# mkocabas/EpipolarPose

Measured on AMD Instinct MI355X. Metric: images/sec (4-view 256x256, ResNet-50) at 1/2/4/8 MI355X; MPJPE vs ref, higher is better.
Workload: dtype bf16; 1 GPU; configs[1]: ResNet-50 Integral-pose, 4-view 256x256 synthetic, batch=32/GPU, fully-supervised SmoothL1 loss; global_batch=32, joints=17, depth_res=64, optimizer=adam, parallelism=dp1, launch=eager, streams=2, deterministic=True

## Files before the change

### epipolarpose_amd/csrc/head_gemm.hip

```cpp
#include "common.h"
#include "bn_affine.h"
#include <algorithm>
#include <cstdlib>
#include <mutex>
#include <type_traits>
#include <unordered_map>
#include <utility>
#include <vector>

namespace epi {

typedef __bf16 bf16x8 __attribute__((ext_vector_type(8)));
typedef float f32x16 __attribute__((ext_vector_type(16)));

constexpr int GBK = 64;

template <int TM_, int WM_, int WN_, int MIN_WAVES_, int NSTAGE_, bool STAGGER_ = false> struct GemmCfg {
    static constexpr int TM = TM_, WM = WM_, WN = WN_, NW = WM_ * WN_, THREADS = 64 * NW, MIN_WAVES = MIN_WAVES_, NSTAGE = NSTAGE_;
    static constexpr bool STAGGER = STAGGER_;
    static constexpr int BM = WM_ * TM_ * 32, BN = WN_ * 64;
    static constexpr int A_BYTES = BM * 128, B_BYTES = BN * 128, STAGE_BYTES = A_BYTES + B_BYTES;
    static constexpr int AP = BM / 8 / NW, BP = BN / 8 / NW;
    static constexpr bool EARLY = NW == 4 && NSTAGE_ == 2;
    static_assert(AP >= 1 && BP >= 1 && BM % (8 * NW) == 0 && BN % (8 * NW) == 0, "whole pieces per wave");
    static_assert(NSTAGE_ >= 2 && NSTAGE_ <= 4, "LDS ring depth");
};
typedef GemmCfg<2, 2, 2, 2, 2> CfgSmall;
typedef GemmCfg<2, 4, 1, 2, 2> CfgTall;
typedef GemmCfg<4, 2, 4, 1, 2> CfgBigLock;
typedef GemmCfg<4, 2, 4, 1, 2, true> CfgBig;
typedef GemmCfg<1, 2, 2, 3, 2> CfgHalf;
typedef GemmCfg<1, 2, 1, 3, 2> CfgQuarter;
typedef GemmCfg<2, 2, 2, 1, 4> CfgSmallP;
typedef GemmCfg<2, 4, 1, 1, 3> CfgTallP;

struct GemmGather {
    int enabled;
    int Hg, Wg;
    int Hs, Ws, Cs;
    int stride;
    int dy[16], dx[16];
    int pitch;
};
struct GemmScatter {
    int enabled;
    int Hg, Wg;
    int Ho, Wo;
    int so, oy, ox;
};
struct GemmPhases {
    int enabled;
    int ntap[4];
    int dy[4][4], dx[4][4];
    long long bt_off[4];
};
struct GemmBnRed {
    const unsigned short* z;
    const unsigned short* y;
    const float* bn;
    float* sums;
    int relu;
};

struct GemmArgs {
    const unsigned short* A;
    const unsigned short* Bt;
    void* C;
    const float* bias;
    int M, N, K, lda, ldb, ldc;
    GemmGather ga;
    GemmScatter sc;
    GemmPhases ph;
    int k_per_split;
    float* slabs;
    const unsigned short* addend;
    float* stats;
    int stats_copies;
    int coalesce;
    int patch_px;
    int chunks_per_split;
    GemmBnRed br;
    int addend_step;
    int add_h, add_w;
    int store_policy;
    int bn_in_on;
    BnAffine bn_in;
};

__device__ __forceinline__ int lds_off(int row, int chunk) { return row * 128 + ((chunk ^ ((row >> 1) & 7)) << 4); }

__device__ __forceinline__ int xcd_remap(int lin, int total) {
    const int q = total >> 3, r = total & 7, xcd = lin & 7, idx = lin >> 3;
    return (xcd < r ? xcd * (q + 1) : r * (q + 1) + (xcd - r) * q) + idx;
}

__device__ uint4v epi_zero_chunk[1];

__device__ __forceinline__ void glds16(const void* gsrc, char* lds_base) {
    __builtin_amdgcn_global_load_lds((const __attribute__((address_space(1))) void*)gsrc,
                                     (__attribute__((address_space(3))) void*)lds_base, 16, 0, 0);
}

__device__ __forceinline__ uint4v add_bf16x8(uint4v a, uint4v b) {
    const unsigned int aw[4] = {a.x, a.y, a.z, a.w}, bw[4] = {b.x, b.y, b.z, b.w};
    unsigned int o[4];
#pragma unroll
    for (int k = 0; k < 4; ++k)
        o[k] = pack_bf16x2(__uint_as_float(aw[k] << 16) + __uint_as_float(bw[k] << 16),
                           __uint_as_float(aw[k] & 0xffff0000u) + __uint_as_float(bw[k] & 0xffff0000u));
    uint4v r; r.x = o[0]; r.y = o[1]; r.z = o[2]; r.w = o[3];
    return r;
}

struct BnRedCols { float mu[8], rs[8], sc[8], sh[8]; };
__device__ __forceinline__ void bnred_cols(const GemmBnRed& br, int N, int n, BnRedCols& c) {
    const bool ok = n < N;
#pragma unroll
    for (int h = 0; h < 2; ++h) {
        const float4v zero = float4v{0.f, 0.f, 0.f, 0.f};
        const float4v mu = ok ? *reinterpret_cast<const float4v*>(br.bn + n + 4 * h) : zero;
        const float4v rs = ok ? *reinterpret_cast<const float4v*>(br.bn + N + n + 4 * h) : zero;
        const float4v sc = ok ? *reinterpret_cast<const float4v*>(br.bn + 2 * N + n + 4 * h) : zero;
        const float4v sh = ok ? *reinterpret_cast<const float4v*>(br.bn + 3 * N + n + 4 * h) : zero;
        c.mu[4 * h] = mu.x; c.mu[4 * h + 1] = mu.y; c.mu[4 * h + 2] = mu.z; c.mu[4 * h + 3] = mu.w;
        c.rs[4 * h] = rs.x; c.rs[4 * h + 1] = rs.y; c.rs[4 * h + 2] = rs.z; c.rs[4 * h + 3] = rs.w;
        c.sc[4 * h] = sc.x; c.sc[4 * h + 1] = sc.y; c.sc[4 * h + 2] = sc.z; c.sc[4 * h + 3] = sc.w;
        c.sh[4 * h] = sh.x; c.sh[4 * h + 1] = sh.y; c.sh[4 * h + 2] = sh.z; c.sh[4 * h + 3] = sh.w;
    }
}
__device__ __forceinline__ uint4v bnred_apply(const GemmBnRed& br, uint4v o, uint4v zv, uint4v yv, const BnRedCols& c, float (&s)[8], float (&q)[8]);
__device__ __forceinline__ uint4v bnred_row(const GemmBnRed& br, uint4v o, long long off, const BnRedCols& c, float (&s)[8], float (&q)[8]) {
    const uint4v zv = *reinterpret_cast<const uint4v*>(br.z + off);
    uint4v yv = uint4v{0u, 0u, 0u, 0u};
    if (br.relu && br.y) yv = *reinterpret_cast<const uint4v*>(br.y + off);
    return bnred_apply(br, o, zv, yv, c, s, q);
}
__device__ __forceinline__ uint4v bnred_apply(const GemmBnRed& br, uint4v o, uint4v zv, uint4v yv, const BnRedCols& c, float (&s)[8], float (&q)[8]) {
    unsigned int ow[4] = {o.x, o.y, o.z, o.w};
    const unsigned int zw[4] = {zv.x, zv.y, zv.z, zv.w}, yw[4] = {yv.x, yv.y, yv.z, yv.w};
#pragma unroll
    for (int k = 0; k < 4; ++k) {
#pragma unroll
        for (int h = 0; h < 2; ++h) {
            const int e = 2 * k + h;
            const unsigned int keep = h ? 0xffff0000u : 0x0000ffffu;
            const float g = __uint_as_float(h ? (ow[k] & 0xffff0000u) : (ow[k] << 16));
            const float xv = __uint_as_float(h ? (zw[k] & 0xffff0000u) : (zw[k] << 16));
            bool on = true;
            if (br.relu) on = br.y ? (__uint_as_float(h ? (yw[k] & 0xffff0000u) : (yw[k] << 16)) > 0.f) : (xv * c.sc[e] + c.sh[e] > 0.f);
            const float dz = on ? g : 0.f;
            s[e] += dz;
            q[e] = fmaf(dz, (xv - c.mu[e]) * c.rs[e], q[e]);
            if (!on) ow[k] &= ~keep;
        }
    }
    uint4v r; r.x = ow[0]; r.y = ow[1]; r.z = ow[2]; r.w = ow[3];
    return r;
}

#ifdef EPI_GEMM_TRACE
constexpr int GEMM_TRACE_WGS = 8192, GEMM_TRACE_SLOTS = 16;
__device__ unsigned long long epi_gemm_trace[GEMM_TRACE_WGS * GEMM_TRACE_SLOTS];
#define GEMM_STAMP_V(i, v)                                                                                               \
    do {                                                                                                                 \
        const int wg_ = blockIdx.x + gridDim.x * (blockIdx.y + gridDim.y * blockIdx.z);                                  \
        if (threadIdx.x == 0 && wg_ < GEMM_TRACE_WGS) epi_gemm_trace[wg_ * GEMM_TRACE_SLOTS + (i)] = (v);               \
    } while (0)
#define GEMM_STAMP(i) GEMM_STAMP_V(i, __builtin_amdgcn_s_memtime())
#else
#define GEMM_STAMP_V(i, v) do {} while (0)
#define GEMM_STAMP(i) do {} while (0)
#endif

struct EpiArgs {
    void* C;
    const float* bias;
    const unsigned short* addend;
    float* stats;
    int M, N, ldc, stats_copies, addend_step, add_h, add_w, store_policy;
    GemmScatter sc;
    GemmBnRed br;
};
#define EPI_ARGS_OF(p) EpiArgs{(p).C, (p).bias, (p).addend, (p).stats, (p).M, (p).N, (p).ldc, (p).stats_copies, (p).addend_step, (p).add_h, (p).add_w, (p).store_policy, (p).sc, (p).br}
template <int TM, int WM, int WN, int THREADS, bool RED, bool RED_PREFETCH = true>
__device__ __forceinline__ void coalesced_epilogue(const EpiArgs p, f32x16 (&acc)[TM][2], char* smem, int m0, int n0, int tile_m, int wm, int wn, int wid,
                                                   int lane, int tid, int sc_oy, int sc_ox) {
    constexpr int GBN = WN * 64, ROWS = TM * 4;
    const int frow = lane & 31, fhalf = lane >> 5, c8 = lane & 7, r8 = lane >> 3;
    char* mine = smem + wid * (TM * 32 * 128);
    const int n = n0 + wn * 64 + c8 * 8;
    const int m_first = m0 + wm * (TM * 32) + r8;
    const bool col_ok = n < p.N;
    const bool scatter = p.sc.enabled != 0, has_add = p.addend != nullptr, half_add = p.addend_step == 2, nt_stores = p.store_policy == 1;
    auto row_off = [&](int it, bool& ok, auto sc_c) __attribute__((always_inline)) -> long long {
        const int m = m_first + 8 * it;
        ok = col_ok && m < p.M;
        if (!decltype(sc_c)::value) return (long long)m * p.ldc + n;
        const int hw = p.sc.Hg * p.sc.Wg;
        const int b = m / hw, rem = m - b * hw;
        const int i = rem / p.sc.Wg, j = rem - i * p.sc.Wg;
        return (((long long)b * p.sc.Ho + i * p.sc.so + sc_oy) * p.sc.Wo + j * p.sc.so + sc_ox) * p.ldc + n;
    };
    auto addend_at = [&](int m, long long off) __attribute__((always_inline)) -> uint4v {
        if (!half_add) return *reinterpret_cast<const uint4v*>(p.addend + off);
        const int hw = p.add_h * p.add_w;
        const int b = m / hw, rem = m - b * hw;
        const int yy = rem / p.add_w, xx = rem - yy * p.add_w;
        if ((yy | xx) & 1) return uint4v{0u, 0u, 0u, 0u};
        const long long ar = ((long long)b * (p.add_h >> 1) + (yy >> 1)) * (p.add_w >> 1) + (xx >> 1);
        return *reinterpret_cast<const uint4v*>(p.addend + ar * p.ldc + n);
    };
    constexpr bool AD_EARLY = !(RED && (TM >= 4 || !RED_PREFETCH));
    constexpr int RED_GROUP = 4;
    constexpr bool RED_EARLY = RED && RED_PREFETCH && TM <= 2;
    uint4v ad[AD_EARLY ? ROWS : 1];
    uint4v zpre[RED_EARLY ? ROWS : 1], ypre[RED_EARLY ? ROWS : 1];
    auto prefetch = [&](auto sc_c) __attribute__((always_inline)) {
        if (AD_EARLY && has_add) {
#pragma unroll
            for (int it = 0; it < ROWS; ++it) {
                bool ok;
                const long long off = row_off(it, ok, sc_c);
                ad[it] = ok ? addend_at(m_first + 8 * it, off) : uint4v{0u, 0u, 0u, 0u};
            }
        }
        if (RED_EARLY) {
            const bool use_y = p.br.relu && p.br.y;
#pragma unroll
            for (int it = 0; it < ROWS; ++it) {
                bool ok;
                const long long off = row_off(it, ok, sc_c);
                zpre[it] = ok ? *reinterpret_cast<const uint4v*>(p.br.z + off) : uint4v{0u, 0u, 0u, 0u};
                ypre[it] = (ok && use_y) ? *reinterpret_cast<const uint4v*>(p.br.y + off) : uint4v{0u, 0u, 0u, 0u};
            }
        }
    };
    if (RED_EARLY || (AD_EARLY && has_add)) { if (scatter) prefetch(std::true_type{}); else prefetch(std::false_type{}); }
    auto park = [&](auto bias_c) __attribute__((always_inline)) {
        constexpr bool BIAS = decltype(bias_c)::value;
#pragma unroll
        for (int tj = 0; tj < 2; ++tj)
#pragma unroll
            for (int q = 0; q < 4; ++q) {
                float b[4] = {0.f, 0.f, 0.f, 0.f};
                if (BIAS) {
                    const int nq = n0 + wn * 64 + tj * 32 + 8 * q + 4 * fhalf;
#pragma unroll
                    for (int e = 0; e < 4; ++e) b[e] = nq + e < p.N ? p.bias[nq + e] : 0.f;
                }
#pragma unroll
                for (int ti = 0; ti < TM; ++ti) {
                    const int row = ti * 32 + frow;
                    uint2 t;
                    if (BIAS) {
                        t.x = pack_bf16x2(acc[ti][tj][4 * q] + b[0], acc[ti][tj][4 * q + 1] + b[1]);
                        t.y = pack_bf16x2(acc[ti][tj][4 * q + 2] + b[2], acc[ti][tj][4 * q + 3] + b[3]);
                    } else {
                        t.x = pack_bf16x2(acc[ti][tj][4 * q], acc[ti][tj][4 * q + 1]);
                        t.y = pack_bf16x2(acc[ti][tj][4 * q + 2], acc[ti][tj][4 * q + 3]);
                    }
                    const int unit = tj * 8 + 2 * q + fhalf;
                    *reinterpret_cast<uint2*>(mine + row * 128 + ((unit ^ (row & 15)) << 3)) = t;
                }
            }
    };
    if (p.bias) park(std::true_type{}); else park(std::false_type{});
    GEMM_STAMP(5);
    float ssum[8], ssq[8];
#pragma unroll
    for (int k = 0; k < 8; ++k) { ssum[k] = 0.f; ssq[k] = 0.f; }
    BnRedCols rcols;
    if (RED) bnred_cols(p.br, p.N, n, rcols);
    auto copy_rows = [&](auto stats_c, auto add_c, auto sc_c) __attribute__((always_inline)) {
        constexpr bool STATS = decltype(stats_c)::value, ADD = decltype(add_c)::value;
#pragma unroll
        for (int it = 0; it < ROWS; ++it) {
            if (RED && !RED_EARLY && it % RED_GROUP == 0 && it) __builtin_amdgcn_sched_barrier(0);
            const int row = it * 8 + r8, sw = row & 15;
            const uint2 lo = *reinterpret_cast<const uint2*>(mine + row * 128 + (((2 * c8) ^ sw) << 3));
            const uint2 hi = *reinterpret_cast<const uint2*>(mine + row * 128 + (((2 * c8 + 1) ^ sw) << 3));
            bool ok;
            const long long off = row_off(it, ok, sc_c);
            if (!ok) continue;
            if (STATS) {
                const unsigned int w4[4] = {lo.x, lo.y, hi.x, hi.y};
#pragma unroll
                for (int k = 0; k < 4; ++k) {
                    const float a = __uint_as_float(w4[k] << 16), b = __uint_as_float(w4[k] & 0xffff0000u);
                    ssum[2 * k] += a; ssq[2 * k] = fmaf(a, a, ssq[2 * k]);
                    ssum[2 * k + 1] += b; ssq[2 * k + 1] = fmaf(b, b, ssq[2 * k + 1]);
                }
            }
            uint4v o; o.x = lo.x; o.y = lo.y; o.z = hi.x; o.w = hi.y;
            if (ADD) o = add_bf16x8(o, AD_EARLY ? ad[it] : addend_at(m_first + 8 * it, off));
            if (RED) o = RED_EARLY ? bnred_apply(p.br, o, zpre[it], ypre[it], rcols, ssum, ssq) : bnred_row(p.br, o, off, rcols, ssum, ssq);
            uint4v* dst = reinterpret_cast<uint4v*>(reinterpret_cast<unsigned short*>(p.C) + off);
            if (nt_stores) __builtin_nontemporal_store(o, dst);
            else *dst = o;
        }
    };
    const bool has_stats = !RED && p.stats != nullptr;
    auto copy_sc = [&](auto sc_c) __attribute__((always_inline)) {
        if (has_stats) { if (has_add) copy_rows(std::true_type{}, std::true_type{}, sc_c); else copy_rows(std::true_type{}, std::false_type{}, sc_c); }
        else if (has_add) copy_rows(std::false_type{}, std::true_type{}, sc_c);
        else copy_rows(std::false_type{}, std::false_type{}, sc_c);
    };
    if (scatter) copy_sc(std::true_type{}); else copy_sc(std::false_type{});
    GEMM_STAMP(6);
    if (has_stats || RED) {
#pragma unroll
        for (int k = 0; k < 8; ++k) {
#pragma unroll
            for (int o = 8; o < 64; o <<= 1) { ssum[k] += __shfl_xor(ssum[k], o, 64); ssq[k] += __shfl_xor(ssq[k], o, 64); }
        }
        float* st = reinterpret_cast<float*>(smem + WM * WN * (TM * 32 * 128));
        if (lane < 8) {
            float* row = st + wm * (2 * GBN) + wn * 64 + c8 * 8;
            *reinterpret_cast<float4v*>(row) = float4v{ssum[0], ssum[1], ssum[2], ssum[3]};
            *reinterpret_cast<float4v*>(row + 4) = float4v{ssum[4], ssum[5], ssum[6], ssum[7]};
            *reinterpret_cast<float4v*>(row + GBN) = float4v{ssq[0], ssq[1], ssq[2], ssq[3]};
            *reinterpret_cast<float4v*>(row + GBN + 4) = float4v{ssq[4], ssq[5], ssq[6], ssq[7]};
        }
        __syncthreads();
        float* dst = RED ? p.br.sums : p.stats + (long long)(tile_m % p.stats_copies) * 2 * p.N;
        for (int t = tid; t < 2 * GBN; t += THREADS) {
            float v = 0.f;
#pragma unroll
            for (int w = 0; w < WM; ++w) v += st[w * (2 * GBN) + t];
            const int which = t / GBN, col = n0 + (t % GBN);
            if (col < p.N) atomicAdd(dst + which * p.N + col, v);
        }
    }
#ifdef EPI_GEMM_TRACE
    asm volatile("s_waitcnt vmcnt(0)" ::: "memory");
    GEMM_STAMP(7);
    GEMM_STAMP_V(8, __builtin_amdgcn_s_memrealtime());
#endif
}

enum { A_PLAIN = 0, A_GATHER = 1, A_PHASED = 2 };


__device__ __forceinline__ bf16x8 bn_in_apply(bf16x8 a, const float4v (&t)[4]) {
    const uint4v u = __builtin_bit_cast(uint4v, a);
    const unsigned int w[4] = {u.x, u.y, u.z, u.w};
    unsigned int o[4];
#pragma unroll
    for (int k = 0; k < 4; ++k) {
        const float lo = __uint_as_float(w[k] << 16), hi = __uint_as_float(w[k] & 0xffff0000u);
        o[k] = pack_bf16x2(fmaxf(lo * t[k].x + t[k].y, 0.f), fmaxf(hi * t[k].z + t[k].w, 0.f));
    }
    uint4v r; r.x = o[0]; r.y = o[1]; r.z = o[2]; r.w = o[3];
    return __builtin_bit_cast(bf16x8, r);
}

template <bool OUT_F32, typename Cfg, int MODE, bool RED = false, bool BNIN = false>
__global__ __launch_bounds__(Cfg::THREADS, Cfg::MIN_WAVES) void head_gemm_kernel(GemmArgs p) {
    static_assert(!BNIN || (MODE == A_PLAIN && Cfg::NSTAGE == 2), "BatchNorm on the A operand: plain rows, two-stage loop");
    constexpr int GBM = Cfg::BM, GBN = Cfg::BN, TM = Cfg::TM, AP = Cfg::AP, BP = Cfg::BP;
    extern __shared__ __attribute__((aligned(16))) char smem[];
    const int tid = threadIdx.x, lane = tid & 63, wid = tid >> 6;
    GEMM_STAMP(0);
    GEMM_STAMP_V(1, __builtin_amdgcn_s_memrealtime());
    GEMM_STAMP_V(9, (unsigned long long)__builtin_amdgcn_s_getreg((31 << 11) | 4));
    GEMM_STAMP_V(10, (unsigned long long)__builtin_amdgcn_s_getreg((31 << 11) | 20));
    const int wm = wid / Cfg::WN, wn = wid % Cfg::WN;
    const int tiles_n = (p.N + GBN - 1) / GBN;
    const int total_wg = gridDim.x * gridDim.y * gridDim.z;
    int lid = xcd_remap(blockIdx.x + gridDim.x * (blockIdx.y + gridDim.y * blockIdx.z), total_wg);
    const int tile_id = lid % (int)gridDim.x;
    lid /= (int)gridDim.x;
    const int split_id = lid % (int)gridDim.y, phase = lid / (int)gridDim.y;
    int tile_m = tile_id / tiles_n, tile_n = tile_id - tile_m * tiles_n;
    if constexpr (GBM == 256 && GBN == 256) {
        constexpr int GM = 4;
        const int tiles_m = (p.M + GBM - 1) / GBM, per_group = GM * tiles_n, g = tile_id / per_group, i = tile_id - g * per_group;
        const int rows = min(GM, tiles_m - g * GM);
        tile_m = g * GM + i % rows;
        tile_n = i / rows;
    }
    const int m0 = tile_m * GBM, n0 = tile_n * GBN;
    const int ph = phase >> 1, pw = phase & 1;
    const unsigned short* Bt = p.Bt + (MODE == A_PHASED ? p.ph.bt_off[phase] : 0);
    const int ldb = MODE == A_PHASED ? p.ph.ntap[phase] * p.ga.Cs : p.ldb;
    const int sc_oy = MODE == A_PHASED ? ph : p.sc.oy, sc_ox = MODE == A_PHASED ? pw : p.sc.ox;
    const int k_total = MODE == A_PHASED ? p.ph.ntap[phase] * p.ga.Cs : p.K;
    const int k_begin = split_id * p.k_per_split;
    const int k_end = min(k_total, k_begin + p.k_per_split);
    const int* tap_dy = MODE == A_PHASED ? p.ph.dy[phase] : p.ga.dy;
    const int* tap_dx = MODE == A_PHASED ? p.ph.dx[phase] : p.ga.dx;

    const int schunk_phys = lane & 7;
    int a_pix[AP], a_mask[AP], a_chunk[AP], b_chunk[BP];
    const unsigned short* a_ptr[AP];
    const unsigned short* b_ptr[BP];
    bool b_ok[BP];
    const int ntaps = MODE == A_PLAIN ? 0 : k_total / p.ga.Cs;
#pragma unroll
    for (int ps = 0; ps < AP; ++ps) {
        const int trow = (wid * AP + ps) * 8 + (lane >> 3);
        a_chunk[ps] = (schunk_phys ^ ((trow >> 1) & 7)) * 8;
        const int m = m0 + trow;
        const bool ok = m < p.M;
        if (MODE != A_PLAIN) {
            const int hw = p.ga.Hg * p.ga.Wg;
            const int n = m / hw, rem = m - n * hw;
            const int i = rem / p.ga.Wg, j = rem - i * p.ga.Wg;
            const int iy = i * p.ga.stride, jx = j * p.ga.stride;
            a_pix[ps] = (n * p.ga.Hs + iy) * p.ga.Ws + jx;
            int mask = 0;
            for (int t = 0; t < ntaps; ++t) {
                const int y = iy + tap_dy[t], x = jx + tap_dx[t];
                if (ok && (unsigned)y < (unsigned)p.ga.Hs && (unsigned)x < (unsigned)p.ga.Ws) mask |= 1 << t;
            }
            a_mask[ps] = mask;
            a_ptr[ps] = p.A + a_chunk[ps];
        } else {
            a_pix[ps] = 0;
            a_mask[ps] = ok ? 1 : 0;
            a_ptr[ps] = p.A + (long long)(ok ? m : 0) * p.lda + a_chunk[ps];
        }
    }
#pragma unroll
    for (int ps = 0; ps < BP; ++ps) {
        const int trow = (wid * BP + ps) * 8 + (lane >> 3);
        b_chunk[ps] = (schunk_phys ^ ((trow >> 1) & 7)) * 8;
        const int n = n0 + trow;
        b_ok[ps] = n < p.N;
        b_ptr[ps] = Bt + (long long)(b_ok[ps] ? n : 0) * ldb + b_chunk[ps];
    }
    const char* zero_src = reinterpret_cast<const char*>(epi_zero_chunk);
    const int nk = k_end > k_begin ? (k_end - k_begin + GBK - 1) / GBK : 0;
    int k_run = k_begin;
    int g_tap = MODE == A_PLAIN ? 0 : k_run / p.ga.Cs;
    int g_c0 = MODE == A_PLAIN ? 0 : k_run - g_tap * p.ga.Cs;
    int g_shift = (MODE == A_PLAIN || ntaps == 0) ? 0 : tap_dy[min(g_tap, ntaps - 1)] * p.ga.Ws + tap_dx[min(g_tap, ntaps - 1)];
    auto issue_a = [&](int ps, int, int buf) {
        const int k0 = k_run;
        char* a_s = smem + buf * Cfg::STAGE_BYTES + __builtin_amdgcn_readfirstlane(wid) * (AP * 1024);
        const void* src;
        if (MODE != A_PLAIN) {
            const unsigned eoff = (unsigned)(a_pix[ps] + g_shift) * (unsigned)(p.ga.pitch ? p.ga.pitch : p.ga.Cs) + (unsigned)g_c0;
            const bool in_k = !Cfg::STAGGER || k0 < k_end;
            src = (in_k && ((a_mask[ps] >> (g_tap & 31)) & 1)) ? reinterpret_cast<const void*>(a_ptr[ps] + eoff) : reinterpret_cast<const void*>(zero_src);
        } else {
            const bool ok = a_mask[ps] && (k0 + a_chunk[ps] < k_end);
            src = ok ? reinterpret_cast<const void*>(a_ptr[ps] + k0) : reinterpret_cast<const void*>(zero_src);
        }
        glds16(src, a_s + ps * 1024);
    };
    auto issue_b = [&](int ps, int, int buf) {
        const int k0 = k_run;
        char* b_s = smem + buf * Cfg::STAGE_BYTES + Cfg::A_BYTES + __builtin_amdgcn_readfirstlane(wid) * (BP * 1024);
        const bool ok = b_ok[ps] && (MODE != A_PLAIN || k0 + b_chunk[ps] < k_end);
        glds16(ok ? reinterpret_cast<const void*>(b_ptr[ps] + k0) : reinterpret_cast<const void*>(zero_src), b_s + ps * 1024);
    };
    auto advance_gather = [&]() {
        k_run += GBK;
        if (MODE != A_PLAIN) {
            g_c0 += GBK;
            if (g_c0 >= p.ga.Cs) {
                g_c0 = 0;
                g_tap += 1;
                const int t = min(g_tap, ntaps - 1);
                g_shift = tap_dy[t] * p.ga.Ws + tap_dx[t];
            }
        }
    };
    auto issue_tile = [&](int k0, int buf) {
#pragma unroll
        for (int ps = 0; ps < AP; ++ps) issue_a(ps, k0, buf);
#pragma unroll
        for (int ps = 0; ps < BP; ++ps) issue_b(ps, k0, buf);
        advance_gather();
    };

    f32x16 acc[TM][2];
#pragma unroll
    for (int i = 0; i < TM; ++i)
#pragma unroll
        for (int j = 0; j < 2; ++j)
#pragma unroll
            for (int r = 0; r < 16; ++r) acc[i][j][r] = 0.f;

    const int frow = lane & 31, fhalf = lane >> 5;
    float2* bn_tab = reinterpret_cast<float2*>(smem + Cfg::NSTAGE * Cfg::STAGE_BYTES);
    if (BNIN) {
        const bool lead = (blockIdx.x | blockIdx.y | blockIdx.z) == 0;
        for (int k = tid; k < p.K; k += Cfg::THREADS) {
            float sc, sh;
            bn_derive(p.bn_in, p.K, k, lead, sc, sh);
            bn_tab[k] = float2{sc, sh};
        }
        if (lead && tid == 0 && p.bn_in.num_batches && p.bn_in.sums) p.bn_in.num_batches[0] += 1;
    }
    const int a_frag = lds_off(wm * (TM * 32) + frow, fhalf), b_frag = lds_off(wn * 64 + frow, fhalf);
    auto read_frags = [&](const char* a_s, const char* b_s, int ks, bf16x8 (&af)[TM], bf16x8 (&bfr)[2]) {
#pragma unroll
        for (int t = 0; t < TM; ++t)
            af[t] = __builtin_bit_cast(bf16x8, *reinterpret_cast<const uint4v*>(a_s + ((a_frag ^ (ks << 5)) + t * 4096)));
#pragma unroll
        for (int t = 0; t < 2; ++t)
            bfr[t] = __builtin_bit_cast(bf16x8, *reinterpret_cast<const uint4v*>(b_s + ((b_frag ^ (ks << 5)) + t * 4096)));
    };
    auto issue_quarter = [&](int ks, int k0, int buf) {
#pragma unroll
        for (int ps = 0; ps < AP; ++ps)
            if (ps * 4 / AP == ks) issue_a(ps, k0, buf);
#pragma unroll
        for (int ps = 0; ps < BP; ++ps)
            if ((BP >= 4 ? ps * 4 / BP : ps) == ks) issue_b(ps, k0, buf);
        if (ks == 3) advance_gather();
    };
    auto compute_tile = [&](int buf, bool spread_next, int k_next, int buf_next, int k_tile = 0) {
        const char* a_s = smem + buf * Cfg::STAGE_BYTES;
        const char* b_s = a_s + Cfg::A_BYTES;
        bf16x8 af[2][TM], bfr[2][2];
        float4v bt[2][4];
        auto read_tab = [&](int ks, float4v (&t)[4]) {
            const float4v* src = reinterpret_cast<const float4v*>(bn_tab + k_tile + ks * 16 + fhalf * 8);
#pragma unroll
            for (int q = 0; q < 4; ++q) t[q] = src[q];
        };
        read_frags(a_s, b_s, 0, af[0], bfr[0]);
        if (BNIN) read_tab(0, bt[0]);
#pragma unroll
        for (int ks = 0; ks < 4; ++ks) {
            if (ks < 3) read_frags(a_s, b_s, ks + 1, af[(ks + 1) & 1], bfr[(ks + 1) & 1]);
            if (BNIN && ks < 3) read_tab(ks + 1, bt[(ks + 1) & 1]);
            __builtin_amdgcn_sched_barrier(0);
            if (BNIN) {
#pragma unroll
                for (int ti = 0; ti < TM; ++ti) af[ks & 1][ti] = bn_in_apply(af[ks & 1][ti], bt[ks & 1]);
            }
            if (spread_next) issue_quarter(ks, k_next, buf_next);
#pragma unroll
            for (int ti = 0; ti < TM; ++ti)
#pragma unroll
                for (int tj = 0; tj < 2; ++tj)
                    acc[ti][tj] = __builtin_amdgcn_mfma_f32_32x32x16_bf16(bfr[ks & 1][tj], af[ks & 1][ti], acc[ti][tj], 0, 0, 0);
        }
    };
    GEMM_STAMP(2);
    GEMM_STAMP_V(11, (unsigned long long)nk);
    if constexpr (Cfg::STAGGER) {
        static_assert(AP == 4 && BP == 4 && TM == 4 && Cfg::NW == 8 && Cfg::NSTAGE == 2 && !BNIN, "staggered loop: 256 x 256 tile, 8 waves");
        const int grp = __builtin_amdgcn_readfirstlane(wid) >> 2;
        int kb_run = k_begin;
        auto issue_a_tile = [&](int buf) {
#pragma unroll
            for (int ps = 0; ps < AP; ++ps) issue_a(ps, 0, buf);
            advance_gather();
        };
        auto issue_b_tile = [&](int buf) {
            char* b_s = smem + buf * Cfg::STAGE_BYTES + Cfg::A_BYTES + __builtin_amdgcn_readfirstlane(wid) * (BP * 1024);
#pragma unroll
            for (int ps = 0; ps < BP; ++ps) {
                const bool ok = b_ok[ps] && kb_run + b_chunk[ps] < k_end;
                glds16(ok ? reinterpret_cast<const void*>(b_ptr[ps] + kb_run) : reinterpret_cast<const void*>(zero_src), b_s + ps * 1024);
            }
            kb_run += GBK;
        };
        issue_b_tile(0);
        issue_a_tile(0);
        issue_b_tile(1);
        asm volatile("s_waitcnt vmcnt(4)" ::: "memory");
        __builtin_amdgcn_s_barrier();
        GEMM_STAMP(3);
        if (grp) __builtin_amdgcn_s_barrier();
        bf16x8 af[4][2], bfr[4][2];
        auto mfma_half = [&](int h) {
            __builtin_amdgcn_s_setprio(1);
#pragma unroll
            for (int ks = 0; ks < 4; ++ks)
#pragma unroll
                for (int ti = 0; ti < 2; ++ti)
#pragma unroll
                    for (int tj = 0; tj < 2; ++tj)
                        acc[2 * h + ti][tj] = __builtin_amdgcn_mfma_f32_32x32x16_bf16(bfr[ks][tj], af[ks][ti], acc[2 * h + ti][tj], 0, 0, 0);
            __builtin_amdgcn_s_setprio(0);
        };
        for (int kt = 0; kt < nk; ++kt) {
            const int buf = kt & 1;
            const char* a_s = smem + buf * Cfg::STAGE_BYTES;
            const char* b_s = a_s + Cfg::A_BYTES;
#pragma unroll
            for (int ks = 0; ks < 4; ++ks)
#pragma unroll
                for (int tj = 0; tj < 2; ++tj)
                    bfr[ks][tj] = __builtin_bit_cast(bf16x8, *reinterpret_cast<const uint4v*>(b_s + ((b_frag ^ (ks << 5)) + tj * 4096)));
#pragma unroll
            for (int ks = 0; ks < 4; ++ks)
#pragma unroll
                for (int ti = 0; ti < 2; ++ti)
                    af[ks][ti] = __builtin_bit_cast(bf16x8, *reinterpret_cast<const uint4v*>(a_s + ((a_frag ^ (ks << 5)) + ti * 4096)));
            __builtin_amdgcn_sched_barrier(0);
            issue_a_tile(buf ^ 1);
            __builtin_amdgcn_sched_barrier(0);
            asm volatile("s_waitcnt lgkmcnt(0)" ::: "memory");
            __builtin_amdgcn_s_barrier();
            __builtin_amdgcn_sched_barrier(0);
            mfma_half(0);
            __builtin_amdgcn_sched_barrier(0);
            asm volatile("s_waitcnt vmcnt(4)" ::: "memory");
            __builtin_amdgcn_s_barrier();
            __builtin_amdgcn_sched_barrier(0);
#pragma unroll
            for (int ks = 0; ks < 4; ++ks)
#pragma unroll
                for (int ti = 0; ti < 2; ++ti)
                    af[ks][ti] = __builtin_bit_cast(bf16x8, *reinterpret_cast<const uint4v*>(a_s + ((a_frag ^ (ks << 5)) + (2 + ti) * 4096)));
            __builtin_amdgcn_sched_barrier(0);
            issue_b_tile(buf);
            __builtin_amdgcn_sched_barrier(0);
            asm volatile("s_waitcnt lgkmcnt(0)" ::: "memory");
            __builtin_amdgcn_s_barrier();
            __builtin_amdgcn_sched_barrier(0);
            mfma_half(1);
            __builtin_amdgcn_sched_barrier(0);
            asm volatile("s_waitcnt vmcnt(4)" ::: "memory");
            __builtin_amdgcn_s_barrier();
            __builtin_amdgcn_sched_barrier(0);
        }
        if (!grp) __builtin_amdgcn_s_barrier();
        asm volatile("s_waitcnt vmcnt(0) lgkmcnt(0)" ::: "memory");
        __builtin_amdgcn_s_barrier();
    } else if constexpr (Cfg::NSTAGE > 2) {
        constexpr int S = Cfg::NSTAGE, DPT = AP + BP;
#pragma unroll
        for (int t = 0; t < S - 1; ++t)
            if (t < nk) issue_tile(k_begin + t * GBK, t);
        int kt = 0;
        for (; kt + (S - 2) < nk; ++kt) {
            asm volatile("s_waitcnt vmcnt(%0)" ::"n"((S - 2) * DPT) : "memory");
            __builtin_amdgcn_s_barrier();
#ifdef EPI_GEMM_TRACE
            if (kt == 0) GEMM_STAMP(3);
#endif
            const int nxt = kt + S - 1;
            compute_tile(kt % S, nxt < nk, k_begin + nxt * GBK, nxt % S);
        }
        for (; kt < nk; ++kt) {
            if (S > 3 && nk - 1 - kt == 1) asm volatile("s_waitcnt vmcnt(%0)" ::"n"(DPT) : "memory");
            else asm volatile("s_waitcnt vmcnt(0)" ::: "memory");
            __builtin_amdgcn_s_barrier();
            compute_tile(kt % S, false, 0, 0);
        }
        asm volatile("s_waitcnt lgkmcnt(0)" ::: "memory");
        __builtin_amdgcn_s_barrier();
    } else {
        if (nk > 0) issue_tile(k_begin, 0);
        __syncthreads();
        GEMM_STAMP(3);
        for (int kt = 0; kt < nk; ++kt) {
            const bool has_next = kt + 1 < nk;
            const int k_next = k_begin + (kt + 1) * GBK, buf = kt & 1;
            if (Cfg::EARLY && has_next) issue_tile(k_next, buf ^ 1);
            compute_tile(buf, !Cfg::EARLY && has_next, k_next, buf ^ 1, k_begin + kt * GBK);
            __syncthreads();
        }
    }

    GEMM_STAMP(4);
    if (gridDim.y > 1) {
        float* slab = p.slabs + ((long long)split_id * gridDim.z + phase) * p.M * p.N;
#pragma unroll
        for (int ti = 0; ti < TM; ++ti) {
            const int m = m0 + wm * (TM * 32) + ti * 32 + frow;
            if (m >= p.M) continue;
#pragma unroll
            for (int tj = 0; tj < 2; ++tj)
#pragma unroll
                for (int q = 0; q < 4; ++q) {
                    const int n = n0 + wn * 64 + tj * 32 + 8 * q + 4 * fhalf;
                    if (n + 3 < p.N) {
                        float4v t; t.x = acc[ti][tj][4 * q]; t.y = acc[ti][tj][4 * q + 1]; t.z = acc[ti][tj][4 * q + 2]; t.w = acc[ti][tj][4 * q + 3];
                        *reinterpret_cast<float4v*>(slab + (long long)m * p.N + n) = t;
                    } else {
                        for (int e = 0; e < 4 && n + e < p.N; ++e) slab[(long long)m * p.N + n + e] = acc[ti][tj][4 * q + e];
                    }
                }
        }
#ifdef EPI_GEMM_TRACE
        GEMM_STAMP(6);
        asm volatile("s_waitcnt vmcnt(0)" ::: "memory");
        GEMM_STAMP(7);
        GEMM_STAMP_V(8, __builtin_amdgcn_s_memrealtime());
#endif
        return;
    }
    if constexpr (!OUT_F32) {
        if (p.coalesce) {
            coalesced_epilogue<TM, Cfg::WM, Cfg::WN, Cfg::THREADS, RED>(EPI_ARGS_OF(p), acc, smem, m0, n0, tile_m, wm, wn, wid, lane, tid, sc_oy, sc_ox);
            return;
        }
    }
#pragma unroll
    for (int ti = 0; ti < TM; ++ti) {
        const int m = m0 + wm * (TM * 32) + ti * 32 + frow;
        const bool row_ok = m < p.M;
        long long orow = m;
        if (p.sc.enabled) {
            const int hw = p.sc.Hg * p.sc.Wg;
            const int n = m / hw, rem = m - n * hw;
            const int i = rem / p.sc.Wg, j = rem - i * p.sc.Wg;
            orow = ((long long)n * p.sc.Ho + i * p.sc.so + sc_oy) * p.sc.Wo + j * p.sc.so + sc_ox;
        }
#pragma unroll
        for (int tj = 0; tj < 2; ++tj) {
#pragma unroll
            for (int q = 0; q < 4; ++q) {
                const int n = n0 + wn * 64 + tj * 32 + 8 * q + 4 * fhalf;
                float v[4];
#pragma unroll
                for (int e = 0; e < 4; ++e) {
                    v[e] = acc[ti][tj][4 * q + e];
                    if (p.bias && n + e < p.N) v[e] += p.bias[n + e];
                }
                if (row_ok && n < p.N) {
                    if (OUT_F32) {
                        float* c = reinterpret_cast<float*>(p.C) + orow * p.ldc + n;
                        if (n + 3 < p.N) { float4v t; t.x = v[0]; t.y = v[1]; t.z = v[2]; t.w = v[3]; *reinterpret_cast<float4v*>(c) = t; }
                        else for (int e = 0; e < 4 && n + e < p.N; ++e) c[e] = v[e];
                    } else {
                        unsigned short* c = reinterpret_cast<unsigned short*>(p.C) + orow * p.ldc + n;
                        if (p.addend)
                            for (int e = 0; e < 4 && n + e < p.N; ++e) v[e] = bf16_to_f32(f32_to_bf16(v[e])) + bf16_to_f32(p.addend[orow * p.ldc + n + e]);
                        if (n + 3 < p.N) {
                            uint2 t;
                            t.x = pack_bf16x2(v[0], v[1]);
                            t.y = pack_bf16x2(v[2], v[3]);
                            *reinterpret_cast<uint2*>(c) = t;
                        } else for (int e = 0; e < 4 && n + e < p.N; ++e) c[e] = f32_to_bf16(v[e]);
                    }
                }
            }
        }
    }
}

constexpr int AS_WAVES = 8, AS_LOADERS = 2, AS_RING = 3;
constexpr int AS_THREADS = 64 * (AS_WAVES + AS_LOADERS), AS_BM = 32 * AS_WAVES, AS_BN = 64;

template <int KSTEPS>
__global__ __launch_bounds__(AS_THREADS, 1) void head_gemm_astat_kernel(GemmArgs p) {
    constexpr int K = 16 * KSTEPS, ROW_BYTES = 2 * K, CHUNKS = ROW_BYTES / 16;
    constexpr int BTILE = AS_BN * ROW_BYTES;
    constexpr int ROWS_PER_PIECE = 1024 / ROW_BYTES, PIECES = BTILE / 1024 / AS_LOADERS;
    extern __shared__ __attribute__((aligned(16))) char smem[];
    const int tid = threadIdx.x, lane = tid & 63, wid = tid >> 6;
    const bool loader = wid >= AS_WAVES;
    const int frow = lane & 31, fhalf = lane >> 5;
    const int m0 = xcd_remap(blockIdx.x, gridDim.x) * AS_BM + wid * 32;
    const int n_tiles = (p.N + AS_BN - 1) / AS_BN;
    const char* zero_src = reinterpret_cast<const char*>(epi_zero_chunk);
    float* bias_s = reinterpret_cast<float*>(smem + AS_RING * BTILE + AS_WAVES * 4096);
    float* stats_s = bias_s + n_tiles * AS_BN;
    for (int n = tid; n < n_tiles * AS_BN; n += AS_THREADS) bias_s[n] = (p.bias && n < p.N) ? p.bias[n] : 0.f;
    if (p.stats)
        for (int n = tid; n < 2 * n_tiles * AS_BN; n += AS_THREADS) stats_s[n] = 0.f;

    auto issue_b = [&](int nt) {
        const int lw = wid - AS_WAVES;
        char* dst = smem + (nt % AS_RING) * BTILE + lw * (PIECES * 1024);
#pragma unroll 8
        for (int q = 0; q < PIECES; ++q) {
            const int r = (lw * PIECES + q) * ROWS_PER_PIECE + lane / CHUNKS;
            const int chunk = (lane % CHUNKS) ^ (r % CHUNKS);
            const int n = nt * AS_BN + r;
            const void* src = n < p.N ? reinterpret_cast<const void*>(p.Bt + (long long)n * p.ldb + chunk * 8)
                                      : reinterpret_cast<const void*>(zero_src);
            glds16(src, dst + q * 1024);
        }
    };
    bf16x8 af[KSTEPS];
    if (loader) {
        issue_b(0);
        if (n_tiles > 1) issue_b(1);
    } else {
        const int m = m0 + frow;
        const uint4v* arow = reinterpret_cast<const uint4v*>(p.A + (long long)(m < p.M ? m : 0) * p.lda) + fhalf;
#pragma unroll
        for (int ks = 0; ks < KSTEPS; ++ks) {
            uint4v v = arow[2 * ks];
            if (m >= p.M) v.x = v.y = v.z = v.w = 0u;
            af[ks] = __builtin_bit_cast(bf16x8, v);
        }
    }
    __syncthreads();
    if (loader) {
        for (int nt = 0; nt < n_tiles; ++nt) {
            if (nt + 2 < n_tiles) {
                issue_b(nt + 2);
                asm volatile("s_waitcnt vmcnt(%0)\n\ts_barrier" ::"n"(PIECES) : "memory");
            } else {
                asm volatile("s_waitcnt vmcnt(0)\n\ts_barrier" ::: "memory");
            }
        }
        if (p.stats) __builtin_amdgcn_s_barrier();
        return;
    }
    char* stage = smem + AS_RING * BTILE + wid * 4096;
    const int c8 = lane & 7;
    auto slices = [&](auto add_c, auto stats_c) __attribute__((always_inline)) {
    constexpr bool ADD = decltype(add_c)::value, STATS = decltype(stats_c)::value;
    for (int nt = 0; nt < n_tiles; ++nt) {
        f32x16 acc[2];
#pragma unroll
        for (int j = 0; j < 2; ++j)
#pragma unroll
            for (int r = 0; r < 16; ++r) acc[j][r] = 0.f;
        const unsigned slice_off = (unsigned)(nt % AS_RING) * BTILE;
        auto read_b = [&](int ks, uint4v (&f)[2]) {
#pragma unroll
            for (int tj = 0; tj < 2; ++tj) {
                const int r = tj * 32 + frow;
                const unsigned off = (slice_off + r * ROW_BYTES + (((fhalf ^ r) % CHUNKS) << 4)) ^ (unsigned)(((2 * ks) % CHUNKS) << 4);
                f[tj] = *reinterpret_cast<const uint4v*>(smem + off);
            }
        };
        uint4v ad[4];
        auto load_addend = [&]() {
            if (!ADD) return;
#pragma unroll
            for (int it = 0; it < 4; ++it) {
                const int m = m0 + it * 8 + (lane >> 3), nn = nt * AS_BN + (lane & 7) * 8;
                ad[it] = (m < p.M && nn < p.N) ? *reinterpret_cast<const uint4v*>(p.addend + (long long)m * p.ldc + nn) : uint4v{0u, 0u, 0u, 0u};
            }
        };
        if (KSTEPS <= 8) load_addend();
        uint4v fb[3][2];
        read_b(0, fb[0]);
        if (KSTEPS > 1) read_b(1, fb[1]);
#pragma unroll
        for (int ks = 0; ks < KSTEPS; ++ks) {
            if (ks + 2 < KSTEPS) read_b(ks + 2, fb[(ks + 2) % 3]);
            __builtin_amdgcn_sched_barrier(0);
#pragma unroll
            for (int tj = 0; tj < 2; ++tj)
                acc[tj] = __builtin_amdgcn_mfma_f32_32x32x16_bf16(__builtin_bit_cast(bf16x8, fb[ks % 3][tj]), af[ks], acc[tj], 0, 0, 0);
        }
        asm volatile("s_waitcnt lgkmcnt(0)\n\ts_barrier" ::: "memory");
        const int n0 = nt * AS_BN;
#pragma unroll
        for (int tj = 0; tj < 2; ++tj)
#pragma unroll
            for (int q = 0; q < 4; ++q) {
                const int nl = tj * 32 + 8 * q + 4 * fhalf;
                const float4v bv = *reinterpret_cast<const float4v*>(bias_s + n0 + nl);
                const float v0 = acc[tj][4 * q] + bv.x, v1 = acc[tj][4 * q + 1] + bv.y, v2 = acc[tj][4 * q + 2] + bv.z,
                            v3 = acc[tj][4 * q + 3] + bv.w;
                uint2 t;
                t.x = pack_bf16x2(v0, v1);
                t.y = pack_bf16x2(v2, v3);
                const int unit = tj * 8 + 2 * q + fhalf;
                *reinterpret_cast<uint2*>(stage + frow * 128 + ((unit ^ (frow & 15)) << 3)) = t;
            }
        const int n = n0 + c8 * 8;
        float ssum[8], ssq[8];
#pragma unroll
        for (int k = 0; k < 8; ++k) { ssum[k] = 0.f; ssq[k] = 0.f; }
#pragma unroll
        for (int it = 0; it < 4; ++it) {
            const int row = it * 8 + (lane >> 3), sw = row & 15;
            const uint2 lo = *reinterpret_cast<const uint2*>(stage + row * 128 + (((2 * c8) ^ sw) << 3));
            const uint2 hi = *reinterpret_cast<const uint2*>(stage + row * 128 + (((2 * c8 + 1) ^ sw) << 3));
            const int m = m0 + row;
            if (m < p.M && n < p.N) {
                uint4v o; o.x = lo.x; o.y = lo.y; o.z = hi.x; o.w = hi.y;
                if (ADD) o = add_bf16x8(o, KSTEPS <= 8 ? ad[it] : *reinterpret_cast<const uint4v*>(p.addend + (long long)m * p.ldc + n));
                *reinterpret_cast<uint4v*>(reinterpret_cast<unsigned short*>(p.C) + (long long)m * p.ldc + n) = o;
                if (STATS) {
                    const unsigned int w4[4] = {lo.x, lo.y, hi.x, hi.y};
#pragma unroll
                    for (int k = 0; k < 4; ++k) {
                        const float a = __uint_as_float(w4[k] << 16), b = __uint_as_float(w4[k] & 0xffff0000u);
                        ssum[2 * k] += a; ssq[2 * k] = fmaf(a, a, ssq[2 * k]);
                        ssum[2 * k + 1] += b; ssq[2 * k + 1] = fmaf(b, b, ssq[2 * k + 1]);
                    }
                }
            }
        }
        if (STATS) {
#pragma unroll
            for (int k = 0; k < 8; ++k) {
#pragma unroll
                for (int o = 8; o < 64; o <<= 1) { ssum[k] += __shfl_xor(ssum[k], o, 64); ssq[k] += __shfl_xor(ssq[k], o, 64); }
            }
            if (lane < 8) {
#pragma unroll
                for (int k = 0; k < 8; ++k) {
                    atomicAdd(stats_s + n + k, ssum[k]);
                    atomicAdd(stats_s + n_tiles * AS_BN + n + k, ssq[k]);
                }
            }
        }
    }
    };
    if (p.addend) { if (p.stats) slices(std::true_type{}, std::true_type{}); else slices(std::true_type{}, std::false_type{}); }
    else if (p.stats) slices(std::false_type{}, std::true_type{});
    else slices(std::false_type{}, std::false_type{});
    if (p.stats) {
        asm volatile("s_waitcnt lgkmcnt(0)\n\ts_barrier" ::: "memory");
        float* dst = p.stats + (long long)(blockIdx.x % p.stats_copies) * 2 * p.N;
        for (int n = tid; n < p.N; n += 64 * AS_WAVES) {
            atomicAdd(dst + n, stats_s[n]);
            atomicAdd(dst + p.N + n, stats_s[n_tiles * AS_BN + n]);
        }
    }
}

template <int TM_, int WM_, int WN_> struct PatchCfg {
    static constexpr int TM = TM_, WM = WM_, WN = WN_, NW = WM_ * WN_, THREADS = 64 * NW;
    static constexpr int BM = WM_ * TM_ * 32, BN = WN_ * 64, B_BYTES = BN * 128, BP = BN / 8 / NW;
    static_assert(NW == 8 && BP >= 1, "8 waves");
};
typedef PatchCfg<2, 4, 2> PatchWide;
typedef PatchCfg<1, 8, 1> PatchNarrow;
typedef PatchCfg<1, 4, 2> PatchHalf;
constexpr int PATCH_TAPS = 9, PATCH_APW = 8;

#ifdef EPI_PATCH_TRACE
__device__ unsigned long long epi_patch_trace[64 * 96];
#define PATCH_STAMP(i)                                                                                                   \
    do {                                                                                                                 \
        const int wg_ = blockIdx.x + gridDim.x * blockIdx.y;                                                             \
        if (lane == 0 && wid == 0 && wg_ % 16 == 0 && wg_ / 16 < 64 && (i) < 96) epi_patch_trace[(wg_ / 16) * 96 + (i)] = __builtin_amdgcn_s_memtime(); \
    } while (0)
#else
#define PATCH_STAMP(i) do {} while (0)
#endif

template <typename Cfg, int NB, bool SINGLE, bool RED = false>
__global__ __launch_bounds__(Cfg::THREADS, SINGLE ? 4 : 2) void conv_patch_kernel(GemmArgs p) {
    constexpr int TM = Cfg::TM, GBN = Cfg::BN, BP = Cfg::BP, NW = Cfg::NW, BB = Cfg::B_BYTES;
    constexpr int NPATCH = SINGLE ? 1 : 2, GROUP = BP + (SINGLE ? 0 : 1);
    extern __shared__ __attribute__((aligned(16))) char smem[];
    const int tid = threadIdx.x, lane = tid & 63, wid = __builtin_amdgcn_readfirstlane(tid >> 6);
    const int wm = wid / Cfg::WN, wn = wid % Cfg::WN;
    const int tiles_n = (p.N + GBN - 1) / GBN;
    const int lid = xcd_remap(blockIdx.x + gridDim.x * blockIdx.y, gridDim.x * gridDim.y);
    const int tile_id = lid % (int)gridDim.x, split_id = lid / (int)gridDim.x;
    const int tile_m = tile_id / tiles_n, tile_n = tile_id - tile_m * tiles_n;
    const int m0 = tile_m * Cfg::BM, n0 = tile_n * GBN;
    const int W = p.ga.Wg, H = p.ga.Hg, Cs = p.ga.Cs;
    const int c_begin = split_id * p.chunks_per_split, c_end = min(Cs / GBK, c_begin + p.chunks_per_split);
    const int PB = p.patch_px * 128;
    const int ring_off = NPATCH * PB, dummy_off = ring_off + NB * BB, zero_off = dummy_off + 1024;
    PATCH_STAMP(0);
    if (tid < 32) reinterpret_cast<float*>(smem + zero_off)[tid] = 0.f;
    const char* zero_src = reinterpret_cast<const char*>(epi_zero_chunk);

    auto a_off = [&](int j) -> int {
        const int prow = (j * NW + wid) * 8 + (lane >> 3);
        const long long pin = (long long)m0 - (W + 1) + prow;
        const bool ok = prow < p.patch_px && pin >= 0 && pin < p.M;
        return ok ? (int)pin * Cs + (((lane & 7) ^ ((prow >> 1) & 7)) << 3) : -1;
    };
    const unsigned short* b_ptr[BP];
    bool b_ok[BP];
#pragma unroll
    for (int ps = 0; ps < BP; ++ps) {
        const int trow = (wid * BP + ps) * 8 + (lane >> 3);
        const int n = n0 + trow;
        b_ok[ps] = n < p.N;
        b_ptr[ps] = p.Bt + (long long)(b_ok[ps] ? n : 0) * p.ldb + (((lane & 7) ^ ((trow >> 1) & 7)) << 3);
    }
    auto issue_a = [&](int j, int c, int buf) {
        const bool real = j < PATCH_APW && (j * NW + wid) * 8 < p.patch_px && c < c_end;
        char* dst = real ? smem + buf * PB + (j * NW + wid) * 1024 : smem + dummy_off;
        const int off = a_off(j);
        glds16((real && off >= 0) ? reinterpret_cast<const void*>(p.A + off + c * GBK) : reinterpret_cast<const void*>(zero_src), dst);
    };
    auto issue_b = [&](int t, int c, int slot, bool real) {
#pragma unroll
        for (int ps = 0; ps < BP; ++ps) {
            char* dst = real ? smem + ring_off + slot * BB + (wid * BP + ps) * 1024 : smem + dummy_off;
            const void* src = (real && b_ok[ps]) ? reinterpret_cast<const void*>(b_ptr[ps] + t * Cs + c * GBK) : reinterpret_cast<const void*>(zero_src);
            glds16(src, dst);
        }
    };

    const int frow = lane & 31, fhalf = lane >> 5;
    const int b_frag = ring_off + lds_off(wn * 64 + frow, fhalf);

    f32x16 acc[TM][2];
#pragma unroll
    for (int i = 0; i < TM; ++i)
#pragma unroll
        for (int j = 0; j < 2; ++j)
#pragma unroll
            for (int r = 0; r < 16; ++r) acc[i][j][r] = 0.f;

    const int nsteps = (c_end - c_begin) * PATCH_TAPS;
    if (nsteps > 0) {
#pragma unroll
        for (int j = 0; j < PATCH_APW; ++j) issue_a(j, c_begin, 0);
        issue_b(0, c_begin, 0, true);
        if (NB > 2) issue_b(1, c_begin, 1, true);
    }
    __builtin_amdgcn_sched_barrier(0);
    int amask[TM], arow[TM];
#pragma unroll
    for (int ti = 0; ti < TM; ++ti) {
        const int r = wm * (TM * 32) + ti * 32 + frow, m = m0 + r;
        arow[ti] = r;
        const int j = m % W, i = (m / W) % H;
        int mask = 0;
#pragma unroll
        for (int t = 0; t < PATCH_TAPS; ++t) {
            const int y = i + p.ga.dy[t], x = j + p.ga.dx[t];
            if (m < p.M && (unsigned)y < (unsigned)H && (unsigned)x < (unsigned)W) mask |= 1 << t;
        }
        amask[ti] = mask;
    }
    PATCH_STAMP(1);
    asm volatile("s_waitcnt vmcnt(0) lgkmcnt(0)" ::: "memory");
    __builtin_amdgcn_s_barrier();
    PATCH_STAMP(2);
    int step_no = 0;

    int slot = 0;
    for (int c = c_begin; c < c_end; ++c) {
        const int pbuf = SINGLE ? 0 : (c - c_begin) & 1;
#pragma unroll
        for (int t = 0; t < PATCH_TAPS; ++t) {
            {
                int ta = t + NB - 1, ca = c;
                if (ta >= PATCH_TAPS) { ta -= PATCH_TAPS; ca += 1; }
                int sa = slot + NB - 1; if (sa >= NB) sa -= NB;
                issue_b(ta, ca, sa, ca < c_end);
                if (!SINGLE) issue_a(t, c + 1, pbuf ^ 1);
            }
            const int sh = (p.ga.dy[t] + 1) * W + p.ga.dx[t] + 1;
            int a_addr[TM];
#pragma unroll
            for (int ti = 0; ti < TM; ++ti) {
                const int pr = arow[ti] + sh;
                const int in = pbuf * PB + pr * 128 + ((fhalf ^ ((pr >> 1) & 7)) << 4);
                a_addr[ti] = ((amask[ti] >> t) & 1) ? in : zero_off;
            }
            const int b_addr = b_frag + slot * BB;
            bf16x8 af[2][TM], bfr[2][2];
            auto read_frags = [&](int ks, bf16x8 (&a)[TM], bf16x8 (&b)[2]) {
#pragma unroll
                for (int ti = 0; ti < TM; ++ti) a[ti] = __builtin_bit_cast(bf16x8, *reinterpret_cast<const uint4v*>(smem + (a_addr[ti] ^ (ks << 5))));
#pragma unroll
                for (int tj = 0; tj < 2; ++tj) b[tj] = __builtin_bit_cast(bf16x8, *reinterpret_cast<const uint4v*>(smem + ((b_addr ^ (ks << 5)) + tj * 4096)));
            };
            read_frags(0, af[0], bfr[0]);
#pragma unroll
            for (int ks = 0; ks < 4; ++ks) {
                if (ks < 3) read_frags(ks + 1, af[(ks + 1) & 1], bfr[(ks + 1) & 1]);
                __builtin_amdgcn_sched_barrier(0);
#pragma unroll
                for (int ti = 0; ti < TM; ++ti)
#pragma unroll
                    for (int tj = 0; tj < 2; ++tj)
                        acc[ti][tj] = __builtin_amdgcn_mfma_f32_32x32x16_bf16(bfr[ks & 1][tj], af[ks & 1][ti], acc[ti][tj], 0, 0, 0);
            }
            asm volatile("s_waitcnt vmcnt(%0)" ::"n"((NB - 2) * GROUP) : "memory");
            __builtin_amdgcn_s_barrier();
            slot = slot + 1 == NB ? 0 : slot + 1;
            PATCH_STAMP(3 + step_no);
            ++step_no;
        }
    }
    asm volatile("s_waitcnt vmcnt(0) lgkmcnt(0)" ::: "memory");
    __builtin_amdgcn_s_barrier();
    PATCH_STAMP(3 + step_no);

    if (gridDim.y > 1) {
        float* slab = p.slabs + (long long)split_id * p.M * p.N;
#pragma unroll
        for (int ti = 0; ti < TM; ++ti) {
            const int m = m0 + arow[ti];
            if (m >= p.M) continue;
#pragma unroll
            for (int tj = 0; tj < 2; ++tj)
#pragma unroll
                for (int q = 0; q < 4; ++q) {
                    const int n = n0 + wn * 64 + tj * 32 + 8 * q + 4 * fhalf;
                    if (n + 3 < p.N) {
                        float4v t; t.x = acc[ti][tj][4 * q]; t.y = acc[ti][tj][4 * q + 1]; t.z = acc[ti][tj][4 * q + 2]; t.w = acc[ti][tj][4 * q + 3];
                        *reinterpret_cast<float4v*>(slab + (long long)m * p.N + n) = t;
                    }
                }
        }
#ifdef EPI_PATCH_TRACE
        asm volatile("s_waitcnt vmcnt(0)" ::: "memory");
        PATCH_STAMP(4 + step_no);
#endif
        return;
    }
    coalesced_epilogue<TM, Cfg::WM, Cfg::WN, Cfg::THREADS, RED, false>(EPI_ARGS_OF(p), acc, smem, m0, n0, tile_m, wm, wn, wid, lane, tid, 0, 0);
#ifdef EPI_PATCH_TRACE
    asm volatile("s_waitcnt vmcnt(0)" ::: "memory");
    PATCH_STAMP(4 + step_no);
#endif
}

template <bool OUT_F32>
__global__ void splitk_finish_kernel(const float* __restrict__ slabs, int nsplit, int nphase, GemmArgs p) {
    const long long nq = (long long)p.N >> 2;
    const long long t = (long long)blockIdx.x * blockDim.x + threadIdx.x;
    if (t >= (long long)nphase * p.M * nq) return;
    const int n = (int)(t % nq) * 4;
    const long long pm = t / nq;
    const int m = (int)(pm % p.M), phase = (int)(pm / p.M);
    float4v a; a.x = a.y = a.z = a.w = 0.f;
    for (int s = 0; s < nsplit; ++s) {
        const float4v v = *reinterpret_cast<const float4v*>(slabs + (((long long)s * nphase + phase) * p.M + m) * p.N + n);
        a.x += v.x; a.y += v.y; a.z += v.z; a.w += v.w;
    }
    if (p.bias) { a.x += p.bias[n]; a.y += p.bias[n + 1]; a.z += p.bias[n + 2]; a.w += p.bias[n + 3]; }
    long long orow = m;
    if (p.sc.enabled) {
        const int hw = p.sc.Hg * p.sc.Wg;
        const int b = m / hw, rem = m - b * hw;
        const int i = rem / p.sc.Wg, j = rem - i * p.sc.Wg;
        const int oy = p.ph.enabled ? (phase >> 1) : p.sc.oy, ox = p.ph.enabled ? (phase & 1) : p.sc.ox;
        orow = ((long long)b * p.sc.Ho + i * p.sc.so + oy) * p.sc.Wo + j * p.sc.so + ox;
    }
    if (OUT_F32) {
        *reinterpret_cast<float4v*>(reinterpret_cast<float*>(p.C) + orow * p.ldc + n) = a;
    } else {
        if (p.addend) {
            const uint2 r = *reinterpret_cast<const uint2*>(p.addend + orow * p.ldc + n);
            a.x = bf16_to_f32(f32_to_bf16(a.x)) + __uint_as_float(r.x << 16); a.y = bf16_to_f32(f32_to_bf16(a.y)) + __uint_as_float(r.x & 0xffff0000u);
            a.z = bf16_to_f32(f32_to_bf16(a.z)) + __uint_as_float(r.y << 16); a.w = bf16_to_f32(f32_to_bf16(a.w)) + __uint_as_float(r.y & 0xffff0000u);
        }
        uint2 o;
        o.x = pack_bf16x2(a.x, a.y);
        o.y = pack_bf16x2(a.z, a.w);
        *reinterpret_cast<uint2*>(reinterpret_cast<unsigned short*>(p.C) + orow * p.ldc + n) = o;
    }
}

constexpr int FS_ROWS = 32;
__global__ __launch_bounds__(256) void splitk_finish_stats_kernel(const float* __restrict__ slabs, int nsplit, GemmArgs p) {
    __shared__ float red[4][2][256];
    const int tx = threadIdx.x & 63, ty = threadIdx.x >> 6;
    const int col_tiles = (p.N + 255) / 256;
    const int tile_m = blockIdx.x / col_tiles, tile_n = blockIdx.x - tile_m * col_tiles;
    const int n = tile_n * 256 + tx * 4;
    float s1[4] = {0.f, 0.f, 0.f, 0.f}, s2[4] = {0.f, 0.f, 0.f, 0.f};
    if (n < p.N) {
        for (int r = ty; r < FS_ROWS; r += 4) {
            const int m = tile_m * FS_ROWS + r;
            if (m >= p.M) break;
            float4v a; a.x = a.y = a.z = a.w = 0.f;
            for (int sp = 0; sp < nsplit; ++sp) {
                const float4v v = *reinterpret_cast<const float4v*>(slabs + ((long long)sp * p.M + m) * p.N + n);
                a.x += v.x; a.y += v.y; a.z += v.z; a.w += v.w;
            }
            uint2 o;
            o.x = pack_bf16x2(a.x, a.y);
            o.y = pack_bf16x2(a.z, a.w);
            *reinterpret_cast<uint2*>(reinterpret_cast<unsigned short*>(p.C) + (long long)m * p.ldc + n) = o;
            const float v[4] = {__uint_as_float(o.x << 16), __uint_as_float(o.x & 0xffff0000u), __uint_as_float(o.y << 16), __uint_as_float(o.y & 0xffff0000u)};
#pragma unroll
            for (int e = 0; e < 4; ++e) { s1[e] += v[e]; s2[e] = fmaf(v[e], v[e], s2[e]); }
        }
    }
#pragma unroll
    for (int e = 0; e < 4; ++e) { red[ty][0][tx * 4 + e] = s1[e]; red[ty][1][tx * 4 + e] = s2[e]; }
    __syncthreads();
    float* dst = p.stats + (long long)(tile_m % p.stats_copies) * 2 * p.N;
    for (int t = threadIdx.x; t < 512; t += 256) {
        const int which = t >> 8, c = t & 255, col = tile_n * 256 + c;
        if (col < p.N) atomicAdd(dst + which * p.N + col, red[0][which][c] + red[1][which][c] + red[2][which][c] + red[3][which][c]);
    }
}

}

using namespace epi;

enum { CFG_SMALL = 0, CFG_TALL = 1, CFG_BIG = 2, CFG_HALF = 3, CFG_QUARTER = 4 };
struct GemmPlan { int cfg; int nsplit, kps; long long tiles; int pipe; };

static int g_tile_force_fwd();
static int gemm_tile_override() {
    const int v = 0;
    const int f = g_tile_force_fwd();
    return f == 1 || f == 2 ? f : (f == 5 ? 2 : v);
}

static int g_pipe_force_fwd();
static int gemm_pipe_mode() {
    const int v = 0;
    const int f = g_pipe_force_fwd();
    return f >= 0 ? f : v;
}

static int g_store_policy = -1;
static int gemm_store_policy() {
    if (g_store_policy < 0) g_store_policy = 0;
    return g_store_policy;
}
extern "C" int epi_gemm_store_policy(int v) {
    const int before = gemm_store_policy();
    if (v >= 0) g_store_policy = v;
    return before;
}
static int g_tile_force = 0, g_pipe_force = -1;
extern "C" int epi_gemm_tune(int tile, int pipe) {
    if (tile >= 0) g_tile_force = tile;
    if (pipe >= -1) g_pipe_force = pipe;
    return g_tile_force;
}

static int g_tile_force_fwd() { return g_tile_force; }
static int g_pipe_force_fwd() { return g_pipe_force; }

static GemmPlan gemm_plan_cfg(int cfg, int M, int N, int K, int nphase, bool pipe = false) {
    GemmPlan pl;
    pl.cfg = cfg;
    pl.pipe = pipe ? 1 : 0;
    const int bm = cfg == CFG_SMALL ? 128 : (cfg == CFG_HALF || cfg == CFG_QUARTER ? 64 : 256);
    const int bn = cfg == CFG_BIG ? 256 : (cfg == CFG_TALL || cfg == CFG_QUARTER ? 64 : 128);
    pl.tiles = (long long)((M + bm - 1) / bm) * ((N + bn - 1) / bn);
    const long long wgs = pl.tiles * nphase;
    const bool one_per_cu = cfg == CFG_BIG || pipe;
    const long long enough_env = 120;
    const long long enough = enough_env, target = one_per_cu ? 256 : 512;
    int nsplit = 1;
    if (wgs < enough) {
        nsplit = (int)(target / wgs);
        const int max_split = K / 512 > 0 ? K / 512 : 1;
        if (nsplit > max_split) nsplit = max_split;
        if (nsplit > 16) nsplit = 16;
        if (nsplit < 1) nsplit = 1;
    }
    if (N % 4) nsplit = 1;
    pl.kps = K;
    if (nsplit > 1) {
        pl.kps = ((K + nsplit - 1) / nsplit + GBK - 1) / GBK * GBK;
        nsplit = (K + pl.kps - 1) / pl.kps;
    }
    pl.nsplit = nsplit;
    return pl;
}

static GemmPlan gemm_plan(int M, int N, int K, int ldc, int nphase, bool out_f32, bool allow_pipe = true) {
    const int ov = gemm_tile_override();
    const bool can_big = !out_f32 && N % 8 == 0 && ldc % 8 == 0;
    if (can_big && ov != 1) {
        const GemmPlan pb = gemm_plan_cfg(CFG_BIG, M, N, K, nphase);
        const int tiles_n = (N + 255) / 256;
        const bool fills = M >= 256 && tiles_n * 256 <= N + N / 4;
        const bool deep = pb.nsplit == 1 ? (K >= 512 && pb.tiles * nphase >= 200) : pb.kps >= 1024;
        const bool big_split_ok = false;
        const bool small_fills_unsplit = (long long)((M + 127) / 128) * ((N + 127) / 128) * nphase >= 200;
        if (ov == 2 || (fills && deep && (pb.nsplit == 1 || big_split_ok || !small_fills_unsplit))) return pb;
    }
    int cfg = (ov == 0 && !out_f32 && N <= 64 && (long long)M * nphase >= 256 * 256) ? CFG_TALL : CFG_SMALL;
    const long long fill_env = 0;
    if (cfg == CFG_SMALL && !out_f32 && (g_tile_force == 3 || g_tile_force == 4)) cfg = g_tile_force == 3 ? CFG_HALF : CFG_QUARTER;
    else if (cfg == CFG_SMALL && ov == 0 && !out_f32 && fill_env > 0) {
        const long long t128 = (long long)((M + 127) / 128) * ((N + 127) / 128) * nphase;
        const long long t64x128 = (long long)((M + 63) / 64) * ((N + 127) / 128) * nphase;
        if (t128 < fill_env) cfg = t64x128 < fill_env ? CFG_QUARTER : CFG_HALF;
    }
    const int pm = (out_f32 || !allow_pipe || cfg == CFG_HALF || cfg == CFG_QUARTER) ? 0 : gemm_pipe_mode();
    if (pm) {
        const GemmPlan pp = gemm_plan_cfg(cfg, M, N, K, nphase, true);
        const bool one_round = pp.tiles * nphase * pp.nsplit <= 256;
        const bool long_underfilled = pp.tiles * nphase * pp.nsplit <= 128 && pp.kps >= 32 * GBK;
        if (pm == 2 || (pm == 1 && pp.kps >= 6 * GBK) || (pm == 3 && one_round && pp.kps >= 6 * GBK) || (pm == 4 && long_underfilled)) return pp;
    }
    return gemm_plan_cfg(cfg, M, N, K, nphase);
}

extern "C" size_t epi_gemm_workspace_bytes(int M, int N, int K, int nphase) {
    if (M <= 0 || N <= 0 || K <= 0 || nphase <= 0) return 0;
    size_t need = 0;
    for (int pipe = 0; pipe < 2; ++pipe) {
        for (int f32 = 0; f32 < 2; ++f32) {
            const GemmPlan pl = gemm_plan(M, N, K, 8, nphase, f32 != 0, pipe != 0);
            if (pl.nsplit > 1) need = std::max(need, (size_t)pl.nsplit * nphase * M * N * sizeof(float));
        }
        const GemmPlan ps = gemm_plan(M, N, K, 4, nphase, false, pipe != 0);
        if (ps.nsplit > 1) need = std::max(need, (size_t)ps.nsplit * nphase * M * N * sizeof(float));
    }
    return need;
}

template <bool OUT_F32, typename Cfg, int MODE, bool RED = false, bool BNIN = false>
static int launch_gemm_mode(const GemmArgs& a, const GemmPlan& pl, int nphase, hipStream_t st) {
    constexpr size_t ring = (size_t)Cfg::NSTAGE * Cfg::STAGE_BYTES;
    const bool one_tile = !BNIN && !Cfg::STAGGER && Cfg::NSTAGE == 2 && pl.kps <= GBK;
    const size_t staged = one_tile ? (size_t)Cfg::STAGE_BYTES : ring;
    const size_t lds = BNIN ? ring + (size_t)a.K * sizeof(float2)
                            : std::max(staged, (size_t)Cfg::WM * Cfg::WN * (Cfg::TM * 32 * 128) + (size_t)Cfg::WM * 2 * Cfg::BN * sizeof(float));
    static_assert(!BNIN || ring >= (size_t)Cfg::WM * Cfg::WN * (Cfg::TM * 32 * 128) + (size_t)Cfg::WM * 2 * Cfg::BN * sizeof(float), "epilogue areas end below the table");
    if (lds > 65536) {
        constexpr size_t full = std::max(ring, (size_t)Cfg::WM * Cfg::WN * (Cfg::TM * 32 * 128) + (size_t)Cfg::WM * 2 * Cfg::BN * sizeof(float));
        static const hipError_t attr = hipFuncSetAttribute(reinterpret_cast<const void*>(&head_gemm_kernel<OUT_F32, Cfg, MODE, RED, BNIN>),
                                                           hipFuncAttributeMaxDynamicSharedMemorySize, BNIN ? (int)(ring + 2048 * sizeof(float2)) : (int)full);
        if (attr != hipSuccess) return EPI_ERR_LAUNCH;
    }
    const dim3 grid((unsigned)pl.tiles, (unsigned)pl.nsplit, (unsigned)nphase);
    hipLaunchKernelGGL((head_gemm_kernel<OUT_F32, Cfg, MODE, RED, BNIN>), grid, dim3(Cfg::THREADS), lds, st, a);
    EPI_CHECK_LAUNCH();
    return EPI_OK;
}
template <bool OUT_F32, typename Cfg, bool RED = false>
static int launch_gemm_cfg(const GemmArgs& a, const GemmPlan& pl, int nphase, hipStream_t st) {
    if (a.ph.enabled) return launch_gemm_mode<OUT_F32, Cfg, A_PHASED, RED>(a, pl, nphase, st);
    if (a.ga.enabled) return launch_gemm_mode<OUT_F32, Cfg, A_GATHER, RED>(a, pl, nphase, st);
    return launch_gemm_mode<OUT_F32, Cfg, A_PLAIN, RED>(a, pl, nphase, st);
}

#ifdef EPI_GEMM_TRACE
extern "C" int epi_gemm_trace_read(unsigned long long* out, int clear) {
    const size_t bytes = sizeof(unsigned long long) * epi::GEMM_TRACE_WGS * epi::GEMM_TRACE_SLOTS;
    if (hipMemcpyFromSymbol(out, HIP_SYMBOL(epi::epi_gemm_trace), bytes) != hipSuccess) return 1;
    if (clear) {
        static unsigned long long zeros[epi::GEMM_TRACE_WGS * epi::GEMM_TRACE_SLOTS];
        if (hipMemcpyToSymbol(HIP_SYMBOL(epi::epi_gemm_trace), zeros, bytes) != hipSuccess) return 1;
    }
    return 0;
}
#endif

#ifdef EPI_PATCH_TRACE
extern "C" int epi_patch_trace_read(unsigned long long* out, int clear) {
    if (hipMemcpyFromSymbol(out, HIP_SYMBOL(epi::epi_patch_trace), sizeof(unsigned long long) * 64 * 96) != hipSuccess) return 1;
    if (clear) {
        static unsigned long long zeros[64 * 96];
        if (hipMemcpyToSymbol(HIP_SYMBOL(epi::epi_patch_trace), zeros, sizeof(zeros)) != hipSuccess) return 1;
    }
    return 0;
}
#endif

enum { PATCH_WIDE = 0, PATCH_NARROW = 1, PATCH_HALF = 2 };
struct PatchPlan { bool ok; int cfg, nb, patch_px, nsplit, cps; long long tiles; size_t lds; bool single; };
static int g_patch_mode = -1;
static int patch_mode() {
    if (g_patch_mode < 0) g_patch_mode = 2;
    return g_patch_mode;
}
extern "C" int epi_conv3x3_patch_mode(int mode) {
    const int before = patch_mode();
    if (mode >= 0 && mode <= 2) g_patch_mode = mode;
    return before;
}
static PatchPlan patch_plan(int M, int N, int Cs, int W, size_t workspace_bytes) {
    PatchPlan pl = {};
    const int nchunks = Cs / GBK;
    pl.cfg = N <= 64 ? PATCH_NARROW : PATCH_WIDE;
    if (pl.cfg == PATCH_WIDE && (long long)((M + 255) / 256) * ((N + 127) / 128) < 200) pl.cfg = PATCH_HALF;
    const int bm = pl.cfg == PATCH_HALF ? 128 : 256, bn = pl.cfg == PATCH_NARROW ? 64 : 128;
    const int tm = pl.cfg == PATCH_WIDE ? 2 : 1, wmv = pl.cfg == PATCH_NARROW ? 8 : 4;
    pl.patch_px = (bm + 2 * W + 2 + 7) / 8 * 8;
    if (pl.patch_px > 8 * 8 * PATCH_APW) return pl;
    const size_t epi = (size_t)8 * tm * 32 * 128 + (size_t)wmv * 2 * bn * sizeof(float);
    pl.single = pl.cfg == PATCH_NARROW && nchunks == 1;
    for (pl.nb = 3; pl.nb >= 2; --pl.nb) {
        pl.lds = std::max((size_t)(pl.single ? 1 : 2) * pl.patch_px * 128 + (size_t)pl.nb * bn * 128 + 1024 + 128, epi);
        if (pl.lds <= 160 * 1024) break;
    }
    if (pl.nb < 2) return pl;
    pl.tiles = (long long)((M + bm - 1) / bm) * ((N + bn - 1) / bn);
    pl.nsplit = 1;
    if (pl.tiles < 120) {
        if (patch_mode() < 2) return pl;
        pl.nsplit = (int)std::min<long long>(nchunks, std::max<long long>(1, 256 / pl.tiles));
    }
    while (pl.nsplit > 1 && (size_t)pl.nsplit * M * N * sizeof(float) > workspace_bytes) --pl.nsplit;
    pl.cps = (nchunks + pl.nsplit - 1) / pl.nsplit;
    pl.nsplit = (nchunks + pl.cps - 1) / pl.cps;
    pl.ok = pl.tiles <= 0x7fffffffLL;
    return pl;
}
static bool patch_eligible(const GemmArgs& a, bool out_f32, int nphase) {
    if (patch_mode() == 0 || out_f32 || nphase != 1 || !a.ga.enabled || a.ph.enabled || a.sc.enabled || a.bias || !a.coalesce) return false;
    if (a.ga.stride != 1 || a.ga.Hg != a.ga.Hs || a.ga.Wg != a.ga.Ws || a.ga.Cs % GBK || a.K != PATCH_TAPS * a.ga.Cs || a.ga.pitch) return false;
    for (int t = 0; t < PATCH_TAPS; ++t)
        if (a.ga.dy[t] < -1 || a.ga.dy[t] > 1 || a.ga.dx[t] < -1 || a.ga.dx[t] > 1) return false;
    return (long long)a.M * a.ga.Cs < (1LL << 31) && gemm_tile_override() == 0;
}
template <typename Cfg, int NB, bool SINGLE = false, bool RED = false>
static int launch_patch_red(const GemmArgs& a, const PatchPlan& pl, hipStream_t st) {
    static const hipError_t attr = hipFuncSetAttribute(reinterpret_cast<const void*>(&conv_patch_kernel<Cfg, NB, SINGLE, RED>),
                                                       hipFuncAttributeMaxDynamicSharedMemorySize, 160 * 1024);
    if (attr != hipSuccess) return EPI_ERR_LAUNCH;
    hipLaunchKernelGGL((conv_patch_kernel<Cfg, NB, SINGLE, RED>), dim3((unsigned)pl.tiles, (unsigned)pl.nsplit), dim3(Cfg::THREADS), pl.lds, st, a);
    EPI_CHECK_LAUNCH();
    return EPI_OK;
}
template <typename Cfg, int NB, bool SINGLE = false>
static int launch_patch(const GemmArgs& a, const PatchPlan& pl, hipStream_t st) {
    return a.br.z ? launch_patch_red<Cfg, NB, SINGLE, true>(a, pl, st) : launch_patch_red<Cfg, NB, SINGLE, false>(a, pl, st);
}

static int launch_gemm(GemmArgs a, bool out_f32, int nphase, void* workspace, size_t workspace_bytes, hipStream_t st, int* stats_done = nullptr,
                       int* red_done = nullptr) {
    if (stats_done) *stats_done = 0;
    if (red_done) *red_done = 0;
    a.store_policy = gemm_store_policy();
    const bool fuse_red = true;
    GemmBnRed want_red = a.br;
    a.br = GemmBnRed{};
    const long long red_max_rows = 1LL << 40;
    const long long red_min_rows = 0;
    if (deterministic() || !fuse_red || !red_done || !want_red.z || !want_red.bn || !want_red.sums || a.stats || a.bias ||
        ((reinterpret_cast<uintptr_t>(want_red.z) | reinterpret_cast<uintptr_t>(want_red.y)) & 15u) || (long long)a.M * nphase > red_max_rows ||
        (long long)a.M * nphase < red_min_rows)
        want_red.z = nullptr;
    if (a.addend && (out_f32 || (reinterpret_cast<uintptr_t>(a.addend) & 15u))) return EPI_ERR_UNSUPPORTED;
    a.coalesce = (!out_f32 && a.N % 8 == 0 && a.ldc % 8 == 0) ? 1 : 0;
    const bool half_addend = a.addend && a.addend_step == 2;
    if (half_addend && (!a.coalesce || a.ga.enabled || a.sc.enabled || a.ph.enabled || nphase != 1 || a.add_h <= 0 || a.add_w <= 0 || ((a.add_h | a.add_w) & 1) ||
                        (long long)a.M % ((long long)a.add_h * a.add_w)))
        return EPI_ERR_UNSUPPORTED;
    const bool fuse_stats = true;
    float* const want_stats = (fuse_stats && !deterministic()) ? a.stats : nullptr;
    a.stats = nullptr;
    if (!a.A || !a.Bt || !a.C || a.M <= 0 || a.N <= 0 || a.K <= 0) return EPI_ERR_INVALID_ARGUMENT;
    if (a.K % 8 || a.ldb % 8 || a.ldc % 4 || (!a.ga.enabled && a.lda % 8)) return EPI_ERR_UNSUPPORTED;
    if ((reinterpret_cast<uintptr_t>(a.A) | reinterpret_cast<uintptr_t>(a.Bt) | reinterpret_cast<uintptr_t>(a.C)) & 15u) return EPI_ERR_UNSUPPORTED;
    if (a.ga.enabled && (a.ga.Cs % GBK)) return EPI_ERR_UNSUPPORTED;
    if (a.bn_in_on) {
        if (out_f32 || a.ga.enabled || a.sc.enabled || a.ph.enabled || nphase != 1 || a.K % GBK || a.K > 2048 || want_red.z || a.bias || a.addend || !a.coalesce ||
            !a.bn_in.gamma || !a.bn_in.beta || !a.bn_in.scale || !a.bn_in.shift)
            return EPI_ERR_UNSUPPORTED;
        const GemmPlan pl = gemm_plan_cfg(CFG_SMALL, a.M, a.N, a.K, 1);
        if (pl.tiles > 0x7fffffffLL) return EPI_ERR_UNSUPPORTED;
        if (pl.nsplit > 1) {
            if (!workspace || (size_t)pl.nsplit * a.M * a.N * sizeof(float) > workspace_bytes) return EPI_ERR_WORKSPACE;
            a.slabs = (float*)workspace;
        }
        a.k_per_split = pl.kps;
        if (want_stats && pl.nsplit == 1) { a.stats = want_stats; if (stats_done) *stats_done = 1; }
        const int rc = launch_gemm_mode<false, CfgSmall, A_PLAIN, false, true>(a, pl, 1, st);
        if (rc != EPI_OK) return rc;
        if (pl.nsplit > 1) {
            if (want_stats && a.N % 4 == 0) {
                a.stats = want_stats;
                if (stats_done) *stats_done = 1;
                const unsigned blocks = (unsigned)(((a.M + FS_ROWS - 1) / FS_ROWS) * ((a.N + 255) / 256));
                hipLaunchKernelGGL(splitk_finish_stats_kernel, dim3(blocks), dim3(256), 0, st, a.slabs, pl.nsplit, a);
            } else {
                const long long n = (long long)a.M * (a.N >> 2);
                hipLaunchKernelGGL(splitk_finish_kernel<false>, dim3((unsigned)((n + 255) / 256)), dim3(256), 0, st, a.slabs, pl.nsplit, 1, a);
            }
            EPI_CHECK_LAUNCH();
        }
        return EPI_OK;
    }
    const bool stats_off_astat = true;
    if (!want_red.z && !(want_stats && stats_off_astat && !a.bias) && !half_addend &&
        !out_f32 && !a.ga.enabled && !a.sc.enabled && nphase == 1 && (a.K == 64 || a.K == 128 || a.K == 256) && a.N % 8 == 0 &&
        a.ldc % 8 == 0 && a.N >= 4 * AS_BN && a.N <= 8192 && a.M >= 64 * AS_BM && gemm_tile_override() == 0) {
        const unsigned grid = (unsigned)((a.M + AS_BM - 1) / AS_BM);
        const bool astat_stats = false;
        if (want_stats && !a.bias && astat_stats) { a.stats = want_stats; if (stats_done) *stats_done = 1; }
#define EPI_ASTAT(KS)                                                                                                      \
        do {                                                                                                               \
            const size_t lds = AS_RING * (size_t)AS_BN * 32 * KS + AS_WAVES * 4096 + (size_t)((a.N + AS_BN - 1) / AS_BN) * AS_BN * 4 * 3;                                          \
            static const hipError_t attr = hipFuncSetAttribute(reinterpret_cast<const void*>(&head_gemm_astat_kernel<KS>),  \
                                                               hipFuncAttributeMaxDynamicSharedMemorySize, (int)lds);      \
            if (attr != hipSuccess) return EPI_ERR_LAUNCH;                                                                 \
            hipLaunchKernelGGL((head_gemm_astat_kernel<KS>), dim3(grid), dim3(AS_THREADS), lds, st, a);                     \
        } while (0)
        if (a.K == 256) EPI_ASTAT(16);
        else if (a.K == 128) EPI_ASTAT(8);
        else EPI_ASTAT(4);
#undef EPI_ASTAT
        EPI_CHECK_LAUNCH();
        return EPI_OK;
    }
    if (patch_eligible(a, out_f32, nphase)) {
        const PatchPlan pp = patch_plan(a.M, a.N, a.ga.Cs, a.ga.Wg, workspace ? workspace_bytes : 0);
        if (pp.ok) {
            a.patch_px = pp.patch_px;
            a.chunks_per_split = pp.cps;
            if (pp.nsplit > 1) a.slabs = (float*)workspace;
            else if (want_stats) { a.stats = want_stats; if (stats_done) *stats_done = 1; }
            else if (want_red.z) { a.br = want_red; *red_done = 1; }
            int rc;
            if (pp.cfg == PATCH_NARROW && pp.single) rc = pp.nb == 3 ? launch_patch<PatchNarrow, 3, true>(a, pp, st) : launch_patch<PatchNarrow, 2, true>(a, pp, st);
            else if (pp.cfg == PATCH_NARROW) rc = pp.nb == 3 ? launch_patch<PatchNarrow, 3>(a, pp, st) : launch_patch<PatchNarrow, 2>(a, pp, st);
            else if (pp.cfg == PATCH_HALF) rc = pp.nb == 3 ? launch_patch<PatchHalf, 3>(a, pp, st) : launch_patch<PatchHalf, 2>(a, pp, st);
            else rc = pp.nb == 3 ? launch_patch<PatchWide, 3>(a, pp, st) : launch_patch<PatchWide, 2>(a, pp, st);
            if (rc != EPI_OK) return rc;
            if (pp.nsplit > 1) {
                if (want_stats && !a.addend) {
                    a.stats = want_stats;
                    if (stats_done) *stats_done = 1;
                    const unsigned blocks = (unsigned)(((a.M + FS_ROWS - 1) / FS_ROWS) * ((a.N + 255) / 256));
                    hipLaunchKernelGGL(splitk_finish_stats_kernel, dim3(blocks), dim3(256), 0, st, a.slabs, pp.nsplit, a);
                } else {
                    const long long n = (long long)a.M * (a.N >> 2);
                    hipLaunchKernelGGL(splitk_finish_kernel<false>, dim3((unsigned)((n + 255) / 256)), dim3(256), 0, st, a.slabs, pp.nsplit, 1, a);
                }
                EPI_CHECK_LAUNCH();
            }
            return EPI_OK;
        }
    }
    GemmPlan pl = gemm_plan(a.M, a.N, a.K, a.ldc, nphase, out_f32);
    if (want_red.z && pl.pipe && pl.cfg != CFG_SMALL) pl = gemm_plan(a.M, a.N, a.K, a.ldc, nphase, out_f32, false);
    if (pl.tiles > 0x7fffffffLL) return EPI_ERR_UNSUPPORTED;
    if (half_addend && pl.nsplit > 1) return EPI_ERR_UNSUPPORTED;
    if (pl.nsplit > 1) {
        if (!workspace || (size_t)pl.nsplit * nphase * a.M * a.N * sizeof(float) > workspace_bytes) return EPI_ERR_WORKSPACE;
        a.slabs = (float*)workspace;
    }
    a.k_per_split = pl.kps;
    if (want_stats && pl.nsplit == 1 && a.coalesce && !a.bias) { a.stats = want_stats; if (stats_done) *stats_done = 1; }
    if (want_red.z && pl.nsplit == 1 && a.coalesce && (!pl.pipe || pl.cfg == CFG_SMALL) && (pl.cfg == CFG_BIG || pl.cfg == CFG_SMALL || pl.cfg == CFG_TALL)) {
        a.br = want_red;
        *red_done = 1;
    }
    int rc;
    if (a.br.z) rc = pl.cfg == CFG_BIG ? launch_gemm_cfg<false, CfgBig, true>(a, pl, nphase, st)
                   : (pl.cfg == CFG_TALL ? launch_gemm_cfg<false, CfgTall, true>(a, pl, nphase, st)
                      : (pl.pipe ? launch_gemm_cfg<false, CfgSmallP, true>(a, pl, nphase, st) : launch_gemm_cfg<false, CfgSmall, true>(a, pl, nphase, st)));
    else if (pl.cfg == CFG_BIG) rc = g_tile_force == 5 ? launch_gemm_cfg<false, CfgBigLock>(a, pl, nphase, st) : launch_gemm_cfg<false, CfgBig>(a, pl, nphase, st);
    else if (out_f32) rc = launch_gemm_cfg<true, CfgSmall>(a, pl, nphase, st);
    else if (pl.cfg == CFG_HALF) rc = launch_gemm_cfg<false, CfgHalf>(a, pl, nphase, st);
    else if (pl.cfg == CFG_QUARTER) rc = launch_gemm_cfg<false, CfgQuarter>(a, pl, nphase, st);
    else if (pl.cfg == CFG_TALL) rc = pl.pipe ? launch_gemm_cfg<false, CfgTallP>(a, pl, nphase, st) : launch_gemm_cfg<false, CfgTall>(a, pl, nphase, st);
    else rc = pl.pipe ? launch_gemm_cfg<false, CfgSmallP>(a, pl, nphase, st) : launch_gemm_cfg<false, CfgSmall>(a, pl, nphase, st);
    if (rc != EPI_OK) return rc;
    if (pl.nsplit > 1) {
        const long long n = (long long)nphase * a.M * (a.N >> 2);
        const dim3 fg((unsigned)((n + 255) / 256));
        if (!out_f32 && want_stats && nphase == 1 && !a.bias && !a.addend && !a.sc.enabled && !a.ph.enabled && a.N % 4 == 0) {
            a.stats = want_stats;
            if (stats_done) *stats_done = 1;
            const unsigned blocks = (unsigned)(((a.M + FS_ROWS - 1) / FS_ROWS) * ((a.N + 255) / 256));
            hipLaunchKernelGGL(splitk_finish_stats_kernel, dim3(blocks), dim3(256), 0, st, a.slabs, pl.nsplit, a);
        } else if (out_f32) hipLaunchKernelGGL(splitk_finish_kernel<true>, fg, dim3(256), 0, st, a.slabs, pl.nsplit, nphase, a);
        else hipLaunchKernelGGL(splitk_finish_kernel<false>, fg, dim3(256), 0, st, a.slabs, pl.nsplit, nphase, a);
        EPI_CHECK_LAUNCH();
    }
    return EPI_OK;
}

static GemmBnRed bnred_args(const EpiBnReduce* r) {
    GemmBnRed b = {};
    if (r && r->z && r->bn && r->sums) {
        b.z = (const unsigned short*)r->z; b.y = (const unsigned short*)r->y; b.bn = r->bn; b.sums = r->sums; b.relu = r->relu ? 1 : 0;
    }
    return b;
}

extern "C" int epi_gemm_bf16_bnred(const void* A, int lda, const void* Bt, int ldb, void* C, int ldc, int M, int N, int K, const EpiBnReduce* red,
                                   int* red_done, void* workspace, size_t workspace_bytes, epi_stream_t stream) {
    if (!red_done) return EPI_ERR_INVALID_ARGUMENT;
    GemmArgs a = {};
    a.A = (const unsigned short*)A; a.Bt = (const unsigned short*)Bt; a.C = C;
    a.M = M; a.N = N; a.K = K; a.lda = lda; a.ldb = ldb; a.ldc = ldc;
    a.br = bnred_args(red);
    return launch_gemm(a, false, 1, workspace, workspace_bytes, (hipStream_t)stream, nullptr, red_done);
}

extern "C" int epi_gemm_bf16(const void* A, int lda, const void* Bt, int ldb, void* C, int ldc, int c_dtype, int M, int N, int K,
                             const float* bias, void* workspace, size_t workspace_bytes, epi_stream_t stream) {
    GemmArgs a = {};
    a.A = (const unsigned short*)A; a.Bt = (const unsigned short*)Bt; a.C = C; a.bias = bias;
    a.M = M; a.N = N; a.K = K; a.lda = lda; a.ldb = ldb; a.ldc = ldc;
    if (c_dtype != EPI_BF16 && c_dtype != EPI_F32) return EPI_ERR_UNSUPPORTED;
    return launch_gemm(a, c_dtype == EPI_F32, 1, workspace, workspace_bytes, (hipStream_t)stream);
}

extern "C" int epi_deconv4x4s2_fwd(const void* x, const void* w_phase, void* y, int B, int H, int W, int Cin, int Cout,
                                   void* workspace, size_t workspace_bytes, epi_stream_t stream) {
    return epi_deconv4x4s2_fwd_stats(x, w_phase, y, B, H, W, Cin, Cout, nullptr, nullptr, workspace, workspace_bytes, stream);
}

static int deconv4x4s2_fwd_impl(const void* x, const void* w_phase, void* y, int B, int H, int W, int Cin, int Cout, float* bn_sums,
                               int* stats_done, void* workspace, size_t workspace_bytes, epi_stream_t stream, bool out_f32) {
    if (stats_done) *stats_done = 0;
    if (!x || !w_phase || !y || B <= 0 || H <= 0 || W <= 0 || Cin <= 0 || Cout <= 0) return EPI_ERR_INVALID_ARGUMENT;
    if (Cin % GBK || Cout % 4) return EPI_ERR_UNSUPPORTED;
    GemmArgs a = {};
    a.A = (const unsigned short*)x; a.Bt = (const unsigned short*)w_phase; a.C = y;
    a.M = B * H * W; a.N = Cout; a.K = 4 * Cin; a.lda = 0; a.ldb = 4 * Cin; a.ldc = Cout;
    a.ga.enabled = 1; a.ga.Hg = H; a.ga.Wg = W; a.ga.Hs = H; a.ga.Ws = W; a.ga.Cs = Cin; a.ga.stride = 1;
    a.sc.enabled = 1; a.sc.Hg = H; a.sc.Wg = W; a.sc.Ho = 2 * H; a.sc.Wo = 2 * W; a.sc.so = 2;
    a.ph.enabled = 1;
    for (int phase = 0; phase < 4; ++phase) {
        a.ph.ntap[phase] = 4;
        a.ph.bt_off[phase] = (long long)phase * Cout * 4 * Cin;
        for (int t = 0; t < 4; ++t) { a.ph.dy[phase][t] = (phase >> 1) - (t >> 1); a.ph.dx[phase][t] = (phase & 1) - (t & 1); }
    }
    a.stats = out_f32 ? nullptr : bn_sums;
    a.stats_copies = epi_bn_sum_copies(Cout);
    return launch_gemm(a, out_f32, 4, workspace, workspace_bytes, (hipStream_t)stream, stats_done);
}
extern "C" int epi_deconv4x4s2_fwd_stats(const void* x, const void* w_phase, void* y, int B, int H, int W, int Cin, int Cout, float* bn_sums,
                                         int* stats_done, void* workspace, size_t workspace_bytes, epi_stream_t stream) {
    return deconv4x4s2_fwd_impl(x, w_phase, y, B, H, W, Cin, Cout, bn_sums, stats_done, workspace, workspace_bytes, stream, false);
}
extern "C" int epi_deconv4x4s2_fwd_f32(const void* x, const void* w_phase, void* y, int B, int H, int W, int Cin, int Cout,
                                       void* workspace, size_t workspace_bytes, epi_stream_t stream) {
    return deconv4x4s2_fwd_impl(x, w_phase, y, B, H, W, Cin, Cout, nullptr, nullptr, workspace, workspace_bytes, stream, true);
}

static int deconv4x4s2_bwd_data_impl(const void* dy, const void* w_bwd, void* dx, int B, int H, int W, int Cin, int Cout,
                                    void* workspace, size_t workspace_bytes, epi_stream_t stream, bool out_f32,
                                    const EpiBnReduce* red = nullptr, int* red_done = nullptr) {
    if (red_done) *red_done = 0;
    if (!dy || !w_bwd || !dx || B <= 0 || H <= 0 || W <= 0 || Cin <= 0 || Cout <= 0) return EPI_ERR_INVALID_ARGUMENT;
    if (Cout % GBK || Cin % 4) return EPI_ERR_UNSUPPORTED;
    GemmArgs a = {};
    a.A = (const unsigned short*)dy; a.Bt = (const unsigned short*)w_bwd; a.C = dx;
    a.M = B * H * W; a.N = Cin; a.K = 16 * Cout; a.lda = 0; a.ldb = 16 * Cout; a.ldc = Cin;
    a.ga.enabled = 1; a.ga.Hg = H; a.ga.Wg = W; a.ga.Hs = 2 * H; a.ga.Ws = 2 * W; a.ga.Cs = Cout; a.ga.stride = 2;
    for (int kh = 0; kh < 4; ++kh)
        for (int kw = 0; kw < 4; ++kw) { a.ga.dy[4 * kh + kw] = kh - 1; a.ga.dx[4 * kh + kw] = kw - 1; }
    a.br = bnred_args(red);
    return launch_gemm(a, out_f32, 1, workspace, workspace_bytes, (hipStream_t)stream, nullptr, red_done);
}
extern "C" int epi_deconv4x4s2_bwd_data(const void* dy, const void* w_bwd, void* dx, int B, int H, int W, int Cin, int Cout,
                                        void* workspace, size_t workspace_bytes, epi_stream_t stream) {
    return deconv4x4s2_bwd_data_impl(dy, w_bwd, dx, B, H, W, Cin, Cout, workspace, workspace_bytes, stream, false);
}
extern "C" int epi_deconv4x4s2_bwd_data_bnred(const void* dy, const void* w_bwd, void* dx, int B, int H, int W, int Cin, int Cout,
                                              const EpiBnReduce* red, int* red_done, void* workspace, size_t workspace_bytes, epi_stream_t stream) {
    if (!red_done) return EPI_ERR_INVALID_ARGUMENT;
    return deconv4x4s2_bwd_data_impl(dy, w_bwd, dx, B, H, W, Cin, Cout, workspace, workspace_bytes, stream, false, red, red_done);
}
extern "C" int epi_deconv4x4s2_bwd_data_f32(const void* dy, const void* w_bwd, void* dx, int B, int H, int W, int Cin, int Cout,
                                            void* workspace, size_t workspace_bytes, epi_stream_t stream) {
    return deconv4x4s2_bwd_data_impl(dy, w_bwd, dx, B, H, W, Cin, Cout, workspace, workspace_bytes, stream, true);
}

namespace epi {
__global__ void pack_deconv_weight_kernel(const unsigned short* __restrict__ w, int Cin, int Cout,
                                          unsigned short* __restrict__ w_phase, unsigned short* __restrict__ w_bwd) {
    const long long t = (long long)blockIdx.x * blockDim.x + threadIdx.x;
    const long long total = (long long)Cin * Cout * 16;
    if (t >= total) return;
    const int kw = (int)(t & 3), kh = (int)((t >> 2) & 3);
    const long long r = t >> 4;
    const int co = (int)(r % Cout), ci = (int)(r / Cout);
    const unsigned short v = w[t];
    if (w_bwd) w_bwd[(long long)ci * 16 * Cout + (kh * 4 + kw) * Cout + co] = v;
    if (w_phase) {
        const int ph = (kh & 1) ? 0 : 1, ty = ph ? (kh == 0 ? 0 : 1) : (kh == 1 ? 0 : 1);
        const int pw = (kw & 1) ? 0 : 1, tx = pw ? (kw == 0 ? 0 : 1) : (kw == 1 ? 0 : 1);
        w_phase[((long long)(2 * ph + pw) * Cout + co) * 4 * Cin + (2 * ty + tx) * Cin + ci] = v;
    }
}
}

extern "C" int epi_deconv4x4s2_pack_weight(const void* w_bf16, int Cin, int Cout, void* w_phase, void* w_bwd, epi_stream_t stream) {
    if (!w_bf16 || Cin <= 0 || Cout <= 0 || (!w_phase && !w_bwd)) return EPI_ERR_INVALID_ARGUMENT;
    const long long total = (long long)Cin * Cout * 16;
    hipLaunchKernelGGL(epi::pack_deconv_weight_kernel, dim3((unsigned)((total + 255) / 256)), dim3(256), 0, (hipStream_t)stream,
                       (const unsigned short*)w_bf16, Cin, Cout, (unsigned short*)w_phase, (unsigned short*)w_bwd);
    EPI_CHECK_LAUNCH();
    return EPI_OK;
}

namespace epi {

typedef short s16x4 __attribute__((ext_vector_type(4)));

struct GemmTnArgs {
    const unsigned short* A;
    const unsigned short* B;
    void* C;
    int R, I, J, lda, ldb;
    int rows_per_split, nsplit;
    int out_bf16;
    int gather;
    int Hg, Wg, Hs, Ws, Cs;
    int stride, pad, KW;
    const float* b_bn;
};

template <int TI_, int WJ_> struct TnCfg {
    static constexpr int TI = TI_, WJ = WJ_, NW = 2 * WJ_, THREADS = 64 * NW;
    static constexpr int BI = 2 * TI_ * 32, BJ = WJ_ * 64;
    static constexpr int A_ROWB = BI * 2, B_ROWB = BJ * 2;
    static constexpr int A_BYTES = GBK * A_ROWB, B_BYTES = GBK * B_ROWB, STAGE_BYTES = A_BYTES + B_BYTES;
    static constexpr int A_PIECES = A_BYTES / 1024 / NW, B_PIECES = B_BYTES / 1024 / NW;
    static constexpr int WG_PER_CU = (2 * STAGE_BYTES <= 49152) ? 3 : (2 * STAGE_BYTES <= 65536 ? 2 : 1);
    static_assert(A_PIECES >= 1 && B_PIECES >= 1 && A_PIECES <= 4 && B_PIECES <= 4, "pieces per wave");
};
typedef TnCfg<2, 2> TnSmall;
typedef TnCfg<1, 2> TnNarrow;
typedef TnCfg<4, 4> TnBig;

template <int ROWB> __device__ __forceinline__ int tn_swz(int row) { return ROWB >= 256 ? 4 * (row & 3) : 4 * ((row >> 1) & 1); }

template <int ROWB>
__device__ __forceinline__ bf16x8 tr_frag(const char* tile, int row0, int col, int lane_c) {
    const int row = row0 + (lane_c >> 2);
    const int chunk = (col >> 3) + ((lane_c & 3) >> 1);
    const char* p = tile + row * ROWB + ((chunk ^ tn_swz<ROWB>(row)) << 4) + 8 * (lane_c & 1);
    struct { s16x4 lo, hi; } v;
    v.lo = __builtin_amdgcn_ds_read_tr16_b64_v4i16((__attribute__((address_space(3))) s16x4*)(p));
    v.hi = __builtin_amdgcn_ds_read_tr16_b64_v4i16((__attribute__((address_space(3))) s16x4*)(p + 4 * ROWB));
    return __builtin_bit_cast(bf16x8, v);
}

__device__ __forceinline__ bf16x8 tn_bn_apply(bf16x8 b, float sc, float sh) {
    const uint4v u = __builtin_bit_cast(uint4v, b);
    const unsigned int w[4] = {u.x, u.y, u.z, u.w};
    unsigned int o[4];
#pragma unroll
    for (int k = 0; k < 4; ++k) {
        const float lo = __uint_as_float(w[k] << 16), hi = __uint_as_float(w[k] & 0xffff0000u);
        o[k] = pack_bf16x2(fmaxf(lo * sc + sh, 0.f), fmaxf(hi * sc + sh, 0.f));
    }
    uint4v r; r.x = o[0]; r.y = o[1]; r.z = o[2]; r.w = o[3];
    return __builtin_bit_cast(bf16x8, r);
}

template <typename Cfg, bool GATHER, bool BNB = false>
__device__ __forceinline__ void tn_body(const GemmTnArgs& p, const int tile_id, const int split, char* smem) {
    static_assert(!(GATHER && BNB), "BatchNorm on the B operand: plain rows only");
    constexpr int TI = Cfg::TI, BI = Cfg::BI, BJ = Cfg::BJ, AP = Cfg::A_PIECES, BP = Cfg::B_PIECES;
    const int tid = threadIdx.x, lane = tid & 63, wid = tid >> 6;
    const int wm = wid / Cfg::WJ, wn = wid % Cfg::WJ;
    const int tiles_j = (p.J + BJ - 1) / BJ;
    const int tile_i = tile_id / tiles_j, tile_j = tile_id - tile_i * tiles_j;
    const int i0 = tile_i * BI, j0 = tile_j * BJ;
    const int r_begin = split * p.rows_per_split;
    const int r_end = min(p.R, r_begin + p.rows_per_split);
    const char* zero_src = reinterpret_cast<const char*>(epi_zero_chunk);

    constexpr int A_CH = Cfg::A_ROWB / 16, A_RPP = 1024 / Cfg::A_ROWB, B_CH = Cfg::B_ROWB / 16, B_RPP = 1024 / Cfg::B_ROWB;
    int a_row[AP], b_row[BP];
    const unsigned short* a_src[AP];
    bool a_colok[AP], b_colok[BP];
    const unsigned short* b_src[BP];
    int b_n[BP];
#pragma unroll
    for (int q = 0; q < AP; ++q) {
        a_row[q] = (wid * AP + q) * A_RPP + lane / A_CH;
        const int col = i0 + (((lane % A_CH) ^ tn_swz<Cfg::A_ROWB>(a_row[q])) << 3);
        a_colok[q] = col < p.I;
        a_src[q] = p.A + (long long)(r_begin + a_row[q]) * p.lda + col;
    }
    const int adv_w = GATHER ? GBK % p.Wg : 0, adv_h = GATHER ? (GBK / p.Wg) % p.Hg : 0, adv_n = GATHER ? GBK / (p.Wg * p.Hg) : 0;
    int b_ih[BP], b_iw[BP], b_sy[BP], b_sx[BP];
#pragma unroll
    for (int q = 0; q < BP; ++q) {
        b_row[q] = (wid * BP + q) * B_RPP + lane / B_CH;
        const int col = j0 + (((lane % B_CH) ^ tn_swz<Cfg::B_ROWB>(b_row[q])) << 3);
        b_colok[q] = col < p.J;
        if (GATHER) {
            const int tap = col / p.Cs, c = col - tap * p.Cs;
            const int kh = tap / p.KW, kw = tap - kh * p.KW;
            b_sy[q] = kh - p.pad;
            b_sx[q] = kw - p.pad;
            const int r = r_begin + b_row[q], hw = p.Hg * p.Wg;
            b_n[q] = r / hw;
            const int rem = r - b_n[q] * hw;
            b_ih[q] = rem / p.Wg;
            b_iw[q] = rem - b_ih[q] * p.Wg;
            b_src[q] = p.B + c;
        } else {
            b_src[q] = p.B + (long long)(r_begin + b_row[q]) * p.ldb + col;
            b_n[q] = b_ih[q] = b_iw[q] = b_sy[q] = b_sx[q] = 0;
        }
    }
    auto issue_tile_piece_a = [&](int q, int r0, int buf) {
        char* a_s = smem + buf * Cfg::STAGE_BYTES + __builtin_amdgcn_readfirstlane(wid) * (AP * 1024);
        const bool ok = a_colok[q] && r0 + a_row[q] < r_end;
        const unsigned short* src = a_src[q] + (long long)(r0 - r_begin) * p.lda;
        glds16(ok ? reinterpret_cast<const void*>(src) : reinterpret_cast<const void*>(zero_src), a_s + q * 1024);
    };
    auto issue_tile_piece_b = [&](int q, int r0, int buf) {
        char* b_s = smem + buf * Cfg::STAGE_BYTES + Cfg::A_BYTES + __builtin_amdgcn_readfirstlane(wid) * (BP * 1024);
        bool ok = b_colok[q] && r0 + b_row[q] < r_end;
        const unsigned short* src;
        if (GATHER) {
            const int y = b_ih[q] * p.stride + b_sy[q], x = b_iw[q] * p.stride + b_sx[q];
            ok = ok && (unsigned)y < (unsigned)p.Hs && (unsigned)x < (unsigned)p.Ws;
            const unsigned pix = (unsigned)((b_n[q] * p.Hs + y) * p.Ws + x);
            src = b_src[q] + pix * (unsigned)p.ldb;
            b_iw[q] += adv_w;
            if (b_iw[q] >= p.Wg) { b_iw[q] -= p.Wg; b_ih[q] += 1; }
            b_ih[q] += adv_h;
            if (b_ih[q] >= p.Hg) { b_ih[q] -= p.Hg; b_n[q] += 1; }
            b_n[q] += adv_n;
        } else {
// ... 1006 lines not shown
```

### epipolarpose_amd/hip.py

```python
import ctypes
import os

import torch

_LIB_DIR = os.environ.get("EPI_LIB_DIR") or os.path.join(os.path.dirname(os.path.abspath(__file__)), "_lib")
_LIB_PATH = os.path.join(_LIB_DIR, "libepipolar_hip.so")
_lib = None

EPI_F32, EPI_BF16, EPI_F64 = 0, 1, 2
EPI_NCHW, EPI_NHWC = 0, 1
LOSS_KINDS = {"l1": 0, "l2": 1, "smoothl1": 2}
TRI_METHODS = {"iterative": 0, "ls": 1, "dlt": 2, "poly": 3}

_vp, _i, _d, _sz = ctypes.c_void_p, ctypes.c_int, ctypes.c_double, ctypes.c_size_t


class EpiViewMeta(ctypes.Structure):
    _fields_ = [(k, _vp) for k in ("center_x", "center_y", "width", "height", "scale", "rot", "R", "T", "f", "c", "P")]


_SIGNATURES = {
    "epi_version": (ctypes.c_char_p, []),
    "epi_status_string": (ctypes.c_char_p, [_i]),
    "epi_softargmax3d_workspace_bytes": (_sz, [_i] * 5),
    "epi_softargmax3d_fwd": (_i, [_vp, _i, _i, _i, _i, _i, _i, _i, _vp, _vp, _vp, _vp, _sz, _vp]),
    "epi_softargmax3d_bwd": (_i, [_vp, _i, _i, _i, _i, _i, _i, _i, _vp, _vp, _vp, _vp, _vp, _vp, _vp]),
    "epi_softargmax3d_bwd_colsums": (_i, [_vp, _i, _i, _i, _i, _i, _i, _i, _vp, _vp, _vp, _vp, _vp, _vp, _vp, ctypes.POINTER(ctypes.c_int), _vp]),
    "epi_joint_loss": (_i, [_vp, _vp, _vp, _i, _i, _i, _i, _i, _vp, _vp, _vp]),
    "epi_argmax_workspace_bytes": (_sz, [_i, _i]),
    "epi_argmax_rows": (_i, [_vp, _i, _i, _i, _vp, _vp, _vp, _sz, _vp]),
    "epi_decode_to_image": (_i, [_vp, _i, _i, ctypes.POINTER(EpiViewMeta), _d, _d, _d, _vp, _vp]),
    "epi_triangulate_iterls": (_i, [_vp, _i, _vp, _i, _i, _i, _i, _d, _i, _vp, _vp, _vp]),
    "epi_triangulate_ls": (_i, [_vp, _i, _vp, _i, _i, _i, _i, _vp, _vp, _vp]),
    "epi_triangulate_dlt": (_i, [_vp, _i, _vp, _i, _i, _i, _i, _vp, _vp, _vp]),
    "epi_triangulate_poly": (_i, [_vp, _i, _vp, _i, _i, _i, _i, _vp, _vp, _vp]),
    "epi_triangulate_staged": (_i, [_i]),
    "epi_fundamental_8point": (_i, [_vp, _vp, _i, _i, _vp, _vp, _vp]),
    "epi_fundamental_lmeds_medians": (_i, [_vp, _i, _vp, _vp, _i, _vp, _vp]),
    "epi_fundamental_errors": (_i, [_vp, _vp, _vp, _i, _vp, _vp]),
    "epi_correct_matches": (_i, [_vp, _vp, _vp, _i, _i, _vp, _vp, _vp]),
    "epi_reproject_labels": (_i, [_vp, _i, _i, _i, ctypes.POINTER(EpiViewMeta), _d, _d, _d, _i, _vp, _vp, _vp]),
    "epi_self_supervision": (_i, [_vp, _i, _i, _i, ctypes.POINTER(EpiViewMeta), _d, _d, _d, _i, _i, _d, _i, _vp, _vp, _vp, _vp]),
    "epi_gemm_workspace_bytes": (_sz, [_i, _i, _i, _i]),
    "epi_gemm_bf16": (_i, [_vp, _i, _vp, _i, _vp, _i, _i, _i, _i, _i, _vp, _vp, _sz, _vp]),
    "epi_deconv4x4s2_pack_weight": (_i, [_vp, _i, _i, _vp, _vp, _vp]),
    "epi_deconv4x4s2_fwd": (_i, [_vp, _vp, _vp, _i, _i, _i, _i, _i, _vp, _sz, _vp]),
    "epi_deconv4x4s2_fwd_stats": (_i, [_vp, _vp, _vp, _i, _i, _i, _i, _i, _vp, _vp, _vp, _sz, _vp]),
    "epi_deconv4x4s2_bwd_data": (_i, [_vp, _vp, _vp, _i, _i, _i, _i, _i, _vp, _sz, _vp]),
    "epi_conv2d_workspace_bytes": (_sz, [_i] * 9),
    "epi_conv2d_fwd": (_i, [_vp, _vp, _vp, _i, _i, _i, _i, _i, _i, _i, _i, _i, _vp, _vp, _vp, _sz, _vp]),
    "epi_conv1x1_fwd_bn_in": (_i, [_vp, _vp, _i, ctypes.c_float, ctypes.c_float, _vp, _vp, _i, _i, _i, _i, _i, _vp, _vp, _vp, _sz, _vp]),
    "epi_conv2d_pack_weight_bwd": (_i, [_vp, _i, _i, _i, _i, _i, _i, _vp, _vp]),
    "epi_conv2d_pack_row_bytes": (_sz, []),
    "epi_conv2d_pack_fill_row": (_i, [_vp, _vp, _vp, _i, _i, _i, _i, _i, _i, ctypes.c_longlong, ctypes.POINTER(ctypes.c_longlong)]),
    "epi_conv2d_pack_weight_bwd_multi": (_i, [_vp, _i, ctypes.c_longlong, _vp]),
    "epi_conv2d_bwd_data": (_i, [_vp, _vp, _vp, _i, _i, _i, _i, _i, _i, _i, _i, _i, _vp, _vp, _sz, _vp]),
    "epi_conv2d_bwd_data_bnred": (_i, [_vp, _vp, _vp, _i, _i, _i, _i, _i, _i, _i, _i, _i, _vp, _i, _vp, _vp, _vp, _sz, _vp]),
    "epi_conv2d_bwd_data_half_addend_ok": (_i, [_i, _i, _i, _i, _i]),
    "epi_deconv4x4s2_bwd_data_bnred": (_i, [_vp, _vp, _vp, _i, _i, _i, _i, _i, _vp, _vp, _vp, _sz, _vp]),
    "epi_gemm_bf16_bnred": (_i, [_vp, _i, _vp, _i, _vp, _i, _i, _i, _i, _vp, _vp, _vp, _sz, _vp]),
    "epi_bn_finalize": (_i, [_vp, ctypes.c_longlong, _i, ctypes.c_float, ctypes.c_float, _i, _vp]),
    "epi_maxpool3x3s2_bn_relu_fwd": (_i, [_vp, _vp, _vp, _vp, _i, _i, _i, _i, _vp]),
    "epi_bn_act_fwd_dual": (_i, [_vp, _vp, ctypes.c_longlong, _i, _vp, _vp, ctypes.c_float, ctypes.c_float, _i, _vp, _vp]),
    "epi_bn_act_bwd_reduced": (_i, [_vp, _vp, ctypes.c_longlong, _i, _vp, _vp, _vp, _vp, _vp, _vp, _vp, _vp, _vp]),
    "epi_conv2d_bwd_weight": (_i, [_vp, _vp, _vp, _i, _i, _i, _i, _i, _i, _i, _i, _i, _i, _vp, ctypes.c_size_t, _vp]),
    "epi_conv2d_bwd_weight_deferred": (_i, [_vp, _vp, _vp, _i, _i, _i, _i, _i, _i, _i, _i, _i, _i, _vp, ctypes.c_size_t, _vp, _vp]),
    "epi_slab_reduce_chunks": (ctypes.c_longlong, [ctypes.c_longlong]),
    "epi_slab_reduce_multi": (_i, [_vp, _i, ctypes.c_longlong, _vp]),
    "epi_wgrad_group_max": (_i, []),
    "epi_wgrad_group_plan": (_i, [_vp, _i, ctypes.POINTER(ctypes.c_size_t), ctypes.POINTER(ctypes.c_int)]),
    "epi_wgrad_group": (_i, [_vp, _i, _vp, _sz, _vp, _vp]),
    "epi_wgrad_item": (_i, [_vp, _vp, _sz, _vp, _vp]),
    "epi_bn_sum_copies": (_i, [_i]),
    "epi_conv3x3_patch_mode": (_i, [_i]),
    "epi_gemm_tune": (_i, [_i, _i]),
    "epi_gemm_store_policy": (_i, [_i]),
    "epi_set_deterministic": (_i, [_i]),
    "epi_bn_act_fwd": (_i, [_vp, _vp, ctypes.c_longlong, _i, _vp, _vp, ctypes.c_float, ctypes.c_float, _i, _i, _vp, _vp, _vp, _vp,
                            _vp, _vp, _vp, _vp, _vp, _vp]),
    "epi_bn_act_bwd": (_i, [_vp, _vp, _vp, ctypes.c_longlong, _i, _vp, _vp, _vp, _vp, _i, _vp, _vp, _vp, _vp, _vp, _vp]),
    "epi_gemm_tn_workspace_bytes": (_sz, [_i, _i, _i, _i]),
    "epi_gemm_tn_plan": (_i, [_i, _i, _i, _i, ctypes.POINTER(ctypes.c_longlong)]),
    "epi_gemm_tn_bf16": (_i, [_vp, _i, _vp, _i, _vp, _i, _i, _i, _vp, _sz, _vp]),
    "epi_deconv4x4s2_bwd_weight": (_i, [_vp, _vp, _vp, _i, _i, _i, _i, _i, _i, _vp, _sz, _vp]),
    "epi_deconv4x4s2_pack_phase_cl": (_i, [_vp, _i, _i, _vp, _vp]),
    "epi_deconv4x4s2_pack_fill_row": (_i, [_vp, _vp, _vp, _i, _i, ctypes.c_longlong, ctypes.POINTER(ctypes.c_longlong)]),
    "epi_column_sums_bf16": (_i, [_vp, ctypes.c_longlong, _i, _vp, _vp]),
    "epi_stem7x7s2_s2d_bytes": (_sz, [_i, _i, _i]),
    "epi_stem7x7s2_workspace_bytes": (_sz, [_i, _i, _i, _i]),
    "epi_stem7x7s2_s2d": (_i, [_vp, _i, _i, _i, _i, _i, _vp, _vp]),
    "epi_stem7x7s2_pack_weight": (_i, [_vp, _i, _i, _vp, _vp]),
    "epi_stem7x7s2_unpack_weight_grad": (_i, [_vp, _i, _i, _vp, _i, _vp]),
    "epi_stem7x7s2_fwd": (_i, [_vp, _vp, _vp, _i, _i, _i, _i, _vp, _vp, _vp, _sz, _vp]),
    "epi_stem7x7s2_bwd_weight": (_i, [_vp, _vp, _vp, _i, _i, _i, _i, _vp, _sz, _vp]),
    "epi_split_bf16": (_i, [_vp, ctypes.c_longlong, _i, _vp, _i, _i, _vp, _vp]),
    "epi_conv2d_fwd_f32": (_i, [_vp, _vp, _vp, _i, _i, _i, _i, _i, _i, _i, _i, _i, _vp, _sz, _vp]),
    "epi_conv2d_bwd_data_f32": (_i, [_vp, _vp, _vp, _i, _i, _i, _i, _i, _i, _i, _i, _i, _vp, _sz, _vp]),
    "epi_deconv4x4s2_fwd_f32": (_i, [_vp, _vp, _vp, _i, _i, _i, _i, _i, _vp, _sz, _vp]),
    "epi_deconv4x4s2_bwd_data_f32": (_i, [_vp, _vp, _vp, _i, _i, _i, _i, _i, _vp, _sz, _vp]),
    "epi_bn_act_fwd_f32": (_i, [_vp, _vp, ctypes.c_longlong, _i, _vp, _vp, ctypes.c_float, ctypes.c_float, _i, _i, _vp, _vp, _vp, _vp,
                                _vp, _vp, _vp, _vp, _vp, _vp]),
    "epi_bn_act_bwd_f32": (_i, [_vp, _vp, _vp, ctypes.c_longlong, _i, _vp, _vp, _vp, _vp, _i, _vp, _vp, _vp, _vp, _vp, _vp]),
    "epi_column_sums_f32": (_i, [_vp, ctypes.c_longlong, _i, _vp, _vp]),
    "epi_maxpool3x3s2_fwd_f32": (_i, [_vp, _vp, _vp, _i, _i, _i, _i, _vp]),
    "epi_maxpool3x3s2_bwd_f32": (_i, [_vp, _vp, _vp, _i, _i, _i, _i, _vp]),
    "epi_adam_tensor_bytes": (_sz, []),
    "epi_adam_chunk_elems": (_i, []),
    "epi_adam_step": (_i, [_vp, _vp, _i, ctypes.c_float, ctypes.c_float, ctypes.c_float, ctypes.c_float, ctypes.c_longlong, _vp]),
    "epi_adam_step_clipped": (_i, [_vp, _vp, _i, ctypes.c_float, ctypes.c_float, ctypes.c_float, ctypes.c_float, ctypes.c_longlong,
                                   ctypes.c_float, _vp, _vp]),
    "epi_dropout_bf16": (_i, [_vp, _vp, ctypes.c_longlong, ctypes.c_float, ctypes.c_ulonglong, _vp]),
    "epi_maxpool3x3s2_fwd": (_i, [_vp, _vp, _vp, _i, _i, _i, _i, _vp]),
    "epi_maxpool3x3s2_bwd": (_i, [_vp, _vp, _vp, _i, _i, _i, _i, _vp]),
    "epi_crop_patches": (_i, [_vp, _vp, _vp, _vp, _vp, _vp, ctypes.POINTER(ctypes.c_float), ctypes.POINTER(ctypes.c_float), _i, _i, _i, _vp,
                              _i, _i, _vp]),
    "epi_crop_patches_occluded": (_i, [_vp, _vp, _vp, _vp, _vp, _vp, ctypes.POINTER(ctypes.c_float), ctypes.POINTER(ctypes.c_float), _i, _i, _i, _vp,
                                       _vp, _vp, _vp, _i, _vp, _i, _i, _vp]),
    "epi_evaluate_poses": (_i, [_vp, _vp, _vp, _vp, _vp, _i, _i, _i, _vp, _i, _vp, _vp, _vp]),
}
EXPORTED_SYMBOLS = tuple(_SIGNATURES)


def lib_path():
    return _LIB_PATH


class _Library:

    def __init__(self, cdll, path, missing):
        self.__dict__.update(_cdll=cdll, _path=path, _missing=frozenset(missing))

    def __getattr__(self, name):
        if name in self._missing:
            raise RuntimeError("%s (loaded through EPI_LIB_DIR) does not export %s: that build predates the entry point -- "
                               "this code path cannot be part of an A/B run against it" % (self._path, name))
        return getattr(self._cdll, name)


def load():
    global _lib
    if _lib is None:
        if not os.path.exists(_LIB_PATH):
            raise RuntimeError("libepipolar_hip.so not found at %s -- build it with `python -m epipolarpose_amd.build` "
                               "(there is no CPU fallback)" % _LIB_PATH)
        lib = ctypes.CDLL(_LIB_PATH)
        missing = []
        for name, (res, args) in _SIGNATURES.items():
            fn = getattr(lib, name, None)
            if fn is None:
                if os.environ.get("EPI_LIB_DIR"):
                    missing.append(name)
                    continue
                raise RuntimeError("%s does not export %s: stale build -- run `python -m epipolarpose_amd.build`" % (_LIB_PATH, name))
            fn.restype = res
            fn.argtypes = args
        _lib = _Library(lib, _LIB_PATH, missing)
    return _lib


class KernelTimer:

    def __init__(self):
        self.enabled = False
        self.records = {}

    def reset(self):
        self.records = {}

    def start(self, name):
        if not self.enabled:
            return None
        ev = (torch.cuda.Event(enable_timing=True), torch.cuda.Event(enable_timing=True))
        ev[0].record()
        self.records.setdefault(name, []).append(ev)
        return ev

    @staticmethod
    def stop(ev):
        if ev is not None:
            ev[1].record()

    def summary(self):
        return {k: (len(v), sum(a.elapsed_time(b) for a, b in v) / len(v)) for k, v in self.records.items()}


timer = KernelTimer()


def _check(status, what):
    if status != 0:
        raise RuntimeError("%s failed: %s" % (what, load().epi_status_string(status).decode()))


_raw_stream = getattr(torch._C, "_cuda_getCurrentRawStream", None)


def _stream(device_index=None):
    if _raw_stream is not None:
        return _raw_stream(torch.cuda.current_device() if device_index is None else device_index)
    return torch.cuda.current_stream().cuda_stream


class _NoCtx:

    def __enter__(self):
        return self

    def __exit__(self, *a):
        return False


_NOCTX = _NoCtx()


def _on(device):
    return _NOCTX


def _dev(t, dtype=None, name="tensor"):
    if not t.is_cuda:
        raise RuntimeError("%s must live on the GPU (no CPU fallback in epipolarpose_amd)" % name)
    if dtype is not None and t.dtype != dtype:
        raise TypeError("%s must be %s, got %s" % (name, dtype, t.dtype))
    return t


def _ptr(t):
    return t.data_ptr() if t is not None else None


def _logits_format(logits):
    if logits.dim() != 4:
        raise ValueError("logits must be [B, J*D, H, W]")
    if logits.dtype == torch.float32:
        dt = EPI_F32
    elif logits.dtype == torch.bfloat16:
        dt = EPI_BF16
    else:
        raise TypeError("logits must be float32 or bfloat16, got %s" % logits.dtype)
    if logits.is_contiguous():
        return dt, EPI_NCHW, logits
    if logits.is_contiguous(memory_format=torch.channels_last):
        return dt, EPI_NHWC, logits
    return dt, EPI_NCHW, logits.contiguous()


_workspaces = {}


def _workspace(nbytes, device):
    key = (device.index, torch.cuda.current_stream(device).cuda_stream)
    ws = _workspaces.get(key)
    if ws is None or ws.numel() < nbytes:
        ws = torch.empty(max(int(nbytes), 1 << 16), dtype=torch.uint8, device=device)
        _workspaces[key] = ws
    return ws


def softargmax3d_fwd(logits, num_joints):
    lib = load()
    _dev(logits, name="logits")
    dt, layout, logits = _logits_format(logits)
    b, c, h, w = logits.shape
    if c % num_joints:
        raise ValueError("channels %d not divisible by num_joints %d" % (c, num_joints))
    d = c // num_joints
    xyz = torch.empty((b, 3 * num_joints), dtype=torch.float32, device=logits.device)
    rmax = torch.empty((b * num_joints,), dtype=torch.float32, device=logits.device)
    rsum = torch.empty_like(rmax)
    nbytes = lib.epi_softargmax3d_workspace_bytes(b, num_joints, d, h, w)
    ws = _workspace(nbytes, logits.device)
    with _on(logits.device):
        ev = timer.start("epi_softargmax3d_fwd")
        _check(lib.epi_softargmax3d_fwd(_ptr(logits), dt, layout, b, num_joints, d, h, w, _ptr(xyz), _ptr(rmax), _ptr(rsum),
                                        _ptr(ws), ws.numel(), _stream()), "epi_softargmax3d_fwd")
        timer.stop(ev)
    return xyz, rmax, rsum


def softargmax3d_bwd(logits, num_joints, row_max, row_sum, xyz, grad_xyz, grad_scale=None, col_sums=None):
    lib = load()
    _dev(logits, name="logits")
    dt, layout, logits = _logits_format(logits)
    b, c, h, w = logits.shape
    d = c // num_joints
    grad_xyz = _dev(grad_xyz, torch.float32, "grad_xyz").contiguous()
    dlogits = torch.empty_like(logits)
    with _on(logits.device):
        ev = timer.start("epi_softargmax3d_bwd")
        if col_sums is not None:
            if col_sums.dtype != torch.float32 or col_sums.numel() != c or not col_sums.is_contiguous() or col_sums.device != logits.device:
                raise ValueError("col_sums must be a contiguous float32 [C] tensor on the logits' device")
            done = ctypes.c_int(0)
            _check(lib.epi_softargmax3d_bwd_colsums(_ptr(logits), dt, layout, b, num_joints, d, h, w, _ptr(row_max), _ptr(row_sum), _ptr(xyz),
                                                    _ptr(grad_xyz), _ptr(grad_scale), _ptr(dlogits), _ptr(col_sums), ctypes.byref(done), _stream()),
                   "epi_softargmax3d_bwd_colsums")
            timer.stop(ev)
            return dlogits, bool(done.value)
        _check(lib.epi_softargmax3d_bwd(_ptr(logits), dt, layout, b, num_joints, d, h, w, _ptr(row_max), _ptr(row_sum),
                                        _ptr(xyz), _ptr(grad_xyz), _ptr(grad_scale), _ptr(dlogits), _stream()),
               "epi_softargmax3d_bwd")
        timer.stop(ev)
    return dlogits


def joint_loss(pred, target, weight, kind, norm=False, size_average=True, need_grad=True):
    lib = load()
    pred = _dev(pred, torch.float32, "pred").contiguous()
    target = _dev(target, name="target").to(torch.float32).contiguous()
    weight = _dev(weight, name="weight").to(torch.float32).contiguous()
    if pred.shape != target.shape or pred.shape != weight.shape or pred.dim() != 2:
        raise ValueError("pred/target/weight must share a [B, n] shape")
    b, n = pred.shape
    loss = torch.empty((), dtype=torch.float32, device=pred.device)
    grad = torch.empty_like(pred) if need_grad else None
    with _on(pred.device):
        _check(lib.epi_joint_loss(_ptr(pred), _ptr(target), _ptr(weight), b, n, LOSS_KINDS[kind], int(bool(norm)),
                                  int(bool(size_average)), _ptr(loss), _ptr(grad), _stream()), "epi_joint_loss")
    return loss, grad


def argmax_rows(x):
    lib = load()
    _dev(x, name="x")
    x = x.contiguous()
    dt = EPI_F32 if x.dtype == torch.float32 else EPI_BF16 if x.dtype == torch.bfloat16 else None
    if dt is None:
        raise TypeError("argmax_rows: float32 or bfloat16 only")
    rows, n = x.shape
    idx = torch.empty((rows,), dtype=torch.int64, device=x.device)
    val = torch.empty((rows,), dtype=torch.float32, device=x.device)
    nbytes = lib.epi_argmax_workspace_bytes(rows, n)
    ws = _workspace(nbytes, x.device)
    with _on(x.device):
        _check(lib.epi_argmax_rows(_ptr(x), dt, rows, n, _ptr(idx), _ptr(val), _ptr(ws), ws.numel(), _stream()),
               "epi_argmax_rows")
    return idx, val


class DeviceMeta:

    KEYS = ("center_x", "center_y", "width", "height", "scale", "rot", "R", "T", "f", "c", "projection_matrix")
    FIELDS = (("center_x", "center_x"), ("center_y", "center_y"), ("width", "width"), ("height", "height"), ("scale", "scale"),
              ("rot", "rot"), ("R", "R"), ("T", "T"), ("f", "f"), ("c", "c"), ("P", "projection_matrix"))

    def __init__(self, meta, device):
        self.tensors = {}
        host = []
        for k in self.KEYS:
            if k not in meta:
                continue
            v = meta[k]
            t = v if isinstance(v, torch.Tensor) else torch.as_tensor(v)
            if t.is_cuda:
                self.tensors[k] = t.to(device=device, dtype=torch.float64).contiguous()
            else:
                host.append((k, t))
        if host:
            total = sum(t.numel() for _, t in host)
            stage = torch.empty(total, dtype=torch.float64)
            if torch.cuda.is_available():
                stage = stage.pin_memory()
            off = 0
            for _, t in host:
                stage[off:off + t.numel()].copy_(t.reshape(-1))
                off += t.numel()
            dev = stage.to(device=device, non_blocking=True)
            self._stage = stage
            off = 0
            for k, t in host:
                self.tensors[k] = dev[off:off + t.numel()].view(t.shape)
                off += t.numel()
        self.batch = int(self.tensors["center_x"].shape[0])
        s = EpiViewMeta()
        for field, key in self.FIELDS:
            setattr(s, field, self.tensors[key].data_ptr() if key in self.tensors else None)
        self.struct = s
# ... 126 lines not shown

def _nhwc_bf16(t, name):
    _dev(t, torch.bfloat16, name)
    if t.dim() != 4:
        raise ValueError("%s must be [B, C, H, W]" % name)
    return t if t.is_contiguous(memory_format=torch.channels_last) else t.contiguous(memory_format=torch.channels_last)


def gemm_bf16(a, bt, bias=None, out_dtype=torch.bfloat16, out=None):
    lib = load()
    _dev(a, torch.bfloat16, "a")
    _dev(bt, torch.bfloat16, "bt")
    if a.stride(1) != 1:
        a = a.contiguous()
    if bt.stride(1) != 1:
        bt = bt.contiguous()
    m, k = a.shape
    n = bt.shape[0]
    if bt.shape[1] != k:
        raise ValueError("inner dimensions differ")
    if out is None:
        out = torch.empty((m, n), dtype=out_dtype, device=a.device)
    cdt = EPI_BF16 if out.dtype == torch.bfloat16 else EPI_F32
    if bias is not None:
        bias = _dev(bias, torch.float32, "bias").contiguous()
    ws = _workspace(lib.epi_gemm_workspace_bytes(m, n, k, 1), a.device)
    with _on(a.device):
        ev = timer.start("epi_gemm_bf16")
        _check(lib.epi_gemm_bf16(_ptr(a), a.stride(0), _ptr(bt), bt.stride(0), _ptr(out), out.stride(0), cdt, m, n, k,
                                 _ptr(bias), _ptr(ws), ws.numel(), _stream()), "epi_gemm_bf16")
        timer.stop(ev)
    return out


def deconv_pack_weight(weight, want_phase=True, want_bwd=True):
    lib = load()
    _dev(weight, name="weight")
    cin, cout, kh, kw = weight.shape
    if (kh, kw) != (4, 4):
        raise ValueError("deconv head kernels cover kernel 4 / stride 2 / padding 1 only")
    w = weight.detach().to(torch.bfloat16).contiguous()
    wp = torch.empty((4, cout, 4 * cin), dtype=torch.bfloat16, device=w.device) if want_phase else None
    wb = torch.empty((cin, 16 * cout), dtype=torch.bfloat16, device=w.device) if want_bwd else None
    with _on(w.device):
        _check(lib.epi_deconv4x4s2_pack_weight(_ptr(w), cin, cout, _ptr(wp), _ptr(wb), _stream()), "epi_deconv4x4s2_pack_weight")
    return wp, wb


def deconv_weight_forms(weight, w_phase=None):
    lib = load()
    _dev(weight, name="weight")
    cin, cout, kh, kw = weight.shape
    if (kh, kw) != (4, 4):
        raise ValueError("deconv head kernels cover kernel 4 / stride 2 / padding 1 only")
    w = weight.detach()
    if w.dtype != torch.bfloat16:
        w = w.to(torch.bfloat16)
    if not w.is_contiguous(memory_format=torch.channels_last):
        w = w.contiguous(memory_format=torch.channels_last)
    if w_phase is None:
        w_phase = torch.empty((4, cout, 4 * cin), dtype=torch.bfloat16, device=w.device)
        _check(lib.epi_deconv4x4s2_pack_phase_cl(_ptr(w), cin, cout, _ptr(w_phase), _stream()), "epi_deconv4x4s2_pack_phase_cl")
    return w_phase, w


def deconv4x4s2_fwd(x, w_phase, bn_sums=None):
    lib = load()
    x = _nhwc_bf16(x, "x")
    b, cin, h, w = x.shape
    cout = w_phase.shape[1]
    y = torch.empty((b, cout, 2 * h, 2 * w), dtype=torch.bfloat16, device=x.device, memory_format=torch.channels_last)
    ws = _workspace(lib.epi_gemm_workspace_bytes(b * h * w, cout, 4 * cin, 4), x.device)
    with _on(x.device):
        ev = timer.start("epi_deconv4x4s2_fwd")
        done = ctypes.c_int(0)
        _check(lib.epi_deconv4x4s2_fwd_stats(_ptr(x), _ptr(w_phase), _ptr(y), b, h, w, cin, cout, _ptr(bn_sums),
                                             ctypes.addressof(done) if bn_sums is not None else None, _ptr(ws), ws.numel(), _stream()),
               "epi_deconv4x4s2_fwd")
        timer.stop(ev)
    return y if bn_sums is None else (y, bool(done.value))


def deconv4x4s2_bwd_data(dy, w_bwd):
    lib = load()
    dy = _nhwc_bf16(dy, "dy")
    b, cout, h2, w2 = dy.shape
    cin = w_bwd.shape[0]
    dx = torch.empty((b, cin, h2 // 2, w2 // 2), dtype=torch.bfloat16, device=dy.device, memory_format=torch.channels_last)
    ws = _workspace(lib.epi_gemm_workspace_bytes(b * (h2 // 2) * (w2 // 2), cin, 16 * cout, 1), dy.device)
    with _on(dy.device):
        ev = timer.start("epi_deconv4x4s2_bwd_data")
        _check(lib.epi_deconv4x4s2_bwd_data(_ptr(dy), _ptr(w_bwd), _ptr(dx), b, h2 // 2, w2 // 2, cin, cout, _ptr(ws), ws.numel(),
                                            _stream()), "epi_deconv4x4s2_bwd_data")
        timer.stop(ev)
    return dx


_glue = None


def glue():
    global _glue
    if _glue is None:
        import importlib.util
        from . import build as _build
        load()
        path = os.path.join(_LIB_DIR, os.path.basename(_build.glue_path()))
        if not os.path.exists(path):
            raise RuntimeError("epipolarpose_amd: %s is missing -- run `python -m epipolarpose_amd.build` (hipcc + g++, gfx950); "
                               "there is no Python/CPU fallback for the fused BatchNorm" % path)
        spec = importlib.util.spec_from_file_location(_build.GLUE_NAME, path)
        mod = importlib.util.module_from_spec(spec)
        spec.loader.exec_module(mod)
        ver = load().epi_version().decode()
        if mod.abi_version() != ver:
            raise RuntimeError("epipolarpose_amd: glue / library version mismatch (%s vs %s): rebuild" % (mod.abi_version(), ver))
        _glue = mod
    return _glue


def gemm_tn_plan(r, i, j, ntap=1):
    plan = (ctypes.c_longlong * 4)()
    _check(load().epi_gemm_tn_plan(r, i, j, ntap, plan), "epi_gemm_tn_plan")
    return {"cfg": int(plan[0]), "tiles": int(plan[1]), "nsplit": int(plan[2]), "rows_per_split": int(plan[3]),
            "slab_bytes": int(plan[2]) * i * j * ntap * 4 if plan[2] > 1 else 0}


def gemm_tn_bf16(a, b):
    lib = load()
    _dev(a, torch.bfloat16, "a")
    _dev(b, torch.bfloat16, "b")
    if a.stride(1) != 1:
        a = a.contiguous()
    if b.stride(1) != 1:
        b = b.contiguous()
    r, i = a.shape
    j = b.shape[1]
    out = torch.empty((i, j), dtype=torch.float32, device=a.device)
    ws = _workspace(lib.epi_gemm_tn_workspace_bytes(r, i, j, 1), a.device)
    with _on(a.device):
        ev = timer.start("epi_gemm_tn_bf16")
        _check(lib.epi_gemm_tn_bf16(_ptr(a), a.stride(0), _ptr(b), b.stride(0), _ptr(out), r, i, j, _ptr(ws), ws.numel(), _stream()),
               "epi_gemm_tn_bf16")
        timer.stop(ev)
    return out


def deconv4x4s2_bwd_weight(x, dy, dtype=torch.float32):
    lib = load()
    x, dy = _nhwc_bf16(x, "x"), _nhwc_bf16(dy, "dy")
    b, cin, h, w = x.shape
    cout = dy.shape[1]
    taps = torch.empty((cin, 16, cout), dtype=dtype, device=x.device)
    ws = _workspace(lib.epi_gemm_tn_workspace_bytes(b * h * w, cin, cout, 16), x.device)
    with _on(x.device):
        ev = timer.start("epi_deconv4x4s2_bwd_weight")
        _check(lib.epi_deconv4x4s2_bwd_weight(_ptr(x), _ptr(dy), _ptr(taps), EPI_BF16 if dtype == torch.bfloat16 else EPI_F32, b, h, w, cin, cout,
                                              _ptr(ws), ws.numel(), _stream()), "epi_deconv4x4s2_bwd_weight")
        timer.stop(ev)
    return taps.view(cin, 4, 4, cout).permute(0, 3, 1, 2)


def conv2d_bwd_weight(x, dy, kernel, stride=1, padding=0, dtype=torch.float32):
    lib = load()
    x, dy = _nhwc_bf16(x, "x"), _nhwc_bf16(dy, "dy")
    b, cin, h, w = x.shape
    cout = dy.shape[1]
    kh, kw = (kernel, kernel) if isinstance(kernel, int) else kernel
    ho, wo = (h + 2 * padding - kh) // stride + 1, (w + 2 * padding - kw) // stride + 1
    if tuple(dy.shape) != (b, cout, ho, wo):
        raise ValueError("dy shape %s does not match the convolution geometry %s" % (tuple(dy.shape), (b, cout, ho, wo)))
    dw = torch.empty((cout, cin, kh, kw), dtype=dtype, device=x.device).contiguous(memory_format=torch.channels_last)
    ws = _workspace(lib.epi_gemm_tn_workspace_bytes(b * ho * wo, cout, cin, kh * kw), x.device)
    with _on(x.device):
        _check(lib.epi_conv2d_bwd_weight(_ptr(x), _ptr(dy), _ptr(dw), EPI_BF16 if dtype == torch.bfloat16 else EPI_F32, b, h, w, cin, cout,
                                         kh, kw, stride, padding, _ptr(ws), ws.numel(), _stream()), "epi_conv2d_bwd_weight")
    return dw


class EpiWgradItem(ctypes.Structure):
    _fields_ = ([("x", _vp), ("dy", _vp), ("dw", _vp)] + [(k, _i) for k in ("dw_dtype", "kind", "B", "H", "W", "Cin", "Cout", "KH", "KW", "stride", "pad")]
                + [("x_scale_shift", _vp)])


class EpiBnReduce(ctypes.Structure):
    _fields_ = [("z", _vp), ("y", _vp), ("bn", _vp), ("sums", _vp), ("relu", _i)]


class EpiSlabReduce(ctypes.Structure):
    _fields_ = [("slabs", _vp), ("out", _vp), ("n", ctypes.c_longlong), ("chunk_begin", ctypes.c_longlong), ("nsplit", _i), ("out_bf16", _i)]


def wgrad_group_max():
    return int(load().epi_wgrad_group_max())


def wgrad_group_plan(shapes):
    n = len(shapes)
    items = (EpiWgradItem * n)()
    for it, (kind, b, h, w, cin, cout, k, stride, pad) in zip(items, shapes):
        it.dw_dtype, it.kind = EPI_BF16, 1 if kind == "deconv" else 0
        it.B, it.H, it.W, it.Cin, it.Cout, it.KH, it.KW, it.stride, it.pad = b, h, w, cin, cout, k, k, stride, pad
    slab = ctypes.c_size_t(0)
    ns = (ctypes.c_int * n)()
    _check(load().epi_wgrad_group_plan(items, n, ctypes.byref(slab), ns), "epi_wgrad_group_plan")
    return int(slab.value), list(ns)


def wgrad_group(jobs, dtype=torch.float32):
    lib = load()
    n = len(jobs)
    items = (EpiWgradItem * n)()
    outs, keep = [], []
    for it, (kind, x, dy, k, stride, pad) in zip(items, jobs):
        x, dy = _nhwc_bf16(x, "x"), _nhwc_bf16(dy, "dy")
        keep += [x, dy]
        b, cin, h, w = x.shape
        cout = dy.shape[1]
        if kind == "deconv":
            dw = torch.empty((cin, 16, cout), dtype=dtype, device=x.device)
            outs.append(dw.view(cin, 4, 4, cout).permute(0, 3, 1, 2))
            it.kind = 1
        else:
            dw = torch.empty((cout, cin, k, k), dtype=dtype, device=x.device).contiguous(memory_format=torch.channels_last)
            outs.append(dw)
            it.kind = 0
        keep.append(dw)
        it.x, it.dy, it.dw = _ptr(x), _ptr(dy), _ptr(dw)
        it.dw_dtype = EPI_BF16 if dtype == torch.bfloat16 else EPI_F32
        it.B, it.H, it.W, it.Cin, it.Cout, it.KH, it.KW, it.stride, it.pad = b, h, w, cin, cout, k, k, stride, pad
    dev = keep[0].device
    slab = ctypes.c_size_t(0)
    _check(lib.epi_wgrad_group_plan(items, n, ctypes.byref(slab), None), "epi_wgrad_group_plan")
    ws = torch.empty(max(int(slab.value), 256), dtype=torch.uint8, device=dev)
    pend = (EpiSlabReduce * n)()
    with _on(dev):
        _check(lib.epi_wgrad_group(items, n, _ptr(ws), ws.numel(), pend, _stream()), "epi_wgrad_group")
        rows = [p for p in pend if p.nsplit > 0]
        if rows:
            table = (EpiSlabReduce * len(rows))()
            chunks = 0
            for dst, src in zip(table, rows):
                ctypes.memmove(ctypes.byref(dst), ctypes.byref(src), ctypes.sizeof(EpiSlabReduce))
                dst.chunk_begin = chunks
                chunks += int(lib.epi_slab_reduce_chunks(src.n))
            raw = torch.frombuffer(bytearray(bytes(table)), dtype=torch.uint8).to(dev)
            _check(lib.epi_slab_reduce_multi(_ptr(raw), len(rows), chunks, _stream()), "epi_slab_reduce_multi")
            keep.append(raw)
        torch.cuda.current_stream(dev).synchronize()
    return outs


def stem_conv_fwd(x, weight, bn_sums=None):
    lib = load()
    _dev(x, name="x")
    b, _, h, w = x.shape
    cout = weight.shape[0]
    nhwc = x.is_contiguous(memory_format=torch.channels_last)
    if not nhwc:
        x = x.contiguous()
    w16 = weight.detach().to(torch.bfloat16)
    w_cl = w16.is_contiguous(memory_format=torch.channels_last) and not w16.is_contiguous()
    if not w_cl:
        w16 = w16.contiguous()
    s2d = torch.empty(lib.epi_stem7x7s2_s2d_bytes(b, h, w) // 2, dtype=torch.bfloat16, device=x.device)
    wp = torch.empty(cout * 256, dtype=torch.bfloat16, device=x.device)
    y = torch.empty((b, cout, h // 2, w // 2), dtype=torch.bfloat16, device=x.device, memory_format=torch.channels_last)
    ws = _workspace(lib.epi_stem7x7s2_workspace_bytes(b, h, w, cout), x.device)
    done = ctypes.c_int(0)
    _check(lib.epi_stem7x7s2_s2d(_ptr(x), EPI_F32 if x.dtype == torch.float32 else EPI_BF16, EPI_NHWC if nhwc else EPI_NCHW, b, h, w, _ptr(s2d), _stream()),
           "epi_stem7x7s2_s2d")
    _check(lib.epi_stem7x7s2_pack_weight(_ptr(w16), 1 if w_cl else 0, cout, _ptr(wp), _stream()), "epi_stem7x7s2_pack_weight")
    _check(lib.epi_stem7x7s2_fwd(_ptr(s2d), _ptr(wp), _ptr(y), b, h, w, cout, _ptr(bn_sums), ctypes.addressof(done) if bn_sums is not None else None,
                                 _ptr(ws), ws.numel(), _stream()), "epi_stem7x7s2_fwd")
    return y, s2d


def stem_conv_bwd_weight(s2d, dy, image_hw, dtype=torch.float32):
    lib = load()
    dy = _nhwc_bf16(dy, "dy")
    b, cout = dy.shape[0], dy.shape[1]
    h, w = image_hw
    dwp = torch.empty(cout * 256, dtype=torch.float32, device=dy.device)
    dw = torch.empty((cout, 3, 7, 7), dtype=dtype, device=dy.device)
    ws = _workspace(lib.epi_stem7x7s2_workspace_bytes(b, h, w, cout), dy.device)
    _check(lib.epi_stem7x7s2_bwd_weight(_ptr(s2d), _ptr(dy), _ptr(dwp), b, h, w, cout, _ptr(ws), ws.numel(), _stream()), "epi_stem7x7s2_bwd_weight")
    _check(lib.epi_stem7x7s2_unpack_weight_grad(_ptr(dwp), cout, 0, _ptr(dw), EPI_BF16 if dtype == torch.bfloat16 else EPI_F32, _stream()),
           "epi_stem7x7s2_unpack_weight_grad")
    return dw


def _cl_weight_bf16(weight):
    _dev(weight, name="weight")
    w = weight.detach()
    if w.dtype != torch.bfloat16:
        w = w.to(torch.bfloat16)
    return w if w.is_contiguous(memory_format=torch.channels_last) else w.contiguous(memory_format=torch.channels_last)


def conv3x3_patch_mode(mode=-1):
    return int(load().epi_conv3x3_patch_mode(int(mode)))


def set_deterministic(on=True):
    before = int(load().epi_set_deterministic(1 if on else 0))
    if before < 0:
        raise RuntimeError("epi_set_deterministic: could not allocate the partial-sum scratch")
    return bool(before)


def is_deterministic():
    return bool(load().epi_set_deterministic(-1))


def bn_sum_copies(channels):
    return 4 if channels <= 512 else 1


def conv2d_fwd(x, weight, stride=1, padding=0, bn_sums=None):
    lib = load()
    x = _nhwc_bf16(x, "x")
    w = _cl_weight_bf16(weight)
    b, cin, h, wd = x.shape
    cout, _, kh, kw = w.shape
    ho, wo = (h + 2 * padding - kh) // stride + 1, (wd + 2 * padding - kw) // stride + 1
    y = torch.empty((b, cout, ho, wo), dtype=torch.bfloat16, device=x.device, memory_format=torch.channels_last)
    ws = _workspace(lib.epi_conv2d_workspace_bytes(b, h, wd, cin, cout, kh, kw, stride, padding), x.device)
    ev = timer.start("epi_conv2d_fwd")
    done = ctypes.c_int(0)
    _check(lib.epi_conv2d_fwd(_ptr(x), _ptr(w), _ptr(y), b, h, wd, cin, cout, kh, kw, stride, padding, _ptr(bn_sums),
                              ctypes.addressof(done) if bn_sums is not None else None, _ptr(ws), ws.numel(), _stream()), "epi_conv2d_fwd")
    timer.stop(ev)
    return y if bn_sums is None else (y, bool(done.value))


def conv2d_pack_weight_bwd(weight, stride=1, padding=0, out=None):
    lib = load()
    w = _cl_weight_bf16(weight)
    cout, cin, kh, kw = w.shape
    if out is None:
        out = torch.empty(w.numel(), dtype=torch.bfloat16, device=w.device)
    _check(lib.epi_conv2d_pack_weight_bwd(_ptr(w), cout, cin, kh, kw, stride, padding, _ptr(out), _stream()), "epi_conv2d_pack_weight_bwd")
    return out


def conv2d_bwd_data_bnred(dy, w_bwd, in_shape, kernel, stride, padding, z, bn, relu=True, y=None, addend=None, addend_step=1):
    lib = load()
    dy = _nhwc_bf16(dy, "dy")
    z = _nhwc_bf16(z, "z")
    b, cin, h, wd = in_shape
    cout = dy.shape[1]
    kh, kw = (kernel, kernel) if isinstance(kernel, int) else kernel
    if tuple(z.shape) != (b, cin, h, wd) or tuple(bn.shape) != (4, cin) or bn.dtype != torch.float32 or not bn.is_contiguous():
        raise ValueError("z must have the shape of dx and bn must be f32 [4, Cin]")
    dx = torch.empty((b, cin, h, wd), dtype=torch.bfloat16, device=dy.device, memory_format=torch.channels_last)
    sums = torch.zeros(2, cin, dtype=torch.float32, device=dy.device)
    ws = _workspace(lib.epi_conv2d_workspace_bytes(b, h, wd, cin, cout, kh, kw, stride, padding), dy.device)
    if addend is not None:
        addend = _nhwc_bf16(addend, "addend")
    if y is not None:
        y = _nhwc_bf16(y, "y")
    red = EpiBnReduce(_ptr(z), _ptr(y), _ptr(bn), _ptr(sums), 1 if relu else 0)
    done = ctypes.c_int(0)
    with _on(dy.device):
        _check(lib.epi_conv2d_bwd_data_bnred(_ptr(dy), _ptr(w_bwd), _ptr(dx), b, h, wd, cin, cout, kh, kw, stride, padding, _ptr(addend), addend_step,
                                             ctypes.byref(red), ctypes.byref(done), _ptr(ws), ws.numel(), _stream()), "epi_conv2d_bwd_data_bnred")
    return dx, sums, bool(done.value)


def conv2d_bwd_data(dy, w_bwd, in_shape, kernel, stride=1, padding=0, addend=None):
    lib = load()
    dy = _nhwc_bf16(dy, "dy")
    b, cin, h, wd = in_shape
    cout = dy.shape[1]
    kh, kw = (kernel, kernel) if isinstance(kernel, int) else kernel
    dx = torch.empty((b, cin, h, wd), dtype=torch.bfloat16, device=dy.device, memory_format=torch.channels_last)
    ws = _workspace(lib.epi_conv2d_workspace_bytes(b, h, wd, cin, cout, kh, kw, stride, padding), dy.device)
    ev = timer.start("epi_conv2d_bwd_data")
    if addend is not None:
        addend = _nhwc_bf16(addend, "addend")
        if tuple(addend.shape) != tuple(dx.shape):
            raise ValueError("addend must have the shape of dx")
    _check(lib.epi_conv2d_bwd_data(_ptr(dy), _ptr(w_bwd), _ptr(dx), b, h, wd, cin, cout, kh, kw, stride, padding, _ptr(addend), _ptr(ws),
                                   ws.numel(), _stream()), "epi_conv2d_bwd_data")
    timer.stop(ev)
    return dx


def column_sum_bf16(x):
    lib = load()
    _dev(x, torch.bfloat16, "x")
    x = x if x.is_contiguous() else x.contiguous()
    r, c = x.shape
    sums = torch.zeros(2 * c, dtype=torch.float32, device=x.device)
    with _on(x.device):
        _check(lib.epi_column_sums_bf16(_ptr(x), r, c, _ptr(sums), _stream()), "epi_column_sums_bf16")
    return sums[:c]


def adam_step(table_dev, chunks_dev, nchunks, lr, beta1, beta2, eps, step):
    lib = load()
    ev = timer.start("epi_adam_step")
    _check(lib.epi_adam_step(_ptr(table_dev), _ptr(chunks_dev), nchunks, lr, beta1, beta2, eps, step, _stream()), "epi_adam_step")
    timer.stop(ev)


def adam_step_clipped(table_dev, chunks_dev, nchunks, lr, beta1, beta2, eps, step, max_norm, norm_sq):
    lib = load()
    _check(lib.epi_adam_step_clipped(_ptr(table_dev), _ptr(chunks_dev), nchunks, lr, beta1, beta2, eps, step, max_norm, _ptr(norm_sq),
                                     _stream()), "epi_adam_step_clipped")


def dropout_bf16(x, p, seed, out=None):
    lib = load()
    _dev(x, torch.bfloat16, "x")
    x = x.contiguous()
    out = torch.empty_like(x) if out is None else out
    _check(lib.epi_dropout_bf16(_ptr(x), _ptr(out), x.numel(), float(p), int(seed) & 0xFFFFFFFFFFFFFFFF, _stream()), "epi_dropout_bf16")
    return out


def maxpool3x3s2_fwd(x):
    lib = load()
    x = _nhwc_bf16(x, "x")
    b, c, h, w = x.shape
    ho, wo = (h - 1) // 2 + 1, (w - 1) // 2 + 1
    y = torch.empty((b, c, ho, wo), dtype=torch.bfloat16, device=x.device, memory_format=torch.channels_last)
    pos = torch.empty((b, ho, wo, c), dtype=torch.uint8, device=x.device)
    with _on(x.device):
        _check(lib.epi_maxpool3x3s2_fwd(_ptr(x), _ptr(y), _ptr(pos), b, h, w, c, _stream()), "epi_maxpool3x3s2_fwd")
    return y, pos


def maxpool3x3s2_bwd(dy, pos, in_hw):
    lib = load()
    dy = _nhwc_bf16(dy, "dy")
    _dev(pos, torch.uint8, "pos")
    b, c = dy.shape[0], dy.shape[1]
    h, w = in_hw
    dx = torch.empty((b, c, h, w), dtype=torch.bfloat16, device=dy.device, memory_format=torch.channels_last)
    with _on(dy.device):
        _check(lib.epi_maxpool3x3s2_bwd(_ptr(dy), _ptr(pos), _ptr(dx), b, h, w, c, _stream()), "epi_maxpool3x3s2_bwd")
    return dx


def evaluate_poses(pred_img, gt_img, pelvis_z, fl, c_p, root, j14):
    lib = load()
    for t in (pred_img, gt_img, pelvis_z, fl, c_p):
        _dev(t, torch.float64)
    pred_img, gt_img = pred_img.contiguous(), gt_img.contiguous()
    n, j, _ = pred_img.shape
    j14_t = torch.tensor(list(j14), dtype=torch.int32, device=pred_img.device)
    metrics = torch.empty((n, 9), dtype=torch.float64, device=pred_img.device)
    per_joint = torch.empty((n, j), dtype=torch.float64, device=pred_img.device)
    _check(lib.epi_evaluate_poses(_ptr(pred_img), _ptr(gt_img), _ptr(pelvis_z.contiguous()), _ptr(fl.contiguous()), _ptr(c_p.contiguous()),
                                  n, j, root, _ptr(j14_t), len(j14), _ptr(metrics), _ptr(per_joint), _stream()), "epi_evaluate_poses")
    return metrics, per_joint


def crop_patches(frames, frame_offset, frame_hw, trans, patch_h, patch_w, do_flip=None, color_scale=None, mean=None, std=None,
                 dtype=torch.float32, channels_last=False, occluders=None, placements=None):
    lib = load()
    _dev(frames, torch.uint8, "frames")
    frame_offset = _dev(frame_offset, torch.int64, "frame_offset").contiguous()
    frame_hw = _dev(frame_hw, torch.int32, "frame_hw").contiguous()
    trans = _dev(trans, torch.float64, "trans").contiguous()
    b = trans.shape[0]
    if do_flip is not None:
        do_flip = _dev(do_flip, name="do_flip").to(torch.int32).contiguous()
    if color_scale is not None:
        color_scale = _dev(color_scale, name="color_scale").to(torch.float32).contiguous()
    out = torch.empty((b, 3, patch_h, patch_w), dtype=dtype, device=frames.device,
                      memory_format=torch.channels_last if channels_last else torch.contiguous_format)
    m3 = (ctypes.c_float * 3)(*[float(v) for v in mean]) if mean is not None else None
    s3 = (ctypes.c_float * 3)(*[float(v) for v in std]) if std is not None else None
    if occluders is not None and placements is not None:
        bank, occ_off, occ_hw = occluders
        _dev(bank, torch.uint8, "occluder bank")
        occ_off = _dev(occ_off, torch.int64, "occluder offsets").contiguous()
        occ_hw = _dev(occ_hw, torch.int32, "occluder sizes").contiguous()
        placements = _dev(placements, torch.int32, "placements").contiguous()
        if placements.dim() != 3 or placements.shape[0] != b or placements.shape[2] != 5:
            raise ValueError("placements must be int32 [B, max_occ, 5]")
        _check(lib.epi_crop_patches_occluded(_ptr(frames), _ptr(frame_offset), _ptr(frame_hw), _ptr(trans), _ptr(do_flip), _ptr(color_scale), m3, s3,
                                             b, patch_h, patch_w, _ptr(bank), _ptr(occ_off), _ptr(occ_hw), _ptr(placements), placements.shape[1],
                                             _ptr(out), EPI_BF16 if dtype == torch.bfloat16 else EPI_F32,
                                             EPI_NHWC if channels_last else EPI_NCHW, _stream()), "epi_crop_patches_occluded")
        return out
    _check(lib.epi_crop_patches(_ptr(frames), _ptr(frame_offset), _ptr(frame_hw), _ptr(trans), _ptr(do_flip), _ptr(color_scale), m3, s3, b,
                                patch_h, patch_w, _ptr(out), EPI_BF16 if dtype == torch.bfloat16 else EPI_F32,
                                EPI_NHWC if channels_last else EPI_NCHW, _stream()), "epi_crop_patches")
    return out
```

### include/epipolar_hip.h

```cpp
#ifndef EPIPOLAR_HIP_H
#define EPIPOLAR_HIP_H

#include <stddef.h>
#include <stdint.h>

#ifdef __cplusplus
extern "C" {
#endif

typedef void* epi_stream_t;

enum epi_status {
    EPI_OK = 0,
    EPI_ERR_INVALID_ARGUMENT = 1,
    EPI_ERR_UNSUPPORTED = 2,
    EPI_ERR_WORKSPACE = 3,
    EPI_ERR_LAUNCH = 4
};

enum epi_dtype { EPI_F32 = 0, EPI_BF16 = 1, EPI_F64 = 2 };
enum epi_layout {
    EPI_NCHW = 0,
    EPI_NHWC = 1
};
enum epi_loss_kind { EPI_LOSS_L1 = 0, EPI_LOSS_L2 = 1, EPI_LOSS_SMOOTH_L1 = 2 };

const char* epi_version(void);
const char* epi_status_string(int status);

int epi_set_deterministic(int on);

size_t epi_softargmax3d_workspace_bytes(int B, int J, int D, int H, int W);

int epi_softargmax3d_fwd(const void* logits, int dtype, int layout, int B, int J, int D, int H, int W,
                         float* xyz, float* row_max, float* row_sum,
                         void* workspace, size_t workspace_bytes, epi_stream_t stream);

int epi_softargmax3d_bwd(const void* logits, int dtype, int layout, int B, int J, int D, int H, int W,
                         const float* row_max, const float* row_sum, const float* xyz,
                         const float* grad_xyz, const float* grad_scale,
                         void* dlogits, epi_stream_t stream);
int epi_softargmax3d_bwd_colsums(const void* logits, int dtype, int layout, int B, int J, int D, int H, int W,
                                 const float* row_max, const float* row_sum, const float* xyz,
                                 const float* grad_xyz, const float* grad_scale,
                                 void* dlogits, float* col_sums, int* col_sums_done, epi_stream_t stream);

int epi_joint_loss(const float* pred, const float* target, const float* weight, int B, int n,
                   int kind, int norm, int size_average, float* loss, float* grad_pred, epi_stream_t stream);

size_t epi_argmax_workspace_bytes(int rows, int n);
int epi_argmax_rows(const void* x, int dtype, int rows, int n, int64_t* idx, float* val,
                    void* workspace, size_t workspace_bytes, epi_stream_t stream);

typedef struct epi_view_meta {
    const double* center_x;
    const double* center_y;
    const double* width;
    const double* height;
    const double* scale;
    const double* rot;
    const double* R;
    const double* T;
    const double* f;
    const double* c;
    const double* P;
} epi_view_meta;

int epi_decode_to_image(const float* xyz, int B, int J, const epi_view_meta* meta_host,
                        double patch_w, double patch_h, double rect3d, double* kps_img, epi_stream_t stream);

int epi_triangulate_iterls(const void* kps, int kps_stride, const void* P, int dtype, int G, int V, int J,
                           double tolerance, int max_iter, void* X, int32_t* status, epi_stream_t stream);
int epi_triangulate_ls(const void* kps, int kps_stride, const void* P, int dtype, int G, int V, int J,
                       void* X, int32_t* status, epi_stream_t stream);
int epi_triangulate_dlt(const void* kps, int kps_stride, const void* P, int dtype, int G, int V, int J,
                        void* X, int32_t* status, epi_stream_t stream);
int epi_triangulate_staged(int on);

int epi_triangulate_poly(const void* kps, int kps_stride, const void* P, int dtype, int G, int V, int J,
                         void* X, int32_t* status, epi_stream_t stream);

int epi_fundamental_8point(const double* u1, const double* u2, int G, int J, double* F, int32_t* status, epi_stream_t stream);

int epi_fundamental_lmeds_medians(const double* F, int H, const double* u1, const double* u2, int N, double* medians, epi_stream_t stream);
int epi_fundamental_errors(const double* F, const double* u1, const double* u2, int N, float* err, epi_stream_t stream);

int epi_correct_matches(const double* F, const double* u1, const double* u2, int G, int J,
                        double* out1, double* out2, epi_stream_t stream);

int epi_reproject_labels(const double* X, int G, int V, int J, const epi_view_meta* meta_host,
                         double patch_w, double patch_h, double rect3d, int root_joint,
                         float* label, float* weight, epi_stream_t stream);

int epi_self_supervision(const float* xyz, int G, int V, int J, const epi_view_meta* meta_host,
                         double patch_w, double patch_h, double rect3d, int root_joint,
                         int method, double tolerance, int max_iter,
                         float* label, float* weight, double* X_out, epi_stream_t stream);


size_t epi_gemm_workspace_bytes(int M, int N, int K, int nphase);
int epi_gemm_bf16(const void* A, int lda, const void* Bt, int ldb, void* C, int ldc, int c_dtype,
                  int M, int N, int K, const float* bias, void* workspace, size_t workspace_bytes, epi_stream_t stream);

int epi_deconv4x4s2_pack_weight(const void* w_bf16, int Cin, int Cout, void* w_phase, void* w_bwd,
                                epi_stream_t stream);
int epi_deconv4x4s2_pack_phase_cl(const void* w_cl, int Cin, int Cout, void* w_phase, epi_stream_t stream);
int epi_deconv4x4s2_pack_fill_row(void* row_host, const void* w_cl, void* w_phase, int Cin, int Cout, long long tile_begin,
                                  long long* ntiles);

int epi_deconv4x4s2_fwd(const void* x, const void* w_phase, void* y, int B, int H, int W, int Cin, int Cout,
                        void* workspace, size_t workspace_bytes, epi_stream_t stream);
int epi_deconv4x4s2_fwd_stats(const void* x, const void* w_phase, void* y, int B, int H, int W, int Cin, int Cout, float* bn_sums,
                              int* stats_done, void* workspace, size_t workspace_bytes, epi_stream_t stream);

int epi_deconv4x4s2_bwd_data(const void* dy, const void* w_bwd, void* dx, int B, int H, int W, int Cin, int Cout,
                             void* workspace, size_t workspace_bytes, epi_stream_t stream);

int epi_bn_sum_copies(int C);
int epi_bn_act_fwd(const void* x, const void* residual, long long R, int C, const float* gamma, const float* beta,
                   float eps, float momentum, int training, int relu, float* running_mean, float* running_var,
                   long long* num_batches_tracked, float* mean, float* rstd, float* scale_shift, float* sums_ws,
                   float* bwd_sums, void* y, epi_stream_t stream);
int epi_bn_act_bwd(const void* dy, const void* x, const void* y, long long R, int C, const float* gamma,
                   const float* mean, const float* rstd, const float* scale_shift, int relu,
                   float* dbeta_dgamma, void* dx, void* dres, float* fwd_sums_clear, float* param_grads, epi_stream_t stream);

typedef struct EpiBnLayer {
    const float* gamma;
    const float* beta;
    float* running_mean;
    float* running_var;
    long long* num_batches_tracked;
    float* mean;
    float* rstd;
    float* scale_shift;
    float* sums_ws;
    float* bwd_sums;
} EpiBnLayer;
int epi_bn_act_fwd_dual(const void* x, const void* x_proj, long long R, int C, const EpiBnLayer* main_bn, const EpiBnLayer* proj_bn,
                        float eps, float momentum, int training, void* y, epi_stream_t stream);
int epi_bn_finalize(const EpiBnLayer* layer, long long R, int C, float eps, float momentum, int training, epi_stream_t stream);
int epi_maxpool3x3s2_bn_relu_fwd(const void* x, const float* scale_shift, void* y, void* pos, int B, int H, int W, int C, epi_stream_t stream);

typedef struct EpiBnReduce {
    const void* z;
    const void* y;
    const float* bn;
    float* sums;
    int relu;
} EpiBnReduce;
int epi_bn_act_bwd_reduced(const void* dz, const void* x, long long R, int C, const float* gamma, const float* mean, const float* rstd,
                           const float* scale_shift, const float* dbeta_dgamma, void* dx, float* fwd_sums_clear, float* param_grads,
                           epi_stream_t stream);
int epi_conv2d_bwd_data_bnred(const void* dy, const void* w_bwd, void* dx, int B, int H, int W, int Cin, int Cout, int KH, int KW,
                              int stride, int pad, const void* addend, int addend_step, const EpiBnReduce* red, int* red_done, void* workspace,
                              size_t workspace_bytes, epi_stream_t stream);
int epi_conv2d_bwd_data_half_addend_ok(int B, int H, int W, int Cin, int Cout);
int epi_deconv4x4s2_bwd_data_bnred(const void* dy, const void* w_bwd, void* dx, int B, int H, int W, int Cin, int Cout,
                                   const EpiBnReduce* red, int* red_done, void* workspace, size_t workspace_bytes, epi_stream_t stream);
int epi_gemm_bf16_bnred(const void* A, int lda, const void* Bt, int ldb, void* C, int ldc, int M, int N, int K, const EpiBnReduce* red,
                        int* red_done, void* workspace, size_t workspace_bytes, epi_stream_t stream);

size_t epi_conv2d_workspace_bytes(int B, int H, int W, int Cin, int Cout, int KH, int KW, int stride, int pad);
int epi_conv3x3_patch_mode(int mode);
int epi_gemm_tune(int tile, int pipe);
int epi_gemm_store_policy(int policy);
int epi_conv2d_fwd(const void* x, const void* w, void* y, int B, int H, int W, int Cin, int Cout, int KH, int KW,
                   int stride, int pad, float* bn_sums, int* bn_sums_done, void* workspace, size_t workspace_bytes,
                   epi_stream_t stream);
int epi_conv1x1_fwd_bn_in(const void* z, const EpiBnLayer* in_bn, int in_training, float eps, float momentum, const void* w, void* y, int B, int H, int W,
                          int Cin, int Cout, float* bn_sums, int* bn_sums_done, void* workspace, size_t workspace_bytes, epi_stream_t stream);
int epi_conv2d_pack_weight_bwd(const void* w, int Cout, int Cin, int KH, int KW, int stride, int pad, void* w_bwd,
                               epi_stream_t stream);
size_t epi_conv2d_pack_row_bytes(void);
int epi_conv2d_pack_fill_row(void* row_host, const void* w, void* w_bwd, int Cout, int Cin, int KH, int KW, int stride, int pad,
                             long long tile_begin, long long* ntiles);
int epi_conv2d_pack_weight_bwd_multi(const void* rows, int nrows, long long total_tiles, epi_stream_t stream);
int epi_conv2d_bwd_data(const void* dy, const void* w_bwd, void* dx, int B, int H, int W, int Cin, int Cout, int KH, int KW,
                        int stride, int pad, const void* addend, void* workspace, size_t workspace_bytes, epi_stream_t stream);

int epi_conv2d_bwd_weight(const void* x, const void* dy, void* dw, int dw_dtype, int B, int H, int W, int Cin, int Cout,
                          int KH, int KW, int stride, int pad, void* workspace, size_t workspace_bytes, epi_stream_t stream);
typedef struct EpiSlabReduce {
    const float* slabs;
    void* out;
    long long n;
    long long chunk_begin;
    int nsplit, out_bf16;
} EpiSlabReduce;
int epi_conv2d_bwd_weight_deferred(const void* x, const void* dy, void* dw, int dw_dtype, int B, int H, int W, int Cin, int Cout,
                                   int KH, int KW, int stride, int pad, void* workspace, size_t workspace_bytes,
                                   EpiSlabReduce* pending, epi_stream_t stream);
long long epi_slab_reduce_chunks(long long n);
int epi_slab_reduce_multi(const EpiSlabReduce* rows_dev, int nrows, long long total_chunks, epi_stream_t stream);

enum { EPI_WGRAD_CONV2D = 0, EPI_WGRAD_DECONV4X4S2 = 1 };
typedef struct EpiWgradItem {
    const void* x;
    const void* dy;
    void* dw;
    int dw_dtype, kind;
    int B, H, W, Cin, Cout, KH, KW, stride, pad;
    const float* x_scale_shift;
} EpiWgradItem;
int epi_wgrad_group_max(void);
int epi_wgrad_group_plan(const EpiWgradItem* items, int n, size_t* slab_bytes, int* nsplit);
int epi_wgrad_group(const EpiWgradItem* items, int n, void* slab_ws, size_t slab_bytes, EpiSlabReduce* pending, epi_stream_t stream);
int epi_wgrad_item(const EpiWgradItem* item, void* workspace, size_t workspace_bytes, EpiSlabReduce* pending, epi_stream_t stream);

size_t epi_gemm_tn_workspace_bytes(int R, int I, int J, int ntap);
int epi_gemm_tn_plan(int R, int I, int J, int ntap, long long* plan);
int epi_gemm_tn_bf16(const void* A, int lda, const void* B, int ldb, float* C, int R, int I, int J,
                     void* workspace, size_t workspace_bytes, epi_stream_t stream);
int epi_deconv4x4s2_bwd_weight(const void* x, const void* dy, void* dw_taps, int dw_dtype, int B, int H, int W, int Cin, int Cout,
                               void* workspace, size_t workspace_bytes, epi_stream_t stream);
int epi_column_sums_bf16(const void* x, long long R, int C, float* sums, epi_stream_t stream);

size_t epi_adam_tensor_bytes(void);
int epi_adam_chunk_elems(void);
int epi_adam_step(const void* table, const void* chunks, int nchunks, float lr, float beta1, float beta2, float eps,
                  long long step, epi_stream_t stream);
int epi_adam_step_clipped(const void* table, const void* chunks, int nchunks, float lr, float beta1, float beta2, float eps,
                          long long step, float max_norm, float* norm_sq, epi_stream_t stream);

int epi_dropout_bf16(const void* x, void* y, long long n, float p, unsigned long long seed, epi_stream_t stream);

int epi_maxpool3x3s2_fwd(const void* x, void* y, void* pos, int B, int H, int W, int C, epi_stream_t stream);
int epi_maxpool3x3s2_bwd(const void* dy, const void* pos, void* dx, int B, int H, int W, int C, epi_stream_t stream);

int epi_crop_patches(const void* frames, const long long* frame_offset, const int* frame_hw, const double* trans,
                     const int* do_flip, const float* color_scale, const float* mean_host, const float* std_host, int B,
                     int patch_h, int patch_w, void* out, int out_dtype, int out_layout, epi_stream_t stream);
int epi_crop_patches_occluded(const void* frames, const long long* frame_offset, const int* frame_hw, const double* trans,
                              const int* do_flip, const float* color_scale, const float* mean_host, const float* std_host, int B,
                              int patch_h, int patch_w, const void* occ_bank, const long long* occ_offset, const int* occ_hw,
                              const int* occ_place, int max_occ, void* out, int out_dtype, int out_layout, epi_stream_t stream);

int epi_evaluate_poses(const double* pred_img, const double* gt_img, const double* pelvis_z, const double* fl,
                       const double* c_p, int N, int J, int root, const int32_t* j14, int n14, double* metrics,
                       double* per_joint, epi_stream_t stream);

size_t epi_stem7x7s2_s2d_bytes(int B, int H, int W);
size_t epi_stem7x7s2_workspace_bytes(int B, int H, int W, int Cout);
int epi_stem7x7s2_s2d(const void* x, int x_dtype, int x_layout, int B, int H, int W, void* s2d, epi_stream_t stream);
int epi_stem7x7s2_pack_weight(const void* w_bf16, int channels_last, int Cout, void* wp, epi_stream_t stream);
int epi_stem7x7s2_unpack_weight_grad(const float* dwp, int Cout, int channels_last, void* dw, int dw_dtype, epi_stream_t stream);
int epi_stem7x7s2_fwd(const void* s2d, const void* wp, void* y, int B, int H, int W, int Cout, float* bn_sums, int* bn_sums_done,
                      void* workspace, size_t workspace_bytes, epi_stream_t stream);
int epi_stem7x7s2_bwd_weight(const void* s2d, const void* dy, float* dwp, int B, int H, int W, int Cout, void* workspace,
                             size_t workspace_bytes, epi_stream_t stream);

int epi_split_bf16(const float* x, long long rows, int C, const int* pieces, int nblk, int row_concat, void* out, epi_stream_t stream);
int epi_conv2d_fwd_f32(const void* x, const void* w, void* y, int B, int H, int W, int Cin, int Cout, int KH, int KW, int stride, int pad,
                       void* workspace, size_t workspace_bytes, epi_stream_t stream);
int epi_conv2d_bwd_data_f32(const void* dy, const void* w_bwd, void* dx, int B, int H, int W, int Cin, int Cout, int KH, int KW,
                            int stride, int pad, void* workspace, size_t workspace_bytes, epi_stream_t stream);
int epi_deconv4x4s2_fwd_f32(const void* x, const void* w_phase, void* y, int B, int H, int W, int Cin, int Cout, void* workspace,
                            size_t workspace_bytes, epi_stream_t stream);
int epi_deconv4x4s2_bwd_data_f32(const void* dy, const void* w_bwd, void* dx, int B, int H, int W, int Cin, int Cout, void* workspace,
                                 size_t workspace_bytes, epi_stream_t stream);
int epi_bn_act_fwd_f32(const void* x, const void* residual, long long R, int C, const float* gamma, const float* beta, float eps,
                       float momentum, int training, int relu, float* running_mean, float* running_var,
                       long long* num_batches_tracked, float* mean, float* rstd, float* scale_shift, float* sums_ws, float* bwd_sums,
                       void* y, epi_stream_t stream);
int epi_bn_act_bwd_f32(const void* dy, const void* x, const void* y, long long R, int C, const float* gamma, const float* mean,
                       const float* rstd, const float* scale_shift, int relu, float* dbeta_dgamma, void* dx, void* dres,
                       float* fwd_sums_clear, float* param_grads, epi_stream_t stream);
int epi_column_sums_f32(const void* x, long long R, int C, float* sums, epi_stream_t stream);
int epi_maxpool3x3s2_fwd_f32(const void* x, void* y, void* pos, int B, int H, int W, int C, epi_stream_t stream);
int epi_maxpool3x3s2_bwd_f32(const void* dy, const void* pos, void* dx, int B, int H, int W, int C, epi_stream_t stream);

#ifdef __cplusplus
}
#endif
#endif
```

Baseline: 5303 images/s.

## Add deep-step 3x3 patch conv variant processing one filter row per barrier

```diff
diff --git a/epipolarpose_amd/csrc/head_gemm.hip b/epipolarpose_amd/csrc/head_gemm.hip
--- a/epipolarpose_amd/csrc/head_gemm.hip
+++ b/epipolarpose_amd/csrc/head_gemm.hip
@@ -182,18 +182,19 @@
     GemmBnRed br;
 };
 #define EPI_ARGS_OF(p) EpiArgs{(p).C, (p).bias, (p).addend, (p).stats, (p).M, (p).N, (p).ldc, (p).stats_copies, (p).addend_step, (p).add_h, (p).add_w, (p).store_policy, (p).sc, (p).br}
-template <int TM, int WM, int WN, int THREADS, bool RED, bool RED_PREFETCH = true>
-__device__ __forceinline__ void coalesced_epilogue(const EpiArgs p, f32x16 (&acc)[TM][2], char* smem, int m0, int n0, int tile_m, int wm, int wn, int wid,
+template <int TM, int WM, int WN, int THREADS, bool RED, bool RED_PREFETCH = true, int NJ = 2>
+__device__ __forceinline__ void coalesced_epilogue(const EpiArgs p, f32x16 (&acc)[TM][NJ], char* smem, int m0, int n0, int tile_m, int wm, int wn, int wid,
                                                    int lane, int tid, int sc_oy, int sc_ox) {
-    constexpr int GBN = WN * 64, ROWS = TM * 4;
-    const int frow = lane & 31, fhalf = lane >> 5, c8 = lane & 7, r8 = lane >> 3;
-    char* mine = smem + wid * (TM * 32 * 128);
-    const int n = n0 + wn * 64 + c8 * 8;
+    static_assert(NJ == 1 || NJ == 2, "one or two 32-column blocks per wave");
+    constexpr int WCOLS = NJ * 32, GBN = WN * WCOLS, RB = WCOLS * 2, CL = WCOLS / 8, RPI = 64 / CL, ROWS = TM * 32 / RPI, SWM = 8 * NJ - 1;
+    const int frow = lane & 31, fhalf = lane >> 5, c8 = lane & (CL - 1), r8 = lane / CL;
+    char* mine = smem + wid * (TM * 32 * RB);
+    const int n = n0 + wn * WCOLS + c8 * 8;
     const int m_first = m0 + wm * (TM * 32) + r8;
     const bool col_ok = n < p.N;
     const bool scatter = p.sc.enabled != 0, has_add = p.addend != nullptr, half_add = p.addend_step == 2, nt_stores = p.store_policy == 1;
     auto row_off = [&](int it, bool& ok, auto sc_c) __attribute__((always_inline)) -> long long {
-        const int m = m_first + 8 * it;
+        const int m = m_first + RPI * it;
         ok = col_ok && m < p.M;
         if (!decltype(sc_c)::value) return (long long)m * p.ldc + n;
         const int hw = p.sc.Hg * p.sc.Wg;
@@ -221,7 +222,7 @@
             for (int it = 0; it < ROWS; ++it) {
                 bool ok;
                 const long long off = row_off(it, ok, sc_c);
-                ad[it] = ok ? addend_at(m_first + 8 * it, off) : uint4v{0u, 0u, 0u, 0u};
+                ad[it] = ok ? addend_at(m_first + RPI * it, off) : uint4v{0u, 0u, 0u, 0u};
             }
         }
         if (RED_EARLY) {
@@ -239,12 +240,12 @@
     auto park = [&](auto bias_c) __attribute__((always_inline)) {
         constexpr bool BIAS = decltype(bias_c)::value;
 #pragma unroll
-        for (int tj = 0; tj < 2; ++tj)
+        for (int tj = 0; tj < NJ; ++tj)
 #pragma unroll
             for (int q = 0; q < 4; ++q) {
                 float b[4] = {0.f, 0.f, 0.f, 0.f};
                 if (BIAS) {
-                    const int nq = n0 + wn * 64 + tj * 32 + 8 * q + 4 * fhalf;
+                    const int nq = n0 + wn * WCOLS + tj * 32 + 8 * q + 4 * fhalf;
 #pragma unroll
                     for (int e = 0; e < 4; ++e) b[e] = nq + e < p.N ? p.bias[nq + e] : 0.f;
                 }
@@ -260,7 +261,7 @@
                         t.y = pack_bf16x2(acc[ti][tj][4 * q + 2], acc[ti][tj][4 * q + 3]);
                     }
                     const int unit = tj * 8 + 2 * q + fhalf;
-                    *reinterpret_cast<uint2*>(mine + row * 128 + ((unit ^ (row & 15)) << 3)) = t;
+                    *reinterpret_cast<uint2*>(mine + row * RB + ((unit ^ (row & SWM)) << 3)) = t;
                 }
             }
     };
@@ -276,9 +277,9 @@
 #pragma unroll
         for (int it = 0; it < ROWS; ++it) {
             if (RED && !RED_EARLY && it % RED_GROUP == 0 && it) __builtin_amdgcn_sched_barrier(0);
-            const int row = it * 8 + r8, sw = row & 15;
-            const uint2 lo = *reinterpret_cast<const uint2*>(mine + row * 128 + (((2 * c8) ^ sw) << 3));
-            const uint2 hi = *reinterpret_cast<const uint2*>(mine + row * 128 + (((2 * c8 + 1) ^ sw) << 3));
+            const int row = it * RPI + r8, sw = row & SWM;
+            const uint2 lo = *reinterpret_cast<const uint2*>(mine + row * RB + (((2 * c8) ^ sw) << 3));
+            const uint2 hi = *reinterpret_cast<const uint2*>(mine + row * RB + (((2 * c8 + 1) ^ sw) << 3));
             bool ok;
             const long long off = row_off(it, ok, sc_c);
             if (!ok) continue;
@@ -292,7 +293,7 @@
                 }
             }
             uint4v o; o.x = lo.x; o.y = lo.y; o.z = hi.x; o.w = hi.y;
-            if (ADD) o = add_bf16x8(o, AD_EARLY ? ad[it] : addend_at(m_first + 8 * it, off));
+            if (ADD) o = add_bf16x8(o, AD_EARLY ? ad[it] : addend_at(m_first + RPI * it, off));
             if (RED) o = RED_EARLY ? bnred_apply(p.br, o, zpre[it], ypre[it], rcols, ssum, ssq) : bnred_row(p.br, o, off, rcols, ssum, ssq);
             uint4v* dst = reinterpret_cast<uint4v*>(reinterpret_cast<unsigned short*>(p.C) + off);
             if (nt_stores) __builtin_nontemporal_store(o, dst);
@@ -311,11 +312,11 @@
 #pragma unroll
         for (int k = 0; k < 8; ++k) {
 #pragma unroll
-            for (int o = 8; o < 64; o <<= 1) { ssum[k] += __shfl_xor(ssum[k], o, 64); ssq[k] += __shfl_xor(ssq[k], o, 64); }
-        }
-        float* st = reinterpret_cast<float*>(smem + WM * WN * (TM * 32 * 128));
-        if (lane < 8) {
-            float* row = st + wm * (2 * GBN) + wn * 64 + c8 * 8;
+            for (int o = CL; o < 64; o <<= 1) { ssum[k] += __shfl_xor(ssum[k], o, 64); ssq[k] += __shfl_xor(ssq[k], o, 64); }
+        }
+        float* st = reinterpret_cast<float*>(smem + WM * WN * (TM * 32 * RB));
+        if (lane < CL) {
+            float* row = st + wm * (2 * GBN) + wn * WCOLS + c8 * 8;
             *reinterpret_cast<float4v*>(row) = float4v{ssum[0], ssum[1], ssum[2], ssum[3]};
             *reinterpret_cast<float4v*>(row + 4) = float4v{ssum[4], ssum[5], ssum[6], ssum[7]};
             *reinterpret_cast<float4v*>(row + GBN) = float4v{ssq[0], ssq[1], ssq[2], ssq[3]};
@@ -910,31 +911,34 @@
     }
 }
 
-template <int TM_, int WM_, int WN_> struct PatchCfg {
-    static constexpr int TM = TM_, WM = WM_, WN = WN_, NW = WM_ * WN_, THREADS = 64 * NW;
-    static constexpr int BM = WM_ * TM_ * 32, BN = WN_ * 64, B_BYTES = BN * 128, BP = BN / 8 / NW;
+template <int TM_, int WM_, int WN_, int NJ_ = 2> struct PatchCfg {
+    static constexpr int TM = TM_, WM = WM_, WN = WN_, NJ = NJ_, NW = WM_ * WN_, THREADS = 64 * NW;
+    static constexpr int BM = WM_ * TM_ * 32, BN = WN_ * NJ_ * 32, B_BYTES = BN * 128, BP = BN / 8 / NW;
     static_assert(NW == 8 && BP >= 1, "8 waves");
 };
 typedef PatchCfg<2, 4, 2> PatchWide;
 typedef PatchCfg<1, 8, 1> PatchNarrow;
 typedef PatchCfg<1, 4, 2> PatchHalf;
+typedef PatchCfg<1, 4, 2, 1> PatchDeep;
 constexpr int PATCH_TAPS = 9, PATCH_APW = 8;
 
 #ifdef EPI_PATCH_TRACE
-__device__ unsigned long long epi_patch_trace[64 * 96];
+constexpr int PATCH_TRACE_SLOTS = 128;
+__device__ unsigned long long epi_patch_trace[64 * PATCH_TRACE_SLOTS];
 #define PATCH_STAMP(i)                                                                                                   \
     do {                                                                                                                 \
         const int wg_ = blockIdx.x + gridDim.x * blockIdx.y;                                                             \
-        if (lane == 0 && wid == 0 && wg_ % 16 == 0 && wg_ / 16 < 64 && (i) < 96) epi_patch_trace[(wg_ / 16) * 96 + (i)] = __builtin_amdgcn_s_memtime(); \
+        if (lane == 0 && wid == 0 && wg_ % 16 == 0 && wg_ / 16 < 64 && (i) < PATCH_TRACE_SLOTS) epi_patch_trace[(wg_ / 16) * PATCH_TRACE_SLOTS + (i)] = __builtin_amdgcn_s_memtime(); \
     } while (0)
 #else
 #define PATCH_STAMP(i) do {} while (0)
 #endif
 
-template <typename Cfg, int NB, bool SINGLE, bool RED = false>
+template <typename Cfg, int NB, bool SINGLE, bool RED = false, int TS = 1>
 __global__ __launch_bounds__(Cfg::THREADS, SINGLE ? 4 : 2) void conv_patch_kernel(GemmArgs p) {
-    constexpr int TM = Cfg::TM, GBN = Cfg::BN, BP = Cfg::BP, NW = Cfg::NW, BB = Cfg::B_BYTES;
-    constexpr int NPATCH = SINGLE ? 1 : 2, GROUP = BP + (SINGLE ? 0 : 1);
+    static_assert(TS == 1 || TS == 3, "a step is one tap or one filter row");
+    constexpr int TM = Cfg::TM, NJ = Cfg::NJ, GBN = Cfg::BN, BP = Cfg::BP, NW = Cfg::NW, BB = Cfg::B_BYTES;
+    constexpr int NPATCH = SINGLE ? 1 : 2, GROUP = TS * (BP + (SINGLE ? 0 : 1)), RING = NB * TS, AHEAD = (NB - 1) * TS;
     extern __shared__ __attribute__((aligned(16))) char smem[];
     const int tid = threadIdx.x, lane = tid & 63, wid = __builtin_amdgcn_readfirstlane(tid >> 6);
     const int wm = wid / Cfg::WN, wn = wid % Cfg::WN;
@@ -946,7 +950,7 @@
     const int W = p.ga.Wg, H = p.ga.Hg, Cs = p.ga.Cs;
     const int c_begin = split_id * p.chunks_per_split, c_end = min(Cs / GBK, c_begin + p.chunks_per_split);
     const int PB = p.patch_px * 128;
-    const int ring_off = NPATCH * PB, dummy_off = ring_off + NB * BB, zero_off = dummy_off + 1024;
+    const int ring_off = NPATCH * PB, dummy_off = ring_off + RING * BB, zero_off = dummy_off + 1024;
     PATCH_STAMP(0);
     if (tid < 32) reinterpret_cast<float*>(smem + zero_off)[tid] = 0.f;
     const char* zero_src = reinterpret_cast<const char*>(epi_zero_chunk);
@@ -982,13 +986,13 @@
     };
 
     const int frow = lane & 31, fhalf = lane >> 5;
-    const int b_frag = ring_off + lds_off(wn * 64 + frow, fhalf);
-
-    f32x16 acc[TM][2];
+    const int b_frag = ring_off + lds_off(wn * (NJ * 32) + frow, fhalf);
+
+    f32x16 acc[TM][NJ];
 #pragma unroll
     for (int i = 0; i < TM; ++i)
 #pragma unroll
-        for (int j = 0; j < 2; ++j)
+        for (int j = 0; j < NJ; ++j)
 #pragma unroll
             for (int r = 0; r < 16; ++r) acc[i][j][r] = 0.f;
 
@@ -996,8 +1000,8 @@
     if (nsteps > 0) {
 #pragma unroll
         for (int j = 0; j < PATCH_APW; ++j) issue_a(j, c_begin, 0);
-        issue_b(0, c_begin, 0, true);
-        if (NB > 2) issue_b(1, c_begin, 1, true);
+#pragma unroll
+        for (int g = 0; g < AHEAD; ++g) issue_b(g, c_begin, g, true);
     }
     __builtin_amdgcn_sched_barrier(0);
     int amask[TM], arow[TM];
@@ -1024,51 +1028,61 @@
     for (int c = c_begin; c < c_end; ++c) {
         const int pbuf = SINGLE ? 0 : (c - c_begin) & 1;
 #pragma unroll
-        for (int t = 0; t < PATCH_TAPS; ++t) {
-            {
-                int ta = t + NB - 1, ca = c;
+        for (int t0 = 0; t0 < PATCH_TAPS; t0 += TS) {
+#pragma unroll
+            for (int tt = 0; tt < TS; ++tt) {
+                int ta = t0 + tt + AHEAD, ca = c;
                 if (ta >= PATCH_TAPS) { ta -= PATCH_TAPS; ca += 1; }
-                int sa = slot + NB - 1; if (sa >= NB) sa -= NB;
+                int sa = slot + tt + AHEAD; if (sa >= RING) sa -= RING;
                 issue_b(ta, ca, sa, ca < c_end);
-                if (!SINGLE) issue_a(t, c + 1, pbuf ^ 1);
+                if (!SINGLE) issue_a(t0 + tt, c + 1, pbuf ^ 1);
             }
-            const int sh = (p.ga.dy[t] + 1) * W + p.ga.dx[t] + 1;
-            int a_addr[TM];
-#pragma unroll
-            for (int ti = 0; ti < TM; ++ti) {
-                const int pr = arow[ti] + sh;
-                const int in = pbuf * PB + pr * 128 + ((fhalf ^ ((pr >> 1) & 7)) << 4);
-                a_addr[ti] = ((amask[ti] >> t) & 1) ? in : zero_off;
+            int a_addr[TS][TM], b_addr[TS];
+#pragma unroll
+            for (int tt = 0; tt < TS; ++tt) {
+                const int t = t0 + tt;
+                const int sh = (p.ga.dy[t] + 1) * W + p.ga.dx[t] + 1;
+#pragma unroll
+                for (int ti = 0; ti < TM; ++ti) {
+                    const int pr = arow[ti] + sh;
+                    const int in = pbuf * PB + pr * 128 + ((fhalf ^ ((pr >> 1) & 7)) << 4);
+                    a_addr[tt][ti] = ((amask[ti] >> t) & 1) ? in : zero_off;
+                }
+                int st = slot + tt; if (tt && st >= RING) st -= RING;
+                b_addr[tt] = b_frag + st * BB;
             }
-            const int b_addr = b_frag + slot * BB;
-            bf16x8 af[2][TM], bfr[2][2];
-            auto read_frags = [&](int ks, bf16x8 (&a)[TM], bf16x8 (&b)[2]) {
-#pragma unroll
-                for (int ti = 0; ti < TM; ++ti) a[ti] = __builtin_bit_cast(bf16x8, *reinterpret_cast<const uint4v*>(smem + (a_addr[ti] ^ (ks << 5))));
-#pragma unroll
-                for (int tj = 0; tj < 2; ++tj) b[tj] = __builtin_bit_cast(bf16x8, *reinterpret_cast<const uint4v*>(smem + ((b_addr ^ (ks << 5)) + tj * 4096)));
+            bf16x8 af[2][TM], bfr[2][NJ];
+            auto read_frags = [&](int u, bf16x8 (&a)[TM], bf16x8 (&b)[NJ]) {
+                const int tt = u >> 2, ks = u & 3;
+#pragma unroll
+                for (int ti = 0; ti < TM; ++ti) a[ti] = __builtin_bit_cast(bf16x8, *reinterpret_cast<const uint4v*>(smem + (a_addr[tt][ti] ^ (ks << 5))));
+#pragma unroll
+                for (int tj = 0; tj < NJ; ++tj) b[tj] = __builtin_bit_cast(bf16x8, *reinterpret_cast<const uint4v*>(smem + ((b_addr[tt] ^ (ks << 5)) + tj * 4096)));
             };
             read_frags(0, af[0], bfr[0]);
 #pragma unroll
-            for (int ks = 0; ks < 4; ++ks) {
-                if (ks < 3) read_frags(ks + 1, af[(ks + 1) & 1], bfr[(ks + 1) & 1]);
+            for (int u = 0; u < 4 * TS; ++u) {
+                if (u < 4 * TS - 1) read_frags(u + 1, af[(u + 1) & 1], bfr[(u + 1) & 1]);
                 __builtin_amdgcn_sched_barrier(0);
 #pragma unroll
                 for (int ti = 0; ti < TM; ++ti)
 #pragma unroll
-                    for (int tj = 0; tj < 2; ++tj)
-                        acc[ti][tj] = __builtin_amdgcn_mfma_f32_32x32x16_bf16(bfr[ks & 1][tj], af[ks & 1][ti], acc[ti][tj], 0, 0, 0);
+                    for (int tj = 0; tj < NJ; ++tj)
+                        acc[ti][tj] = __builtin_amdgcn_mfma_f32_32x32x16_bf16(bfr[u & 1][tj], af[u & 1][ti], acc[ti][tj], 0, 0, 0);
             }
+            PATCH_STAMP(3 + 3 * step_no);
             asm volatile("s_waitcnt vmcnt(%0)" ::"n"((NB - 2) * GROUP) : "memory");
+            PATCH_STAMP(4 + 3 * step_no);
             __builtin_amdgcn_s_barrier();
-            slot = slot + 1 == NB ? 0 : slot + 1;
-            PATCH_STAMP(3 + step_no);
+            if (TS == 1) slot = slot + 1 == NB ? 0 : slot + 1;
+            else slot = slot + TS == RING ? 0 : slot + TS;
+            PATCH_STAMP(5 + 3 * step_no);
             ++step_no;
         }
     }
     asm volatile("s_waitcnt vmcnt(0) lgkmcnt(0)" ::: "memory");
     __builtin_amdgcn_s_barrier();
-    PATCH_STAMP(3 + step_no);
+    PATCH_STAMP(3 + 3 * step_no);
 
     if (gridDim.y > 1) {
         float* slab = p.slabs + (long long)split_id * p.M * p.N;
@@ -1077,10 +1091,10 @@
             const int m = m0 + arow[ti];
             if (m >= p.M) continue;
 #pragma unroll
-            for (int tj = 0; tj < 2; ++tj)
+            for (int tj = 0; tj < NJ; ++tj)
 #pragma unroll
                 for (int q = 0; q < 4; ++q) {
-                    const int n = n0 + wn * 64 + tj * 32 + 8 * q + 4 * fhalf;
+                    const int n = n0 + wn * (NJ * 32) + tj * 32 + 8 * q + 4 * fhalf;
                     if (n + 3 < p.N) {
                         float4v t; t.x = acc[ti][tj][4 * q]; t.y = acc[ti][tj][4 * q + 1]; t.z = acc[ti][tj][4 * q + 2]; t.w = acc[ti][tj][4 * q + 3];
                         *reinterpret_cast<float4v*>(slab + (long long)m * p.N + n) = t;
@@ -1089,14 +1103,14 @@
         }
 #ifdef EPI_PATCH_TRACE
         asm volatile("s_waitcnt vmcnt(0)" ::: "memory");
-        PATCH_STAMP(4 + step_no);
+        PATCH_STAMP(4 + 3 * step_no);
 #endif
         return;
     }
-    coalesced_epilogue<TM, Cfg::WM, Cfg::WN, Cfg::THREADS, RED, false>(EPI_ARGS_OF(p), acc, smem, m0, n0, tile_m, wm, wn, wid, lane, tid, 0, 0);
+    coalesced_epilogue<TM, Cfg::WM, Cfg::WN, Cfg::THREADS, RED, false, NJ>(EPI_ARGS_OF(p), acc, smem, m0, n0, tile_m, wm, wn, wid, lane, tid, 0, 0);
 #ifdef EPI_PATCH_TRACE
     asm volatile("s_waitcnt vmcnt(0)" ::: "memory");
-    PATCH_STAMP(4 + step_no);
+    PATCH_STAMP(4 + 3 * step_no);
 #endif
 }
 
@@ -1327,17 +1341,17 @@
 
 #ifdef EPI_PATCH_TRACE
 extern "C" int epi_patch_trace_read(unsigned long long* out, int clear) {
-    if (hipMemcpyFromSymbol(out, HIP_SYMBOL(epi::epi_patch_trace), sizeof(unsigned long long) * 64 * 96) != hipSuccess) return 1;
+    if (hipMemcpyFromSymbol(out, HIP_SYMBOL(epi::epi_patch_trace), sizeof(unsigned long long) * 64 * epi::PATCH_TRACE_SLOTS) != hipSuccess) return 1;
     if (clear) {
-        static unsigned long long zeros[64 * 96];
+        static unsigned long long zeros[64 * epi::PATCH_TRACE_SLOTS];
         if (hipMemcpyToSymbol(HIP_SYMBOL(epi::epi_patch_trace), zeros, sizeof(zeros)) != hipSuccess) return 1;
     }
     return 0;
 }
 #endif
 
-enum { PATCH_WIDE = 0, PATCH_NARROW = 1, PATCH_HALF = 2 };
-struct PatchPlan { bool ok; int cfg, nb, patch_px, nsplit, cps; long long tiles; size_t lds; bool single; };
+enum { PATCH_WIDE = 0, PATCH_NARROW = 1, PATCH_HALF = 2, PATCH_DEEP = 3 };
+struct PatchPlan { bool ok; int cfg, nb, ts, patch_px, nsplit, cps; long long tiles; size_t lds; bool single; };
 static int g_patch_mode = -1;
 static int patch_mode() {
     if (g_patch_mode < 0) g_patch_mode = 2;
@@ -1348,25 +1362,41 @@
     if (mode >= 0 && mode <= 2) g_patch_mode = mode;
     return before;
 }
-static PatchPlan patch_plan(int M, int N, int Cs, int W, size_t workspace_bytes) {
+static int g_patch_variant = 0, g_patch_nsplit = 0;
+extern "C" int epi_conv3x3_patch_variant(int variant, int nsplit) {
+    const int before = g_patch_variant + 16 * g_patch_nsplit;
+    if (variant >= 0 && variant <= 3) g_patch_variant = variant;
+    if (nsplit >= 0 && nsplit <= 15) g_patch_nsplit = nsplit;
+    return before;
+}
+static void patch_cfg_dims(int cfg, int& bm, int& bn, int& tm, int& wmv) {
+    bm = (cfg == PATCH_HALF || cfg == PATCH_DEEP) ? 128 : 256;
+    bn = (cfg == PATCH_NARROW || cfg == PATCH_DEEP) ? 64 : 128;
+    tm = cfg == PATCH_WIDE ? 2 : 1;
+    wmv = cfg == PATCH_NARROW ? 8 : 4;
+}
+static PatchPlan patch_plan_cfg(int cfg, int ts, int M, int N, int Cs, int W, size_t workspace_bytes) {
     PatchPlan pl = {};
     const int nchunks = Cs / GBK;
-    pl.cfg = N <= 64 ? PATCH_NARROW : PATCH_WIDE;
-    if (pl.cfg == PATCH_WIDE && (long long)((M + 255) / 256) * ((N + 127) / 128) < 200) pl.cfg = PATCH_HALF;
-    const int bm = pl.cfg == PATCH_HALF ? 128 : 256, bn = pl.cfg == PATCH_NARROW ? 64 : 128;
-    const int tm = pl.cfg == PATCH_WIDE ? 2 : 1, wmv = pl.cfg == PATCH_NARROW ? 8 : 4;
+    pl.cfg = cfg;
+    pl.ts = ts;
+    int bm, bn, tm, wmv;
+    patch_cfg_dims(cfg, bm, bn, tm, wmv);
     pl.patch_px = (bm + 2 * W + 2 + 7) / 8 * 8;
     if (pl.patch_px > 8 * 8 * PATCH_APW) return pl;
-    const size_t epi = (size_t)8 * tm * 32 * 128 + (size_t)wmv * 2 * bn * sizeof(float);
-    pl.single = pl.cfg == PATCH_NARROW && nchunks == 1;
-    for (pl.nb = 3; pl.nb >= 2; --pl.nb) {
-        pl.lds = std::max((size_t)(pl.single ? 1 : 2) * pl.patch_px * 128 + (size_t)pl.nb * bn * 128 + 1024 + 128, epi);
+    if (cfg == PATCH_DEEP && W > 16) return pl;
+    const size_t epi = (size_t)8 * tm * 32 * (bn == 64 && cfg == PATCH_DEEP ? 64 : 128) + (size_t)wmv * 2 * bn * sizeof(float);
+    pl.single = ts == 1 && cfg == PATCH_NARROW && nchunks == 1;
+    const int nb_hi = (ts == 3 && cfg == PATCH_HALF) ? 2 : 3, nb_lo = (ts == 3 && cfg == PATCH_DEEP) ? 3 : 2;
+    for (pl.nb = nb_hi; pl.nb >= nb_lo; --pl.nb) {
+        pl.lds = std::max((size_t)(pl.single ? 1 : 2) * pl.patch_px * 128 + (size_t)pl.nb * ts * bn * 128 + 1024 + 128, epi);
         if (pl.lds <= 160 * 1024) break;
     }
-    if (pl.nb < 2) return pl;
+    if (pl.nb < nb_lo) return pl;
     pl.tiles = (long long)((M + bm - 1) / bm) * ((N + bn - 1) / bn);
     pl.nsplit = 1;
-    if (pl.tiles < 120) {
+    if (g_patch_nsplit > 0) pl.nsplit = std::min(nchunks, g_patch_nsplit);
+    else if (pl.tiles < 120) {
         if (patch_mode() < 2) return pl;
         pl.nsplit = (int)std::min<long long>(nchunks, std::max<long long>(1, 256 / pl.tiles));
     }
@@ -1375,6 +1405,29 @@
     pl.nsplit = (nchunks + pl.cps - 1) / pl.cps;
     pl.ok = pl.tiles <= 0x7fffffffLL;
     return pl;
+}
+static PatchPlan patch_plan(int M, int N, int Cs, int W, size_t workspace_bytes) {
+    int cfg = N <= 64 ? PATCH_NARROW : PATCH_WIDE;
+    if (cfg == PATCH_WIDE && (long long)((M + 255) / 256) * ((N + 127) / 128) < 200) cfg = PATCH_HALF;
+    if (g_patch_variant == 2 || g_patch_variant == 3) {
+        const PatchPlan pl = patch_plan_cfg(g_patch_variant == 2 ? PATCH_HALF : PATCH_DEEP, 3, M, N, Cs, W, workspace_bytes);
+        if (pl.ok) return pl;
+    }
+    if (g_patch_variant == 0 && cfg == PATCH_HALF && W <= 16 && (long long)((M + 127) / 128) * ((N + 127) / 128) < 200) {
+        const PatchPlan pl = patch_plan_cfg(PATCH_DEEP, 3, M, N, Cs, W, workspace_bytes);
+        if (pl.ok) return pl;
+    }
+    return patch_plan_cfg(cfg, 1, M, N, Cs, W, workspace_bytes);
+}
+extern "C" int epi_conv3x3_patch_plan(int M, int N, int Cs, int W, long long* out) {
+    if (!out || M <= 0 || N <= 0 || Cs <= 0 || W <= 0) return EPI_ERR_INVALID_ARGUMENT;
+    if (Cs % GBK) return EPI_ERR_UNSUPPORTED;
+    const PatchPlan pl = patch_plan(M, N, Cs, W, (size_t)-1);
+    int bm, bn, tm, wmv;
+    patch_cfg_dims(pl.cfg, bm, bn, tm, wmv);
+    const long long v[10] = {pl.ok ? 1 : 0, bm, bn, pl.ts, pl.nb, pl.tiles, pl.nsplit, pl.cps, (long long)pl.lds, pl.single ? 1 : 0};
+    for (int i = 0; i < 10; ++i) out[i] = v[i];
+    return EPI_OK;
 }
 static bool patch_eligible(const GemmArgs& a, bool out_f32, int nphase) {
     if (patch_mode() == 0 || out_f32 || nphase != 1 || !a.ga.enabled || a.ph.enabled || a.sc.enabled || a.bias || !a.coalesce) return false;
@@ -1383,18 +1436,18 @@
         if (a.ga.dy[t] < -1 || a.ga.dy[t] > 1 || a.ga.dx[t] < -1 || a.ga.dx[t] > 1) return false;
     return (long long)a.M * a.ga.Cs < (1LL << 31) && gemm_tile_override() == 0;
 }
-template <typename Cfg, int NB, bool SINGLE = false, bool RED = false>
+template <typename Cfg, int NB, bool SINGLE = false, bool RED = false, int TS = 1>
 static int launch_patch_red(const GemmArgs& a, const PatchPlan& pl, hipStream_t st) {
-    static const hipError_t attr = hipFuncSetAttribute(reinterpret_cast<const void*>(&conv_patch_kernel<Cfg, NB, SINGLE, RED>),
+    static const hipError_t attr = hipFuncSetAttribute(reinterpret_cast<const void*>(&conv_patch_kernel<Cfg, NB, SINGLE, RED, TS>),
                                                        hipFuncAttributeMaxDynamicSharedMemorySize, 160 * 1024);
     if (attr != hipSuccess) return EPI_ERR_LAUNCH;
-    hipLaunchKernelGGL((conv_patch_kernel<Cfg, NB, SINGLE, RED>), dim3((unsigned)pl.tiles, (unsigned)pl.nsplit), dim3(Cfg::THREADS), pl.lds, st, a);
+    hipLaunchKernelGGL((conv_patch_kernel<Cfg, NB, SINGLE, RED, TS>), dim3((unsigned)pl.tiles, (unsigned)pl.nsplit), dim3(Cfg::THREADS), pl.lds, st, a);
     EPI_CHECK_LAUNCH();
     return EPI_OK;
 }
-template <typename Cfg, int NB, bool SINGLE = false>
+template <typename Cfg, int NB, bool SINGLE = false, int TS = 1>
 static int launch_patch(const GemmArgs& a, const PatchPlan& pl, hipStream_t st) {
-    return a.br.z ? launch_patch_red<Cfg, NB, SINGLE, true>(a, pl, st) : launch_patch_red<Cfg, NB, SINGLE, false>(a, pl, st);
+    return a.br.z ? launch_patch_red<Cfg, NB, SINGLE, true, TS>(a, pl, st) : launch_patch_red<Cfg, NB, SINGLE, false, TS>(a, pl, st);
 }
 
 static int launch_gemm(GemmArgs a, bool out_f32, int nphase, void* workspace, size_t workspace_bytes, hipStream_t st, int* stats_done = nullptr,
@@ -1483,7 +1536,8 @@
             else if (want_stats) { a.stats = want_stats; if (stats_done) *stats_done = 1; }
             else if (want_red.z) { a.br = want_red; *red_done = 1; }
             int rc;
-            if (pp.cfg == PATCH_NARROW && pp.single) rc = pp.nb == 3 ? launch_patch<PatchNarrow, 3, true>(a, pp, st) : launch_patch<PatchNarrow, 2, true>(a, pp, st);
+            if (pp.ts == 3) rc = pp.cfg == PATCH_DEEP ? launch_patch<PatchDeep, 3, false, 3>(a, pp, st) : launch_patch<PatchHalf, 2, false, 3>(a, pp, st);
+            else if (pp.cfg == PATCH_NARROW && pp.single) rc = pp.nb == 3 ? launch_patch<PatchNarrow, 3, true>(a, pp, st) : launch_patch<PatchNarrow, 2, true>(a, pp, st);
             else if (pp.cfg == PATCH_NARROW) rc = pp.nb == 3 ? launch_patch<PatchNarrow, 3>(a, pp, st) : launch_patch<PatchNarrow, 2>(a, pp, st);
             else if (pp.cfg == PATCH_HALF) rc = pp.nb == 3 ? launch_patch<PatchHalf, 3>(a, pp, st) : launch_patch<PatchHalf, 2>(a, pp, st);
             else rc = pp.nb == 3 ? launch_patch<PatchWide, 3>(a, pp, st) : launch_patch<PatchWide, 2>(a, pp, st);
diff --git a/epipolarpose_amd/hip.py b/epipolarpose_amd/hip.py
--- a/epipolarpose_amd/hip.py
+++ b/epipolarpose_amd/hip.py
@@ -73,6 +73,8 @@
     "epi_wgrad_item": (_i, [_vp, _vp, _sz, _vp, _vp]),
     "epi_bn_sum_copies": (_i, [_i]),
     "epi_conv3x3_patch_mode": (_i, [_i]),
+    "epi_conv3x3_patch_variant": (_i, [_i, _i]),
+    "epi_conv3x3_patch_plan": (_i, [_i, _i, _i, _i, ctypes.POINTER(ctypes.c_longlong)]),
     "epi_gemm_tune": (_i, [_i, _i]),
     "epi_gemm_store_policy": (_i, [_i]),
     "epi_set_deterministic": (_i, [_i]),
@@ -805,6 +807,20 @@
     return int(load().epi_conv3x3_patch_mode(int(mode)))
 
 
+def conv3x3_patch_variant(variant=-1, nsplit=-1):
+    before = int(load().epi_conv3x3_patch_variant(int(variant), int(nsplit)))
+    return before % 16, before // 16
+
+
+PATCH_PLAN_FIELDS = ("ok", "tile_m", "tile_n", "taps_per_step", "ring_steps", "tiles", "nsplit", "chunks_per_split", "lds_bytes", "single")
+
+
+def conv3x3_patch_plan(m, n, cs, w):
+    out = (ctypes.c_longlong * 10)()
+    _check(load().epi_conv3x3_patch_plan(int(m), int(n), int(cs), int(w), out), "epi_conv3x3_patch_plan")
+    return dict(zip(PATCH_PLAN_FIELDS, (int(v) for v in out)))
+
+
 def set_deterministic(on=True):
     before = int(load().epi_set_deterministic(1 if on else 0))
     if before < 0:
diff --git a/include/epipolar_hip.h b/include/epipolar_hip.h
--- a/include/epipolar_hip.h
+++ b/include/epipolar_hip.h
@@ -163,6 +163,8 @@
 
 size_t epi_conv2d_workspace_bytes(int B, int H, int W, int Cin, int Cout, int KH, int KW, int stride, int pad);
 int epi_conv3x3_patch_mode(int mode);
+int epi_conv3x3_patch_variant(int variant, int nsplit);
+int epi_conv3x3_patch_plan(int M, int N, int Cs, int W, long long* out);
 int epi_gemm_tune(int tile, int pipe);
 int epi_gemm_store_policy(int policy);
 int epi_conv2d_fwd(const void* x, const void* w, void* y, int B, int H, int W, int Cin, int Cout, int KH, int KW,
```

After: 5351 images/s (median of 6 runs). No clear change (+0.9%).
